# masnottuh/point-cloud-toolbox

Measured on AMD Instinct MI355X. Metric: points/sec curvature (1M-pt torus, k=50); HBM GB/s k-NN vs peak, higher is better.
Workload: dtype f64

## Files before the change

### point-cloud-toolbox_amd/csrc/pct_api.hip

```cpp
#include "pct_internal.h"

#include <execinfo.h>
#include <math.h>
#include <mutex>
#include <signal.h>
#include <stdarg.h>
#include <stdlib.h>
#include <sys/prctl.h>
#include <unistd.h>

int pct_fail(pct_ctx* ctx, int code, const char* fmt, ...) {
    if (ctx) {
        va_list ap;
        va_start(ap, fmt);
        vsnprintf(ctx->err, sizeof(ctx->err), fmt, ap);
        va_end(ap);
    }
    return code;
}

extern char** environ;
const char* pct_getenv(const char* name) {
    struct Entry { const char* name; const char* value; };
    static std::mutex m;
    static Entry cache[48];
    static int used = 0;
    static uintptr_t fp = 0;
    std::lock_guard<std::mutex> g(m);
    uintptr_t now = 1469598103934665603ull;
    for (char** e = environ; e && *e; ++e) now = (now ^ (uintptr_t)*e) * 1099511628211ull;
    if (now != fp) { fp = now; used = 0; }
    for (int i = 0; i < used; ++i)
        if (cache[i].name == name) return cache[i].value;
    const char* v = getenv(name);
    if (used < 48) cache[used++] = Entry{name, v};
    return v;
}

void pct_release(pct_buf* b) {
    if (b->p) (void)hipFree(b->p);
    b->p = nullptr;
    b->cap = 0;
}

int pct_reserve(pct_ctx* ctx, pct_buf* b, size_t bytes) {
    if (bytes == 0) bytes = 16;
    if (b->cap >= bytes) return PCT_OK;
    if (b->p) {
        PCT_HIP(ctx, hipStreamSynchronize(ctx->stream));
        pct_release(b);
    }
    size_t want = bytes + bytes / 8 + 256;
    if (pct_getenv("PCT_NO_HEADROOM")) want = bytes;
    hipError_t e = hipMalloc(&b->p, want);
    if (e != hipSuccess) {
        b->p = nullptr;
        return pct_fail(ctx, PCT_ERR_OOM, "hipMalloc(%zu) failed: %s", want, hipGetErrorString(e));
    }
    b->cap = want;
    return PCT_OK;
}

static void release(pct_buf* b) { pct_release(b); }

static float ev_ms(const hipEvent_t* ev, int a, int b) {
    float ms = 0.f;
    if (hipEventElapsedTime(&ms, ev[a], ev[b]) != hipSuccess) ms = 0.f;
    return ms;
}
static float ev_ms(pct_ctx* ctx, int a, int b) { return ev_ms(ctx->ev, a, b); }

static unsigned long long* stat_slot(pct_ctx* ctx, int par) { return (unsigned long long*)(ctx->pin + (par ? 256 : 192)); }
static long long* svd_slot(pct_ctx* ctx, int par) { return (long long*)(ctx->pin + 2048 + 8 * par); }

static void finish_pending(pct_ctx* ctx, const hipEvent_t* ev) {
    pct_timings t = ctx->tm_snap;
    const unsigned long long* c = stat_slot(ctx, ctx->pend_par);
    t.ring_fallbacks = (int64_t)c[0];
    t.lds_overflows = (int64_t)c[1];
    t.flushes = (int64_t)c[2];
    t.candidate_steps = (int64_t)c[3];
    t.redone_queries = (int64_t)c[4];
    t.grid_ms = ev_ms(ev, 2, 3);
    t.knn_ms = ev_ms(ev, 3, 4);
    t.knn_fast_ms = ctx->pend_sorted ? ev_ms(ev, 3, 7) : 0.f;
    t.fit_ms = ev_ms(ev, 4, 6);
    t.total_ms = ev_ms(ev, 2, 6);
    t.fit_svd_rows = *svd_slot(ctx, ctx->pend_par);
    const int64_t redone = (int64_t)(unsigned)(c[7] & 0xFFFFFFFFull);
    if (ctx->pend_sorted && !ctx->pend_levels) ctx->uneven = redone * 20 > ctx->pend_owned && ctx->pend_owned >= 65536;
    else if (ctx->pend_levels && t.levels <= 1) ctx->uneven = false;
    ctx->tm_done = t;
    ctx->pending = false;
}

static int drain(pct_ctx* ctx) {
    if (!ctx->pending) return PCT_OK;
    const hipError_t e = hipStreamSynchronize(ctx->stream);
    finish_pending(ctx, ctx->ev);
    ctx->tm = ctx->tm_done;
    PCT_HIP(ctx, e);
    return PCT_OK;
}

extern "C" {

const char* pct_version(void) { return "pct_hip 0.1 (gfx950)"; }

int pct_device_count(int* count) {
    int n = 0;
    hipError_t e = hipGetDeviceCount(&n);
    if (e != hipSuccess) n = 0;
    if (count) *count = n;
    return e == hipSuccess ? PCT_OK : PCT_ERR_NO_DEVICE;
}

extern "C++" { const char* pct_last_launch = "(none)"; }
static struct sigaction g_prev_abrt;
static int g_abrt_fd = 2;
static volatile sig_atomic_t g_in_abort_trace = 0;
static void abort_trace(int) {
    if (g_in_abort_trace) {
        sigaction(SIGABRT, &g_prev_abrt, nullptr);
        raise(SIGABRT);
        return;
    }
    g_in_abort_trace = 1;
    static const char head[] = "\n[pct] SIGABRT -- native backtrace of the raising thread";
    const int fd = g_abrt_fd;
    (void)!write(fd, head, sizeof(head) - 1);
    char name[32] = {0};
    if (prctl(PR_GET_NAME, name, 0, 0, 0) == 0) {
        (void)!write(fd, " (", 2);
        (void)!write(fd, name, strnlen(name, sizeof(name)));
        (void)!write(fd, ")", 1);
    }
    (void)!write(fd, ":\n", 2);
    static const char last[] = "[pct] last kernel launched by the library: ";
    (void)!write(fd, last, sizeof(last) - 1);
    const char* ll = __atomic_load_n(&pct_last_launch, __ATOMIC_RELAXED);
    (void)!write(fd, ll, strlen(ll));
    (void)!write(fd, "\n", 1);
    void* frames[64];
    const int n = backtrace(frames, 64);
    backtrace_symbols_fd(frames, n, fd);
    sigaction(SIGABRT, &g_prev_abrt, nullptr);
    raise(SIGABRT);
}
static void install_abort_trace() {
    static std::once_flag once;
    std::call_once(once, [] {
        const char* e = getenv("PCT_ABORT_TRACE");
        if (!e) return;
        const int fd = atoi(e);
        if (fd > 2) g_abrt_fd = fd;
        void* warm[4];
        (void)backtrace(warm, 4);
        struct sigaction sa;
        memset(&sa, 0, sizeof(sa));
        sa.sa_handler = abort_trace;
        sigemptyset(&sa.sa_mask);
        sa.sa_flags = 0;
        sigaction(SIGABRT, &sa, &g_prev_abrt);
    });
}

int pct_create(int device, pct_ctx** out) {
    if (!out) return PCT_ERR_INVALID;
    *out = nullptr;
    install_abort_trace();
    int n = 0;
    if (hipGetDeviceCount(&n) != hipSuccess || n <= 0 || device < 0 || device >= n) return PCT_ERR_NO_DEVICE;
    if (hipSetDevice(device) != hipSuccess) return PCT_ERR_NO_DEVICE;
    pct_ctx* ctx = new pct_ctx();
    ctx->device = device;
    if (hipStreamCreateWithFlags(&ctx->stream, hipStreamNonBlocking) != hipSuccess) {
        delete ctx;
        return PCT_ERR_HIP;
    }
    for (auto& e : ctx->ev)
        if (hipEventCreate(&e) != hipSuccess) {
            delete ctx;
            return PCT_ERR_HIP;
        }
    for (int i = 2; i <= 7; ++i)
        if (hipEventCreate(&ctx->ev_prev[i]) != hipSuccess) {
            delete ctx;
            return PCT_ERR_HIP;
        }
    if (hipHostMalloc((void**)&ctx->pin, 4096, hipHostMallocMapped) != hipSuccess) {
        delete ctx;
        return PCT_ERR_OOM;
    }
    memset(ctx->pin, 0, 4096);
    *out = ctx;
    return PCT_OK;
}

void pct_destroy(pct_ctx* ctx) {
    if (!ctx) return;
    (void)hipSetDevice(ctx->device);
    if (ctx->stream) (void)hipStreamSynchronize(ctx->stream);
    pct_comm_release(ctx);
    pct_buf* all[] = {&ctx->xyz, &ctx->pts4, &ctx->pts4d, &ctx->cell_of, &ctx->cell_cnt, &ctx->cell_fill,
                      &ctx->scan_tmp, &ctx->occ, &ctx->redo, &ctx->row_of, &ctx->owned_pos, &ctx->cell_own, &ctx->cell_oth, &ctx->own_start, &ctx->sorted4, &ctx->sorted4d, &ctx->red, &ctx->nbr_pos,
                      &ctx->nbr_dist, &ctx->nbr_cnt, &ctx->counters, &ctx->coefs, &ctx->K, &ctx->H, &ctx->H2,
                      &ctx->stage_a, &ctx->stage_b, &ctx->stage_c, &ctx->stage_d, &ctx->row_done, &ctx->redo_m, &ctx->flag_buf, &ctx->dens_buf, &ctx->pub_pos, &ctx->pub_dist, &ctx->pub_cnt, &ctx->qpts4, &ctx->fit_flag, &ctx->lvl_src,
                      &ctx->tree_codes, &ctx->tree_vals, &ctx->tree_lvl, &ctx->tree_head, &ctx->tree_marks, &ctx->tree_seg, &ctx->tree_runs, &ctx->tree_range, &ctx->tree_bucket, &ctx->tree_tmp,
                      &ctx->pca, &ctx->pca_aux, &ctx->pca_nbr, &ctx->pca_orig,
                      &ctx->bin_rec, &ctx->bin_mat, &ctx->bin_plan, &ctx->bin_base};
    for (pct_buf* b : all) release(b);
    if (ctx->pin) (void)hipHostFree(ctx->pin);
    for (auto& e : ctx->ev)
        if (e) (void)hipEventDestroy(e);
    for (auto& e : ctx->ev_prev)
        if (e) (void)hipEventDestroy(e);
    if (ctx->stream) (void)hipStreamDestroy(ctx->stream);
    delete ctx;
}

const char* pct_last_error(const pct_ctx* ctx) { return ctx ? ctx->err : "null context"; }

static int begin_call(pct_ctx* ctx, bool wait_for_pending = true) {
    if (!ctx) return PCT_ERR_INVALID;
    ctx->err[0] = 0;
    PCT_HIP(ctx, hipSetDevice(ctx->device));
    if (wait_for_pending) PCT_TRY(drain(ctx));
    return PCT_OK;
}

static int new_cloud(pct_ctx* ctx, int64_t n) {
    if (n <= 0 || n > (int64_t)INT32_MAX - 1024) return pct_fail(ctx, PCT_ERR_INVALID, "cloud size %lld out of range", (long long)n);
    ctx->n = n;
    ctx->q_begin = 0;
    ctx->q_end = n;
    ctx->slab_parts = ctx->slab_part = 0;
    ctx->slab_split_valid = false;
    ctx->grid_valid = ctx->knn_valid = ctx->fit_valid = ctx->pts4_valid = ctx->qpts4_valid = false;
    ctx->pca_valid = false;
    ctx->has_f64 = false;
    ctx->no_cull = ctx->culled = false;
    ctx->retries = 0;
    ctx->tm = pct_timings{};
    return PCT_OK;
}

int pct_set_points_f32(pct_ctx* ctx, const float* xyz, int64_t n) {
    PCT_TRY(begin_call(ctx));
    if (!xyz) return pct_fail(ctx, PCT_ERR_INVALID, "null coordinates");
    PCT_TRY(new_cloud(ctx, n));
    PCT_TRY(pct_reserve(ctx, &ctx->xyz, (size_t)n * 3 * sizeof(float)));
    PCT_HIP(ctx, hipEventRecord(ctx->ev[0], ctx->stream));
    PCT_HIP(ctx, hipMemcpyAsync(ctx->xyz.p, xyz, (size_t)n * 3 * sizeof(float), hipMemcpyHostToDevice, ctx->stream));
    ctx->xyz_view = (const float*)ctx->xyz.p;
    PCT_HIP(ctx, hipEventRecord(ctx->ev[1], ctx->stream));
    PCT_HIP(ctx, hipStreamSynchronize(ctx->stream));
    ctx->tm.upload_ms = ev_ms(ctx, 0, 1);
    return PCT_OK;
}

int pct_set_points_f64(pct_ctx* ctx, const double* xyz, int64_t n) {
    PCT_TRY(begin_call(ctx));
    if (!xyz) return pct_fail(ctx, PCT_ERR_INVALID, "null coordinates");
    PCT_TRY(new_cloud(ctx, n));
    PCT_TRY(pct_reserve(ctx, &ctx->stage_a, (size_t)n * 3 * sizeof(double)));
    PCT_HIP(ctx, hipEventRecord(ctx->ev[0], ctx->stream));
    PCT_HIP(ctx, hipMemcpyAsync(ctx->stage_a.p, xyz, (size_t)n * 3 * sizeof(double), hipMemcpyHostToDevice, ctx->stream));
    PCT_TRY(pct_pack_points_f64(ctx, (const double*)ctx->stage_a.p));
    PCT_HIP(ctx, hipEventRecord(ctx->ev[1], ctx->stream));
    PCT_HIP(ctx, hipStreamSynchronize(ctx->stream));
    ctx->has_f64 = true;
    ctx->tm.upload_ms = ev_ms(ctx, 0, 1);
    return PCT_OK;
}

int pct_set_points_device_f32(pct_ctx* ctx, const void* dev_xyz, int64_t n) {
    PCT_TRY(begin_call(ctx));
    if (!dev_xyz) return pct_fail(ctx, PCT_ERR_INVALID, "null coordinates");
    PCT_TRY(new_cloud(ctx, n));
    PCT_TRY(pct_reserve(ctx, &ctx->xyz, (size_t)n * 3 * sizeof(float)));
    PCT_HIP(ctx, hipMemcpyAsync(ctx->xyz.p, dev_xyz, (size_t)n * 3 * sizeof(float), hipMemcpyDeviceToDevice, ctx->stream));
    PCT_HIP(ctx, hipStreamSynchronize(ctx->stream));
    ctx->xyz_view = (const float*)ctx->xyz.p;
    return PCT_OK;
}

int pct_use_points_device_f32(pct_ctx* ctx, const void* dev_xyz, int64_t n) {
    PCT_TRY(begin_call(ctx));
    if (!dev_xyz) return pct_fail(ctx, PCT_ERR_INVALID, "null coordinates");
    hipPointerAttribute_t attr;
    if (hipPointerGetAttributes(&attr, dev_xyz) != hipSuccess || attr.type != hipMemoryTypeDevice || attr.device != ctx->device) {
        (void)hipGetLastError();
        return pct_fail(ctx, PCT_ERR_INVALID, "pct_use_points_device_f32: not a device pointer of device %d", ctx->device);
    }
    PCT_TRY(new_cloud(ctx, n));
    ctx->xyz_view = (const float*)dev_xyz;
    return PCT_OK;
}

int pct_set_query_range(pct_ctx* ctx, int64_t begin, int64_t end) {
    PCT_TRY(begin_call(ctx));
    if (ctx->n <= 0) return pct_fail(ctx, PCT_ERR_INVALID, "no cloud loaded");
    if (begin < 0 || end > ctx->n || begin > end) return pct_fail(ctx, PCT_ERR_INVALID, "bad query range [%lld,%lld)", (long long)begin, (long long)end);
    ctx->q_begin = begin;
    ctx->q_end = end;
    ctx->slab_parts = ctx->slab_part = 0;
    ctx->slab_split_valid = false;
    ctx->knn_valid = ctx->fit_valid = ctx->grid_valid = false;
    ctx->no_cull = false;
    ctx->retries = 0;
    return PCT_OK;
}

int pct_set_query_slab(pct_ctx* ctx, int32_t part, int32_t parts) {
    PCT_TRY(begin_call(ctx));
    if (ctx->n <= 0) return pct_fail(ctx, PCT_ERR_INVALID, "no cloud loaded");
    if (parts > PCT_SLAB_PARTS_MAX || (parts >= 1 && (part < 0 || part >= parts)))
        return pct_fail(ctx, PCT_ERR_INVALID, "bad slab %d of %d (at most %d parts)", part, parts, PCT_SLAB_PARTS_MAX);
    if (parts >= 1 && (ctx->has_f64 || ctx->n < 4096))
        return pct_fail(ctx, PCT_ERR_INVALID, "slab ownership serves float32 clouds of at least 4096 points (use index ranges)");
    ctx->q_begin = 0;
    ctx->q_end = ctx->n;
    ctx->slab_parts = parts >= 1 ? parts : 0;
    ctx->slab_part = parts >= 1 ? part : 0;
    ctx->slab_split_valid = false;
    ctx->knn_valid = ctx->fit_valid = ctx->grid_valid = false;
    ctx->no_cull = false;
    ctx->retries = 0;
    return PCT_OK;
}

static int refuse_in_slab_mode(pct_ctx* ctx, const char* what) {
    if (ctx->slab_parts >= 1)
        return pct_fail(ctx, PCT_ERR_INVALID, "%s: this handle owns a slab, not an index range (pct_slab_records / pct_scatter_records)", what);
    return PCT_OK;
}

int pct_slab_counts(pct_ctx* ctx, int64_t* counts, int32_t parts) {
    PCT_TRY(begin_call(ctx));
    if (ctx->slab_parts < 1 || !ctx->slab_split_valid || !ctx->fit_valid)
        return pct_fail(ctx, PCT_ERR_INVALID, "pct_slab_counts: no slab pass on this handle (pct_set_query_slab, pct_curvature)");
    if (!counts || parts != ctx->slab_parts) return pct_fail(ctx, PCT_ERR_INVALID, "pct_slab_counts: %d parts asked, the cloud was cut into %d", parts, ctx->slab_parts);
    for (int p = 0; p < parts; ++p) counts[p] = ctx->slab_counts[p];
    return PCT_OK;
}

namespace {
__global__ __launch_bounds__(256) void k_slab_records(const float4* __restrict__ sorted4, const int* __restrict__ owned_pos,
                                                      const float* __restrict__ K, const float* __restrict__ H, int64_t rows,
                                                      float* __restrict__ out) {
    const int64_t r = (int64_t)blockIdx.x * 256 + threadIdx.x;
    if (r >= rows) return;
    out[3 * r + 0] = sorted4[owned_pos[r]].w;
    out[3 * r + 1] = K[r];
    out[3 * r + 2] = H[r];
}

__global__ __launch_bounds__(256) void k_scatter_records(const float* __restrict__ rec, int64_t n_rec, int64_t begin, int64_t end,
                                                         float* __restrict__ K, float* __restrict__ H, unsigned long long* __restrict__ hits) {
    const int64_t i = (int64_t)blockIdx.x * 256 + threadIdx.x;
    bool hit = false;
    if (i < n_rec) {
        const int64_t pub = (int64_t)__float_as_int(rec[3 * i + 0]);
        hit = pub >= begin && pub < end;
        if (hit) {
            K[pub - begin] = rec[3 * i + 1];
            H[pub - begin] = rec[3 * i + 2];
        }
    }
    const unsigned long long m = __ballot(hit);
    if ((threadIdx.x & 63) == 0 && m) atomicAdd(hits, (unsigned long long)__popcll(m));
}
}

int pct_slab_records(pct_ctx* ctx, float* dev_records, int64_t capacity_rows, int64_t* rows_out) {
    PCT_TRY(begin_call(ctx));
    if (ctx->slab_parts < 1 || !ctx->slab_split_valid || !ctx->fit_valid || !ctx->knn_sorted_space || !ctx->fit_row_order)
        return pct_fail(ctx, PCT_ERR_INVALID, "pct_slab_records: no slab pass on this handle (pct_set_query_slab, pct_curvature)");
    const int64_t rows = ctx->q_end - ctx->q_begin;
// ... 793 lines not shown
```

### point-cloud-toolbox_amd/csrc/pct_fit.hip

```cpp
#include "pct_internal.h"

#include <math.h>

namespace {

constexpr int kFitBlock = 64;

struct FitArgs {
    const float4* pts;
    const double4* ptsd;
    const int* table;
    const int* cnt;
    const int64_t* row_query;
    const int* row_query32;
    int64_t row_offset;
    int64_t rows;
    int k;
    int pitch;
    int kp;
    int out_by_row;
    int64_t out_base;
    int q_begin, q_end;
    float* coefs;
    float* K;
    float* H;
    float* H2;
    double* coefs64;
    double* K64;
    double* H64;
    int* flag_list;
    int* flag_count;
    int* flag_next;
    const unsigned long long* stat_src;
    unsigned long long* stat_dst;
    unsigned n_pts;
    const int* row_mask;
    int svd_accumulate;
    int blocks_per_xcd;
};

constexpr double kPivotRatioMin = 1e-6;

#define JACOBI_ROT(app, aqq, apq, arp, arq, vp0, vp1, vp2, vq0, vq1, vq2)          \
    do {                                                                            \
        if (apq != 0.0) {                                                           \
            const double alpha = 0.5 * (aqq - app);                                 \
            const double beta = apq;                                                \
            const double t = (alpha >= 0.0 ? beta : -beta) / (fabs(alpha) + sqrt(alpha * alpha + beta * beta)); \
            const double c = rsqrt(t * t + 1.0);                                    \
            const double s = t * c;                                                 \
            app -= t * apq;                                                         \
            aqq += t * apq;                                                         \
            apq = 0.0;                                                              \
            const double rp = arp, rq = arq;                                        \
            arp = c * rp - s * rq;                                                  \
            arq = s * rp + c * rq;                                                  \
            double a0 = vp0, b0 = vq0; vp0 = c * a0 - s * b0; vq0 = s * a0 + c * b0; \
            double a1 = vp1, b1 = vq1; vp1 = c * a1 - s * b1; vq1 = s * a1 + c * b1; \
            double a2 = vp2, b2 = vq2; vp2 = c * a2 - s * b2; vq2 = s * a2 + c * b2; \
        }                                                                           \
    } while (0)

__device__ __forceinline__ void monge_curvatures(float A, float B, float C, float D, float E, float& Kg, float& Kh) {
    const float Fx = D, Fy = E;
    const float Fxx = 2.0f * A, Fyy = 2.0f * B, Fxy = C;
    const float fx2 = Fx * Fx, fy2 = Fy * Fy;
    const float wgt = (1.0f + fx2) + fy2;
    const float den_k = wgt * wgt;
    const float den_h = (float)((double)wgt * sqrt((double)wgt));
    Kg = (Fxx * Fyy - Fxy * Fxy) / den_k;
    Kh = (((1.0f + fx2) * Fyy - ((2.0f * Fx) * Fy) * Fxy) + (1.0f + fy2) * Fxx) / (2.0f * den_h);
}

template <bool F64>
__device__ __forceinline__ void load_centred(const FitArgs& a, int id, double qx, double qy, double qz,
                                             float qxf, float qyf, float qzf, double& x, double& y, double& z) {
    if (F64) {
        const double4 p = a.ptsd[id];
        x = p.x - qx; y = p.y - qy; z = p.z - qz;
    } else {
        const float4 p = a.pts[id];
        x = (double)(p.x - qxf);
        y = (double)(p.y - qyf);
        z = (double)(p.z - qzf);
    }
}

template <bool F64>
__device__ __forceinline__ void plane_rotation(int m, double sx, double sy, double sz, double sxx, double sxy, double sxz,
                                               double syy, double syz, double szz, double fx, double fy, double fz,
                                               double lx, double ly, double lz, double (&rot)[9]) {
    const double inv_m = 1.0 / (double)m, inv_m1 = 1.0 / (double)(m - 1);
    const double mx = sx * inv_m, my_ = sy * inv_m, mz = sz * inv_m;
    double a00 = (sxx - sx * mx) * inv_m1, a01 = (sxy - sx * my_) * inv_m1, a02 = (sxz - sx * mz) * inv_m1;
    double a11 = (syy - sy * my_) * inv_m1, a12 = (syz - sy * mz) * inv_m1, a22 = (szz - sz * mz) * inv_m1;

    double v00 = 1, v01 = 0, v02 = 0, v10 = 0, v11 = 1, v12 = 0, v20 = 0, v21 = 0, v22 = 1;
#pragma unroll 1
    for (int sweep = 0; sweep < 8; ++sweep) {
        const double off = fabs(a01) + fabs(a02) + fabs(a12);
        if (off <= 1e-22 * (fabs(a00) + fabs(a11) + fabs(a22))) break;
        JACOBI_ROT(a00, a11, a01, a02, a12, v00, v10, v20, v01, v11, v21);
        JACOBI_ROT(a00, a22, a02, a01, a12, v00, v10, v20, v02, v12, v22);
        JACOBI_ROT(a11, a22, a12, a01, a02, v01, v11, v21, v02, v12, v22);
    }
    double n0, n1, n2;
    if (a00 <= a11 && a00 <= a22) { n0 = v00; n1 = v10; n2 = v20; }
    else if (a11 <= a22)          { n0 = v01; n1 = v11; n2 = v21; }
    else                          { n0 = v02; n1 = v12; n2 = v22; }

    double rx, ry, rz;
    if (F64) { rx = lx - fx; ry = ly - fy; rz = lz - fz; }
    else     { rx = (double)((float)lx - (float)fx); ry = (double)((float)ly - (float)fy); rz = (double)((float)lz - (float)fz); }
    {
        const double nn = sqrt((n0 * n0 + n1 * n1) + n2 * n2);
        const double rn = sqrt((rx * rx + ry * ry) + rz * rz);
        const double dot = ((n0 / nn) * (rx / rn) + (n1 / nn) * (ry / rn)) + (n2 / nn) * (rz / rn);
        if (dot < 0) { n0 = -n0; n1 = -n1; n2 = -n2; }
    }
    double r00 = 1, r01 = 0, r02 = 0, r10 = 0, r11 = 1, r12 = 0, r20 = 0, r21 = 0, r22 = 1;
    {
        const double nn = sqrt((n0 * n0 + n1 * n1) + n2 * n2);
        const double ax = n0 / nn, ay = n1 / nn, az = n2 / nn;
        const double v0 = ay, v1 = -ax;
        const double c = az;
        const double s = sqrt(v0 * v0 + v1 * v1);
        if (s != 0.0) {
            const double f = (1.0 - c) / (s * s);
            r00 = 1.0 + (-(v1 * v1)) * f;  r01 = (v1 * v0) * f;            r02 = v1;
            r10 = (v0 * v1) * f;           r11 = 1.0 + (-(v0 * v0)) * f;   r12 = -v0;
            r20 = -v1;                     r21 = v0;                       r22 = 1.0 + (-(v1 * v1) + -(v0 * v0)) * f;
        }
    }

    rot[0] = r00; rot[1] = r01; rot[2] = r02; rot[3] = r10; rot[4] = r11; rot[5] = r12; rot[6] = r20; rot[7] = r21; rot[8] = r22;
}

template <bool F64, bool OUT64 = false, bool STAGED = true, bool MASKED = false>
__global__ __launch_bounds__(kFitBlock) void k_fit(FitArgs a) {
    extern __shared__ int s_idx[];
    const int lane = threadIdx.x;
    if (blockIdx.x == 0) {
        if (lane == 0 && a.flag_next) *a.flag_next = 0;
        if (a.stat_dst && lane < 8) a.stat_dst[lane] = a.stat_src[lane];
    }
    const int64_t row0 = (a.blocks_per_xcd ? (int64_t)(blockIdx.x & 7u) * a.blocks_per_xcd + (blockIdx.x >> 3) : (int64_t)blockIdx.x) * kFitBlock;
    if (row0 >= a.rows) return;
    const int k = a.k, kp = a.kp;

    const int nrow = (int)min((int64_t)kFitBlock, a.rows - row0);
    if constexpr (STAGED) {
        const int sub = lane >> 4, c4 = (lane & 15) << 2;
        for (int cb = 0; cb < k; cb += 64) {
            const int c = cb + c4;
#pragma unroll 4
            for (int r0 = 0; r0 < kFitBlock; r0 += 4) {
                const int r = r0 + sub;
                if (r < nrow && c < a.pitch) {
                    const int4 v = *(const int4*)(a.table + (row0 + r) * a.pitch + c);
                    int* dst = s_idx + r * kp + c;
                    if (c + 0 < k) dst[0] = v.x;
                    if (c + 1 < k) dst[1] = v.y;
                    if (c + 2 < k) dst[2] = v.z;
                    if (c + 3 < k) dst[3] = v.w;
                }
            }
        }
    }
    __syncthreads();

    const int64_t row = row0 + lane;
    if (row >= a.rows) return;
    if constexpr (MASKED) {
        if (!a.row_mask[row]) return;
    }
    const int64_t qid = a.row_query32 ? (int64_t)a.row_query32[row] : a.row_query ? a.row_query[row] : row + a.row_offset;
    const float4 qp = a.pts[qid];
    const int pub = __float_as_int(qp.w);
    if (!a.out_by_row && (pub < a.q_begin || pub >= a.q_end)) return;
    const int64_t out = a.out_by_row ? row : (int64_t)pub - a.out_base;

    double qx = qp.x, qy = qp.y, qz = qp.z;
    if (F64) {
        const double4 qd = a.ptsd[qid];
        qx = qd.x; qy = qd.y; qz = qd.z;
    }
    const int m = a.cnt ? a.cnt[row] : k;
    const int* my = STAGED ? s_idx + lane * kp : a.table + row * a.pitch;
    const float nanf_ = __int_as_float(0x7fc00000);

    const auto hand_over = [&]() {
        const unsigned long long fm = __ballot(1);
        const int leader = (int)__builtin_ctzll(fm);
        int base = 0;
        if (lane == leader) base = atomicAdd(a.flag_count, (int)__popcll(fm));
        base = __shfl(base, leader);
        a.flag_list[base + (int)__popcll(fm & ((1ull << lane) - 1ull))] = (int)row;
    };
    if (m < 6) {
        if constexpr (OUT64) {
            for (int j = 0; j < 6; ++j) a.coefs64[out * 6 + j] = (double)nanf_;
            a.K64[out] = (double)nanf_; a.H64[out] = (double)nanf_;
        } else {
            for (int j = 0; j < 6; ++j) a.coefs[out * 6 + j] = nanf_;
            a.K[out] = nanf_; a.H[out] = nanf_; a.H2[out] = nanf_;
        }
        if (m >= 2) hand_over();
        return;
    }

    double sx = 0, sy = 0, sz = 0, sxx = 0, sxy = 0, sxz = 0, syy = 0, syz = 0, szz = 0;
    double fx = 0, fy = 0, fz = 0, lx = 0, ly = 0, lz = 0;
#define PASS1_ACC(x, y, z)                                                          \
    do {                                                                            \
        sx += x; sy += y; sz += z;                                                  \
        sxx = fma(x, x, sxx); sxy = fma(x, y, sxy); sxz = fma(x, z, sxz);           \
        syy = fma(y, y, syy); syz = fma(y, z, syz); szz = fma(z, z, szz);           \
    } while (0)
    bool bad_id = false;
    const auto checked = [&](int id) {
        bad_id |= (unsigned)id >= a.n_pts;
        return (int)min((unsigned)id, a.n_pts - 1u);
    };
    {
        int j = 0;
        for (; j + 8 <= m; j += 8) {
            double x[8], y[8], z[8];
#pragma unroll
            for (int u = 0; u < 8; ++u) load_centred<F64>(a, checked(my[j + u]), qx, qy, qz, qp.x, qp.y, qp.z, x[u], y[u], z[u]);
            if (j == 0) { fx = x[0]; fy = y[0]; fz = z[0]; }
#pragma unroll
            for (int u = 0; u < 8; ++u) PASS1_ACC(x[u], y[u], z[u]);
            lx = x[7]; ly = y[7]; lz = z[7];
        }
        for (; j < m; ++j) {
            double x, y, z;
            load_centred<F64>(a, checked(my[j]), qx, qy, qz, qp.x, qp.y, qp.z, x, y, z);
            if (j == 0) { fx = x; fy = y; fz = z; }
            PASS1_ACC(x, y, z);
            lx = x; ly = y; lz = z;
        }
    }
#undef PASS1_ACC
    if (bad_id) {
        if constexpr (OUT64) {
            for (int j = 0; j < 6; ++j) a.coefs64[out * 6 + j] = (double)nanf_;
            a.K64[out] = (double)nanf_; a.H64[out] = (double)nanf_;
        } else {
            for (int j = 0; j < 6; ++j) a.coefs[out * 6 + j] = nanf_;
            a.K[out] = nanf_; a.H[out] = nanf_; a.H2[out] = nanf_;
        }
        return;
    }
    double rot[9];
    plane_rotation<F64>(m, sx, sy, sz, sxx, sxy, sxz, syy, syz, szz, fx, fy, fz, lx, ly, lz, rot);
    const double r00 = rot[0], r01 = rot[1], r02 = rot[2], r10 = rot[3], r11 = rot[4], r12 = rot[5], r20 = rot[6], r21 = rot[7], r22 = rot[8];

    double g[21];
    double b[6];
#pragma unroll
    for (int i = 0; i < 21; ++i) g[i] = 0;
#pragma unroll
    for (int i = 0; i < 6; ++i) b[i] = 0;
#define PASS2_ACC(x, y, z)                                                          \
    do {                                                                            \
        const float pa = (float)((r00 * x + r01 * y) + r02 * z);                    \
        const float pb = (float)((r10 * x + r11 * y) + r12 * z);                    \
        const float pz = (float)((r20 * x + r21 * y) + r22 * z);                    \
        double c[6];                                                                \
        c[0] = (double)(pa * pa);                                                   \
        c[1] = (double)(pb * pb);                                                   \
        c[2] = (double)(pa * pb);                                                   \
        c[3] = (double)pa;                                                          \
        c[4] = (double)pb;                                                          \
        c[5] = 1.0;                                                                 \
        const double zz = (double)pz;                                               \
        int t = 0;                                                                  \
        _Pragma("unroll") for (int i = 0; i < 6; ++i) {                             \
            _Pragma("unroll") for (int jj = 0; jj <= i; ++jj) { g[t] = fma(c[i], c[jj], g[t]); ++t; } \
            b[i] = fma(c[i], zz, b[i]);                                             \
        }                                                                           \
    } while (0)
    {
        int j = 0;
        for (; j + 8 <= m; j += 8) {
            double x[8], y[8], z[8];
#pragma unroll
            for (int u = 0; u < 8; ++u) load_centred<F64>(a, my[j + u], qx, qy, qz, qp.x, qp.y, qp.z, x[u], y[u], z[u]);
#pragma unroll
            for (int u = 0; u < 8; ++u) PASS2_ACC(x[u], y[u], z[u]);
        }
        for (; j < m; ++j) {
            double x, y, z;
            load_centred<F64>(a, my[j], qx, qy, qz, qp.x, qp.y, qp.z, x, y, z);
            PASS2_ACC(x, y, z);
        }
    }
#undef PASS2_ACC

#define GI(i, j) ((i) * ((i) + 1) / 2 + (j))
    double dinv[6];
    bool well = true;
#pragma unroll
    for (int j = 0; j < 6; ++j) {
        double d = g[GI(j, j)];
#pragma unroll
        for (int p = 0; p < j; ++p) d -= g[GI(j, p)] * g[GI(j, p)];
        well = well && d > kPivotRatioMin * g[GI(j, j)];
        const double inv = rsqrt(d);
        dinv[j] = inv;
#pragma unroll
        for (int i = j + 1; i < 6; ++i) {
            double s = g[GI(i, j)];
#pragma unroll
            for (int p = 0; p < j; ++p) s -= g[GI(i, p)] * g[GI(j, p)];
            g[GI(i, j)] = s * inv;
        }
    }
#pragma unroll
    for (int i = 0; i < 6; ++i) {
        double s = b[i];
#pragma unroll
        for (int p = 0; p < i; ++p) s -= g[GI(i, p)] * b[p];
        b[i] = s * dinv[i];
    }
#pragma unroll
    for (int i = 5; i >= 0; --i) {
        double s = b[i];
#pragma unroll
        for (int p = i + 1; p < 6; ++p) s -= g[GI(p, i)] * b[p];
        b[i] = s * dinv[i];
    }
#undef GI
    if (!well) hand_over();
    if constexpr (OUT64) {
        double* co64 = a.coefs64 + out * 6;
        for (int j = 0; j < 6; ++j) co64[j] = b[j];
        const double Fx = b[3], Fy = b[4], Fxx = 2.0 * b[0], Fyy = 2.0 * b[1], Fxy = b[2];
        const double wgt = (1.0 + Fx * Fx) + Fy * Fy;
        a.K64[out] = (Fxx * Fyy - Fxy * Fxy) / (wgt * wgt);
        a.H64[out] = (((1.0 + Fx * Fx) * Fyy - ((2.0 * Fx) * Fy) * Fxy) + (1.0 + Fy * Fy) * Fxx) / (2.0 * (wgt * sqrt(wgt)));
        return;
    }
    const float A = (float)b[0], B = (float)b[1], C = (float)b[2];
    const float D = (float)b[3], E = (float)b[4], F = (float)b[5];
    float* co = a.coefs + out * 6;
    co[0] = A; co[1] = B; co[2] = C; co[3] = D; co[4] = E; co[5] = F;

    float Kg, Kh;
    monge_curvatures(A, B, C, D, E, Kg, Kh);
    a.K[out] = Kg;
    a.H[out] = Kh;
    a.H2[out] = Kh * Kh;
}

__global__ __launch_bounds__(256) void k_curv(const float* __restrict__ coefs, int64_t rows, float* __restrict__ K,
                                              float* __restrict__ H, float* __restrict__ H2) {
    const int64_t r = (int64_t)blockIdx.x * 256 + threadIdx.x;
    if (r >= rows) return;
    const float* c = coefs + r * 6;
    float Kg, Kh;
    monge_curvatures(c[0], c[1], c[2], c[3], c[4], Kg, Kh);
    K[r] = Kg;
    H[r] = Kh;
    H2[r] = Kh * Kh;
}

struct Lstsq6 {
    double A[6][6];
    double y[6];

    __device__ __forceinline__ void init() {
#pragma unroll
        for (int c = 0; c < 6; ++c) {
            y[c] = 0;
#pragma unroll
            for (int r = 0; r < 6; ++r) A[c][r] = 0;
        }
    }

    __device__ __forceinline__ void add(float pa, float pb, float pc) {
        double x[6] = {(double)(pa * pa), (double)(pb * pb), (double)(pa * pb), (double)pa, (double)pb, 1.0};
        double zi = (double)pc;
#pragma unroll
        for (int r = 0; r < 6; ++r) {
            const double xr = x[r];
            if (xr != 0.0) {
                const double rr = A[r][r];
                const double h = sqrt(rr * rr + xr * xr);
                const double inv = 1.0 / h;
                const double c = rr * inv, sn = xr * inv;
                A[r][r] = h;
#pragma unroll
                for (int c2 = r + 1; c2 < 6; ++c2) {
                    const double t = A[c2][r];
                    A[c2][r] = c * t + sn * x[c2];
                    x[c2] = c * x[c2] - sn * t;
                }
                const double t = y[r];
                y[r] = c * t + sn * zi;
                zi = c * zi - sn * t;
            }
        }
    }

    __device__ __forceinline__ void solve(int m, double (&sol)[6]) {
        double V[6][6];
#pragma unroll
        for (int c = 0; c < 6; ++c)
#pragma unroll
            for (int r = 0; r < 6; ++r) V[c][r] = c == r ? 1.0 : 0.0;
#pragma unroll 1
        for (int sweep = 0; sweep < 40; ++sweep) {
            bool rotated = false;
#pragma unroll
            for (int p = 0; p < 5; ++p) {
#pragma unroll
                for (int q = p + 1; q < 6; ++q) {
                    double al = 0, be = 0, ga = 0;
#pragma unroll
                    for (int r = 0; r < 6; ++r) {
                        al = fma(A[p][r], A[p][r], al);
                        be = fma(A[q][r], A[q][r], be);
                        ga = fma(A[p][r], A[q][r], ga);
                    }
                    if (ga != 0.0 && fabs(ga) > 1e-15 * sqrt(al * be)) {
                        rotated = true;
                        const double zeta = (be - al) / (2.0 * ga);
                        const double t = (zeta >= 0.0 ? 1.0 : -1.0) / (fabs(zeta) + sqrt(1.0 + zeta * zeta));
                        const double c = rsqrt(1.0 + t * t), sn = c * t;
#pragma unroll
                        for (int r = 0; r < 6; ++r) {
                            const double ap = A[p][r], aq = A[q][r];
                            A[p][r] = c * ap - sn * aq;
                            A[q][r] = sn * ap + c * aq;
                            const double vp = V[p][r], vq = V[q][r];
                            V[p][r] = c * vp - sn * vq;
                            V[q][r] = sn * vp + c * vq;
                        }
                    }
                }
            }
            if (!__any(rotated)) break;
        }
        double sig2[6], smax2 = 0;
#pragma unroll
        for (int c = 0; c < 6; ++c) {
            double t = 0;
#pragma unroll
            for (int r = 0; r < 6; ++r) t = fma(A[c][r], A[c][r], t);
            sig2[c] = t;
            smax2 = fmax(smax2, t);
        }
        const double rcond = 2.220446049250313e-16 * (double)(m > 6 ? m : 6);
        const double cut = rcond * sqrt(smax2);
#pragma unroll
        for (int r = 0; r < 6; ++r) sol[r] = 0;
#pragma unroll
        for (int c = 0; c < 6; ++c) {
            if (sqrt(sig2[c]) > cut) {
                double t = 0;
#pragma unroll
                for (int r = 0; r < 6; ++r) t = fma(A[c][r], y[r], t);
                const double w = t / sig2[c];
#pragma unroll
                for (int r = 0; r < 6; ++r) sol[r] = fma(V[c][r], w, sol[r]);
            }
        }
    }
};

template <bool F64, bool OUT64>
__global__ __launch_bounds__(64) void k_fit_svd(FitArgs a, const int* __restrict__ list, const int* __restrict__ list_count,
                                                long long* __restrict__ host_count) {
    const int total = *list_count;
    if (blockIdx.x == 0 && threadIdx.x == 0) *host_count = (a.svd_accumulate ? *host_count : 0ll) + total;
    const float nanf_ = __int_as_float(0x7fc00000);
    for (int64_t it = (int64_t)blockIdx.x * 64 + threadIdx.x; it < total; it += (int64_t)gridDim.x * 64) {
        const int64_t row = list[it];
        const int64_t qid = a.row_query32 ? (int64_t)a.row_query32[row] : a.row_query ? a.row_query[row] : row + a.row_offset;
        const float4 qp = a.pts[qid];
        const int64_t out = a.out_by_row ? row : (int64_t)__float_as_int(qp.w) - a.out_base;
        double qx = qp.x, qy = qp.y, qz = qp.z;
        if (F64) { const double4 qd = a.ptsd[qid]; qx = qd.x; qy = qd.y; qz = qd.z; }
        const int m = a.cnt ? a.cnt[row] : a.k;
        const int* my = a.table + row * a.pitch;

        double sx = 0, sy = 0, sz = 0, sxx = 0, sxy = 0, sxz = 0, syy = 0, syz = 0, szz = 0;
        double fx = 0, fy = 0, fz = 0, lx = 0, ly = 0, lz = 0;
        for (int j = 0; j < m; ++j) {
            double x, y, z;
            load_centred<F64>(a, (int)min((unsigned)my[j], a.n_pts - 1u), qx, qy, qz, qp.x, qp.y, qp.z, x, y, z);
            if (j == 0) { fx = x; fy = y; fz = z; }
            lx = x; ly = y; lz = z;
            sx += x; sy += y; sz += z;
            sxx = fma(x, x, sxx); sxy = fma(x, y, sxy); sxz = fma(x, z, sxz);
            syy = fma(y, y, syy); syz = fma(y, z, syz); szz = fma(z, z, szz);
        }
        double rot[9];
        plane_rotation<F64>(m, sx, sy, sz, sxx, sxy, sxz, syy, syz, szz, fx, fy, fz, lx, ly, lz, rot);

        Lstsq6 ls;
        ls.init();
#pragma unroll 1
        for (int j = 0; j < m; ++j) {
            double px, py, pz;
            load_centred<F64>(a, (int)min((unsigned)my[j], a.n_pts - 1u), qx, qy, qz, qp.x, qp.y, qp.z, px, py, pz);
            ls.add((float)((rot[0] * px + rot[1] * py) + rot[2] * pz), (float)((rot[3] * px + rot[4] * py) + rot[5] * pz),
                   (float)((rot[6] * px + rot[7] * py) + rot[8] * pz));
        }
        double sol[6];
        ls.solve(m, sol);
        if (m < 2) {
#pragma unroll
            for (int r = 0; r < 6; ++r) sol[r] = (double)nanf_;
        }
        if constexpr (OUT64) {
            double* co64 = a.coefs64 + out * 6;
            for (int j = 0; j < 6; ++j) co64[j] = sol[j];
            const double Fx = sol[3], Fy = sol[4], Fxx = 2.0 * sol[0], Fyy = 2.0 * sol[1], Fxy = sol[2];
            const double wgt = (1.0 + Fx * Fx) + Fy * Fy;
            a.K64[out] = (Fxx * Fyy - Fxy * Fxy) / (wgt * wgt);
            a.H64[out] = (((1.0 + Fx * Fx) * Fyy - ((2.0 * Fx) * Fy) * Fxy) + (1.0 + Fy * Fy) * Fxx) / (2.0 * (wgt * sqrt(wgt)));
        } else {
            const float Af = (float)sol[0], Bf = (float)sol[1], Cf = (float)sol[2], Df = (float)sol[3], Ef = (float)sol[4];
            float* co = a.coefs + out * 6;
            co[0] = Af; co[1] = Bf; co[2] = Cf; co[3] = Df; co[4] = Ef; co[5] = (float)sol[5];
            float Kg, Kh;
            monge_curvatures(Af, Bf, Cf, Df, Ef, Kg, Kh);
            a.K[out] = Kg;
            a.H[out] = Kh;
            a.H2[out] = Kh * Kh;
        }
    }
}

template <bool F64>
__global__ __launch_bounds__(64) void k_plane_rotate(const void* __restrict__ nbrs, int64_t batch, int m, double* __restrict__ out) {
    const int64_t b = (int64_t)blockIdx.x * 64 + threadIdx.x;
    if (b >= batch) return;
    const auto at = [&](int j, double& x, double& y, double& z) {
        if (F64) { const double* p = (const double*)nbrs + (b * m + j) * 3; x = p[0]; y = p[1]; z = p[2]; }
        else { const float* p = (const float*)nbrs + (b * m + j) * 3; x = (double)p[0]; y = (double)p[1]; z = (double)p[2]; }
    };
    double mx = 0, my = 0, mz = 0;
    for (int j = 0; j < m; ++j) { double x, y, z; at(j, x, y, z); mx += x; my += y; mz += z; }
    mx /= (double)m; my /= (double)m; mz /= (double)m;
    double sxx = 0, sxy = 0, sxz = 0, syy = 0, syz = 0, szz = 0;
    for (int j = 0; j < m; ++j) {
        double x, y, z;
        at(j, x, y, z);
        x -= mx; y -= my; z -= mz;
        sxx = fma(x, x, sxx); sxy = fma(x, y, sxy); sxz = fma(x, z, sxz);
        syy = fma(y, y, syy); syz = fma(y, z, syz); szz = fma(z, z, szz);
    }
    double fx, fy, fz, lx, ly, lz;
    at(0, fx, fy, fz);
    at(m - 1, lx, ly, lz);
    double rot[9];
    plane_rotation<F64>(m, 0.0, 0.0, 0.0, sxx, sxy, sxz, syy, syz, szz, fx, fy, fz, lx, ly, lz, rot);
    for (int j = 0; j < m; ++j) {
        double x, y, z;
        at(j, x, y, z);
        double* o = out + (b * m + j) * 3;
        o[0] = (rot[0] * x + rot[1] * y) + rot[2] * z;
        o[1] = (rot[3] * x + rot[4] * y) + rot[5] * z;
        o[2] = (rot[6] * x + rot[7] * y) + rot[8] * z;
    }
}

__global__ __launch_bounds__(64) void k_quadric_rows(const float* __restrict__ pts, int64_t batch, int m, float* __restrict__ coefs) {
    const int64_t b = (int64_t)blockIdx.x * 64 + threadIdx.x;
    if (b >= batch) return;
    Lstsq6 ls;
    ls.init();
#pragma unroll 1
    for (int j = 0; j < m; ++j) {
        const float* p = pts + (b * m + j) * 3;
        ls.add(p[0], p[1], p[2]);
    }
    double sol[6];
    ls.solve(m, sol);
    for (int j = 0; j < 6; ++j) coefs[b * 6 + j] = (float)sol[j];
}

__global__ __launch_bounds__(256) void k_prefix_rows(const int* __restrict__ sample_row, const int* __restrict__ owned_pos,
                                                     int q_begin, int64_t n_samples, int n_lo, int n_hi,
                                                     const int* __restrict__ nbr_pos, int nbr_pitch,
                                                     int* __restrict__ table, int pitch, int* __restrict__ cnt,
                                                     int64_t* __restrict__ row_query) {
    const int nn = n_hi - n_lo + 1;
    const int64_t row = blockIdx.x;
    if (row >= n_samples * nn) return;
    const int64_t s = row / nn;
    const int n = n_lo + (int)(row - s * nn);
    const int trow = sample_row[s];
    const int q = owned_pos ? owned_pos[trow] : trow + q_begin;
    int* dst = table + row * pitch;
    for (int j = threadIdx.x; j <= n; j += 256) dst[j] = j == 0 ? q : nbr_pos[(int64_t)trow * nbr_pitch + (j - 1)];
    if (threadIdx.x == 0) { cnt[row] = n + 1; row_query[row] = q; }
}

__global__ __launch_bounds__(256) void k_gather_fit(const int* __restrict__ row_of, int64_t first, int64_t rows,
                                                    const float* __restrict__ coefs, const float* __restrict__ K,
                                                    const float* __restrict__ H, const float* __restrict__ H2,
                                                    float* __restrict__ o_coefs, float* __restrict__ o_K,
                                                    float* __restrict__ o_H, float* __restrict__ o_H2) {
    const int64_t i = (int64_t)blockIdx.x * 256 + threadIdx.x;
    if (i >= rows) return;
    const int64_t r = row_of[first + i];
    if (o_coefs) {
#pragma unroll
        for (int j = 0; j < 6; ++j) o_coefs[i * 6 + j] = coefs[r * 6 + j];
    }
    if (o_K) o_K[i] = K[r];
    if (o_H) o_H[i] = H[r];
    if (o_H2) o_H2[i] = H2[r];
}

int launch(pct_ctx* ctx, const FitArgs& a0, bool f64) {
    FitArgs a = a0;
    a.kp = a.k | 1;
    if (a.row_mask && ((size_t)kFitBlock * a.kp * sizeof(int) > 64 * 1024 || a.coefs64))
        return pct_fail(ctx, PCT_ERR_INVALID, "masked fit: rows too long");
    size_t lds = (size_t)kFitBlock * a.kp * sizeof(int);
    const bool staged = lds <= 64 * 1024;
    if (!staged) lds = 0;
    int blocks = (int)((a.rows + kFitBlock - 1) / kFitBlock);
    if (blocks <= 0) return PCT_OK;
    a.blocks_per_xcd = pct_getenv("PCT_NO_XCD_MAP") ? 0 : (blocks + 7) / 8;
    if (a.blocks_per_xcd) blocks = a.blocks_per_xcd * 8;
    PCT_TRY(pct_reserve(ctx, &ctx->fit_flag, 64 + (size_t)a.rows * sizeof(int)));
    if (ctx->fit_flag.p != ctx->fit_flag_seen || ctx->fit_flag.cap != ctx->fit_flag_cap_seen) {
        PCT_HIP(ctx, hipMemsetAsync(ctx->fit_flag.p, 0, 64, ctx->stream));
        ctx->fit_flag_seen = ctx->fit_flag.p;
        ctx->fit_flag_cap_seen = ctx->fit_flag.cap;
        ctx->fit_parity = 0;
    }
    a.stat_src = nullptr;
    a.stat_dst = nullptr;
    if (ctx->stats_mirror_req && ctx->counters.p) {
        a.stat_src = (const unsigned long long*)ctx->counters.p;
        a.stat_dst = (unsigned long long*)(ctx->pin + (ctx->fit_par ? 256 : 192));
        ctx->stats_mirrored = true;
    }
    ctx->stats_mirror_req = false;
    a.flag_count = (int*)ctx->fit_flag.p + ctx->fit_parity;
    a.flag_next = (int*)ctx->fit_flag.p + (ctx->fit_parity ^ 1);
    ctx->fit_parity ^= 1;
    a.flag_list = (int*)ctx->fit_flag.p + 16;
#define PCT_FIT_LAUNCH(F_, O_)                                                                                      \
    do {                                                                                                            \
        if (a.row_mask && staged && !O_) PCT_LAUNCH((k_fit<F_, false, true, true>), dim3(blocks), dim3(kFitBlock), lds, ctx->stream, a); \
        else if (staged) PCT_LAUNCH((k_fit<F_, O_, true>), dim3(blocks), dim3(kFitBlock), lds, ctx->stream, a);  \
        else PCT_LAUNCH((k_fit<F_, O_, false>), dim3(blocks), dim3(kFitBlock), 0, ctx->stream, a);          \
    } while (0)
    if (a.coefs64) {
        if (f64) PCT_FIT_LAUNCH(true, true);
        else PCT_FIT_LAUNCH(false, true);
    } else if (f64) PCT_FIT_LAUNCH(true, false);
    else PCT_FIT_LAUNCH(false, false);
#undef PCT_FIT_LAUNCH
    PCT_HIP(ctx, hipGetLastError());
    const int sblocks = blocks < 1024 ? blocks : 1024;
    long long* note = (long long*)(ctx->pin + 2048 + 8 * ctx->fit_par);
    if (a.coefs64) {
        if (f64)
            PCT_LAUNCH((k_fit_svd<true, true>), dim3(sblocks), dim3(64), 0, ctx->stream, a, a.flag_list, a.flag_count, note);
        else
            PCT_LAUNCH((k_fit_svd<false, true>), dim3(sblocks), dim3(64), 0, ctx->stream, a, a.flag_list, a.flag_count, note);
    } else if (f64)
        PCT_LAUNCH((k_fit_svd<true, false>), dim3(sblocks), dim3(64), 0, ctx->stream, a, a.flag_list, a.flag_count, note);
    else
        PCT_LAUNCH((k_fit_svd<false, false>), dim3(sblocks), dim3(64), 0, ctx->stream, a, a.flag_list, a.flag_count, note);
    PCT_HIP(ctx, hipGetLastError());
    return PCT_OK;
}

}

int pct_launch_fit_pass(pct_ctx* ctx, int64_t rows) {
    const int64_t nq = ctx->q_end - ctx->q_begin;
    PCT_TRY(pct_reserve(ctx, &ctx->coefs, (size_t)nq * 6 * sizeof(float)));
    PCT_TRY(pct_reserve(ctx, &ctx->K, (size_t)nq * sizeof(float)));
    PCT_TRY(pct_reserve(ctx, &ctx->H, (size_t)nq * sizeof(float)));
    PCT_TRY(pct_reserve(ctx, &ctx->H2, (size_t)nq * sizeof(float)));
    FitArgs a = {};
    a.pts = (const float4*)ctx->sorted4.p;
    a.ptsd = ctx->has_f64 ? (const double4*)ctx->sorted4d.p : nullptr;
    a.table = (const int*)ctx->nbr_pos.p;
    a.cnt = ctx->eps > 0 ? (const int*)ctx->nbr_cnt.p : nullptr;
    a.row_query32 = (const int*)ctx->owned_pos.p;
    a.rows = rows;
    a.k = ctx->k;
    a.pitch = (ctx->k + 3) & ~3;
    a.out_by_row = 0;
    a.out_base = ctx->q_begin;
    a.q_begin = (int)ctx->q_begin;
    a.q_end = (int)ctx->q_end;
    a.coefs = (float*)ctx->coefs.p;
    a.K = (float*)ctx->K.p;
    a.H = (float*)ctx->H.p;
    a.H2 = (float*)ctx->H2.p;
    a.n_pts = (unsigned)ctx->n_grid;
    a.row_mask = (const int*)ctx->row_done.p;
    a.svd_accumulate = 1;
    return launch(ctx, a, ctx->has_f64);
}

int pct_launch_fit_table(pct_ctx* ctx) {
    if (ctx->levels_fitted) {
        ctx->levels_fitted = false;
        ctx->fit_row_order = false;
        return PCT_OK;
    }
    const int64_t nq = ctx->q_end - ctx->q_begin;
    PCT_TRY(pct_reserve(ctx, &ctx->coefs, (size_t)nq * 6 * sizeof(float)));
    PCT_TRY(pct_reserve(ctx, &ctx->K, (size_t)nq * sizeof(float)));
    PCT_TRY(pct_reserve(ctx, &ctx->H, (size_t)nq * sizeof(float)));
    PCT_TRY(pct_reserve(ctx, &ctx->H2, (size_t)nq * sizeof(float)));
    FitArgs a = {};
    const bool sorted = ctx->knn_sorted_space;
    a.pts = (const float4*)(sorted ? ctx->sorted4.p : ctx->pts4.p);
    a.ptsd = ctx->has_f64 ? (const double4*)(sorted ? ctx->sorted4d.p : ctx->pts4d.p) : nullptr;
    a.table = (const int*)ctx->nbr_pos.p;
    a.cnt = ctx->eps > 0 ? (const int*)ctx->nbr_cnt.p : nullptr;
    a.row_query = nullptr;
    a.row_query32 = sorted ? (const int*)ctx->owned_pos.p : nullptr;
    a.row_offset = sorted ? 0 : ctx->q_begin;
    a.rows = nq;
    a.k = ctx->k;
    a.pitch = ctx->nbr_pitch;
    a.out_by_row = sorted ? 1 : 0;
    ctx->fit_row_order = sorted;
    a.out_base = ctx->q_begin;
    a.q_begin = (int)ctx->q_begin;
    a.q_end = (int)ctx->q_end;
    a.coefs = (float*)ctx->coefs.p;
    a.K = (float*)ctx->K.p;
    a.H = (float*)ctx->H.p;
    a.H2 = (float*)ctx->H2.p;
    a.n_pts = (unsigned)(sorted ? ctx->n_grid : ctx->n);
    return launch(ctx, a, ctx->has_f64);
}

int pct_launch_gather_fit(pct_ctx* ctx, int64_t first, int64_t rows, float* d_coefs, float* d_K, float* d_H, float* d_H2) {
    PCT_TRY(pct_ensure_row_of(ctx));
    PCT_LAUNCH(k_gather_fit, dim3((unsigned)((rows + 255) / 256)), dim3(256), 0, ctx->stream, (const int*)ctx->row_of.p,
                       first, rows, (const float*)ctx->coefs.p, (const float*)ctx->K.p, (const float*)ctx->H.p,
                       (const float*)ctx->H2.p, d_coefs, d_K, d_H, d_H2);
    PCT_HIP(ctx, hipGetLastError());
    return PCT_OK;
}

int pct_launch_fit_rows(pct_ctx* ctx, const int32_t* d_idx, const int32_t* d_cnt, const int64_t* d_query,
                        int64_t rows, int32_t k, int32_t pitch, float* d_coefs, float* d_K, float* d_H, float* d_H2,
                        bool sorted_space) {
    FitArgs a = {};
    a.pts = (const float4*)(sorted_space ? ctx->sorted4.p : ctx->pts4.p);
    a.ptsd = ctx->has_f64 ? (const double4*)(sorted_space ? ctx->sorted4d.p : ctx->pts4d.p) : nullptr;
    a.table = d_idx;
    a.cnt = d_cnt;
    a.row_query = d_query;
    a.rows = rows;
    a.k = k;
    a.pitch = pitch;
    a.out_by_row = 1;
    a.out_base = 0;
    a.q_begin = 0;
    a.q_end = (int)ctx->n;
    a.coefs = d_coefs;
    a.K = d_K;
    a.H = d_H;
    a.H2 = d_H2;
    a.n_pts = (unsigned)(sorted_space ? ctx->n_grid : ctx->n);
    return launch(ctx, a, ctx->has_f64);
}

int pct_launch_fit_rows_f64(pct_ctx* ctx, const int32_t* d_idx, const int32_t* d_cnt, const int64_t* d_query, int64_t rows,
                            int32_t k, int32_t pitch, double* d_coefs, double* d_K, double* d_H) {
    PCT_TRY(pct_ensure_plain_records(ctx));
    FitArgs a = {};
    a.pts = (const float4*)ctx->qpts4.p;
    a.ptsd = ctx->has_f64 ? (const double4*)ctx->pts4d.p : nullptr;
    a.table = d_idx;
    a.cnt = d_cnt;
    a.row_query = d_query;
    a.rows = rows;
    a.k = k;
    a.pitch = pitch;
    a.out_by_row = 1;
    a.q_begin = 0;
    a.q_end = (int)ctx->n;
    a.coefs64 = d_coefs;
    a.K64 = d_K;
    a.H64 = d_H;
    a.n_pts = (unsigned)ctx->n;
    return launch(ctx, a, ctx->has_f64);
}

int pct_launch_prefix_rows(pct_ctx* ctx, const int* d_sample_row, int64_t n_samples, int n_lo, int n_hi, int* d_table,
                           int pitch, int* d_cnt, int64_t* d_row_query) {
    const int64_t rows = n_samples * (n_hi - n_lo + 1);
    PCT_LAUNCH(k_prefix_rows, dim3((unsigned)rows), dim3(256), 0, ctx->stream, d_sample_row,
                       ctx->knn_sorted_space ? (const int*)ctx->owned_pos.p : nullptr, (int)ctx->q_begin, n_samples, n_lo, n_hi,
                       (const int*)ctx->nbr_pos.p, ctx->nbr_pitch, d_table, pitch, d_cnt, d_row_query);
    PCT_HIP(ctx, hipGetLastError());
    return PCT_OK;
}

int pct_launch_curvatures(pct_ctx* ctx, const float* d_coefs, int64_t rows, float* d_K, float* d_H, float* d_H2) {
    const int blocks = (int)((rows + 255) / 256);
    if (blocks <= 0) return PCT_OK;
    PCT_LAUNCH(k_curv, dim3(blocks), dim3(256), 0, ctx->stream, d_coefs, rows, d_K, d_H, d_H2);
    PCT_HIP(ctx, hipGetLastError());
    return PCT_OK;
}

int pct_launch_plane_rotate(pct_ctx* ctx, const void* d_nbrs, bool f64, int64_t batch, int32_t m, double* d_out) {
    const unsigned blocks = (unsigned)((batch + 63) / 64);
    if (f64)
        PCT_LAUNCH(k_plane_rotate<true>, dim3(blocks), dim3(64), 0, ctx->stream, d_nbrs, batch, m, d_out);
    else
        PCT_LAUNCH(k_plane_rotate<false>, dim3(blocks), dim3(64), 0, ctx->stream, d_nbrs, batch, m, d_out);
    PCT_HIP(ctx, hipGetLastError());
    return PCT_OK;
}

int pct_launch_quadric_rows(pct_ctx* ctx, const float* d_pts, int64_t batch, int32_t m, float* d_coefs) {
    PCT_LAUNCH(k_quadric_rows, dim3((unsigned)((batch + 63) / 64)), dim3(64), 0, ctx->stream, d_pts, batch, m, d_coefs);
    PCT_HIP(ctx, hipGetLastError());
    return PCT_OK;
}
```

### point-cloud-toolbox_amd/csrc/pct_internal.h

```cpp
#pragma once

#include <hip/hip_runtime.h>
#include <stdint.h>
#include <stdio.h>
#include <string.h>
#include <stdlib.h>

#include "../../include/pct_hip.h"

#define PCT_WAVE 64
#define PCT_K_MAX 511

extern const char* pct_last_launch;
#define PCT_STR2(x) #x
#define PCT_STR(x) PCT_STR2(x)
#define PCT_LAUNCH(kernelName, ...)                                                          \
    do {                                                                                     \
        __atomic_store_n(&pct_last_launch, __FILE__ ":" PCT_STR(__LINE__) "  " #kernelName, __ATOMIC_RELAXED); \
        hipLaunchKernelGGL((kernelName), __VA_ARGS__);                                       \
    } while (0)

struct pct_grid {
    double ox, oy, oz;
    double cell;
    double inv_cell;
    int32_t nx, ny, nz;
    int64_t ncell;
    double lim_lo[3], lim_hi[3];
};

struct pct_buf {
    void* p = nullptr;
    size_t cap = 0;
};

struct pct_comm;

struct pct_ctx {
    int device = 0;
    pct_comm* comm = nullptr;
    hipStream_t stream = nullptr;
    hipEvent_t ev[9] = {};
    hipEvent_t ev_prev[9] = {};
    bool async_mode = false;
    bool pending = false;
    int pend_par = 0;
    bool pend_sorted = false, pend_levels = false;
    int64_t pend_owned = 0;
    int fit_par = 0;
    pct_timings tm_snap = {};
    pct_timings tm_done = {};
    char err[512] = {0};

    int64_t n = 0;
    int64_t q_begin = 0, q_end = 0;
    int64_t n_grid = 0, g_begin = 0;
    bool culled = false;
    bool no_cull = false;
    float cull_box[6] = {0, 0, 0, 0, 0, 0};
    bool cull_box_valid = false;
    int64_t cull_box_n = 0, cull_box_q0 = 0, cull_box_q1 = 0;
    int32_t retries = 0;
    int32_t slab_part = 0, slab_parts = 0;
    int32_t slab_axis = 0, slab_bin_lo = 0, slab_bin_hi = 0;
    float slab_x0 = 0, slab_inv = 0;
    float slab_bbox[6] = {0, 0, 0, 0, 0, 0};
    int64_t slab_counts[PCT_SLAB_PARTS_MAX] = {};
    bool slab_split_valid = false;
    double hint_edge = 0, hint_guess = 0, hint_target = 0;
    float spec_bbox[6] = {0, 0, 0, 0, 0, 0};
    float spec_raw[6] = {0, 0, 0, 0, 0, 0};
    int64_t spec_n = 0;
    bool spec_valid = false;
    const void* own_flag = nullptr;
    float own_lo = 0, own_hi = 0;
    float level_box[6] = {0, 0, 0, 0, 0, 0};
    bool level_box_valid = false;
    int64_t own_count = 0;
    double level_edge = 0;
    bool level_mode = false;
    bool levels_fuse_fit = false;
    bool levels_fitted = false;
    pct_buf lvl_src;
    bool lvl_src_valid = false;
    float lvl_bbox[6] = {0, 0, 0, 0, 0, 0};
    int tree_bits = 0;
    int64_t tree_segs = 0;
    double tree_two_level_share = 1.0;
    int tree_level_spread = 0;
    pct_buf tree_codes, tree_vals;
    pct_buf tree_lvl;
    pct_buf tree_head, tree_marks;
    pct_buf tree_seg, tree_runs;
    pct_buf tree_range;
    pct_buf tree_bucket;
    pct_buf tree_tmp;
    pct_buf row_done;
    pct_buf redo_m;
    pct_buf flag_buf;
    pct_buf dens_buf;
    pct_buf pub_pos, pub_dist, pub_cnt;
    bool uneven = false;
    bool auto_probe = false;
    bool auto_probe_tree = false;
    bool grid_skewed = false;
    float auto_tree_bbox[6] = {0, 0, 0, 0, 0, 0};
    float tree_bbox[6] = {0, 0, 0, 0, 0, 0};
    bool tree_check_bbox = false, tree_hint_mismatch = false;
    int64_t auto_tree_n = 0;
    int32_t auto_tree_calls = 0;
    bool last_levels = false;
    bool has_f64 = false;
    double occupancy_factor = 0.0;
    bool collect_stats = false;

    pct_buf xyz;
    const float* xyz_view = nullptr;
    pct_buf pts4;
    pct_buf pts4d;
    pct_grid grid = {};
    pct_buf cell_of;
    pct_buf cell_cnt;
    pct_buf cell_own;
    pct_buf cell_oth;
    pct_buf own_start;
    pct_buf cell_fill;
    pct_buf scan_tmp;
    pct_buf bin_rec;
    pct_buf bin_mat;
    pct_buf bin_plan;
    pct_buf bin_base;
    pct_buf occ;
    pct_buf redo;
    int64_t n_items = 0;
    int64_t nonempty_cells = 0;
    int32_t items_q = 12;
    pct_buf sorted4;
    pct_buf sorted4d;
    pct_buf row_of;
    bool row_of_valid = true;
    int64_t row_of_rows = 0;
    int32_t row_of_begin = 0;
    pct_buf owned_pos;
    pct_buf red;
    unsigned char* pin = nullptr;
    int64_t n_occ = 0;
    bool grid_valid = false;
    bool pts4_valid = false;

    pct_buf nbr_pos;
    pct_buf nbr_dist;
    pct_buf nbr_cnt;
    int32_t k = 0;
    int32_t nbr_pitch = 0;
    double eps = 0.0;
    bool counters_clean = false;
    int fit_parity = 0;
    void* fit_flag_seen = nullptr;
    size_t fit_flag_cap_seen = 0;
    bool stats_mirror_req = false;
    bool stats_mirrored = false;
    bool knn_valid = false;
    bool knn_sorted_space = false;
    bool skip_dist_req = false;
    bool dist_valid = true;
    pct_buf counters;

    pct_buf coefs;
    pct_buf K, H, H2;
    int64_t fit_rows = 0;
    bool fit_valid = false;
    bool fit_row_order = false;
    bool fit_cloud_aligned = false;

    pct_buf fit_flag;
    pct_buf stage_a, stage_b, stage_c, stage_d;
    pct_buf qpts4;
    bool qpts4_valid = false;

    pct_buf pca;
    pct_buf pca_aux;
    pct_buf pca_nbr;
    pct_buf pca_orig;
    bool pca_valid = false, pca_has_nbr = false, pca_recentred = false;
    int32_t pca_k = 0;
    int64_t pca_rows = 0;

    pct_timings tm = {};
};

int pct_fail(pct_ctx* ctx, int code, const char* fmt, ...);
const char* pct_getenv(const char* name);
void pct_comm_release(pct_ctx* ctx);

#ifndef PCT_FAST_R1_MAX
#define PCT_FAST_R1_MAX 61
#endif
inline int pct_fast_r1_max() {
    static const int v = [] { const char* e = getenv("PCT_FAST_R1_MAX"); const int x = e ? atoi(e) : PCT_FAST_R1_MAX; return x < 2 ? 2 : x > 64 ? 64 : x; }();
    return v;
}
inline double pct_default_factor(int k) {
    if (k + 1 <= pct_fast_r1_max()) {
        const double per_cell = k <= 47 ? 27.0 : k >= 52 ? 29.5 : 27.0 + 0.5 * (k - 47);
        return per_cell / (k + 1);
    }
    const double n = k + 1;
    if (n > 128) return 0.35;
    return n <= 85 ? 0.52 : n <= 101 ? 0.52 - 0.07 * (n - 85) / 16.0 : 0.45 - 0.05 * (n - 101) / 27.0;
}
int pct_reserve(pct_ctx* ctx, pct_buf* b, size_t bytes);
void pct_release(pct_buf* b);

__host__ __device__ inline unsigned long long pct_spread3(unsigned v) {
    unsigned long long x = v & 0x1fffffu;
    x = (x | x << 32) & 0x1f00000000ffffull;
    x = (x | x << 16) & 0x1f0000ff0000ffull;
    x = (x | x << 8) & 0x100f00f00f00f00full;
    x = (x | x << 4) & 0x10c30c30c30c30c3ull;
    x = (x | x << 2) & 0x1249249249249249ull;
    return x;
}
__host__ __device__ inline unsigned pct_compact3(unsigned long long x) {
    x &= 0x1249249249249249ull;
    x = (x ^ (x >> 2)) & 0x10c30c30c30c30c3ull;
    x = (x ^ (x >> 4)) & 0x100f00f00f00f00full;
    x = (x ^ (x >> 8)) & 0x1f0000ff0000ffull;
    x = (x ^ (x >> 16)) & 0x1f00000000ffffull;
    x = (x ^ (x >> 32)) & 0x1fffffull;
    return (unsigned)x;
}
__host__ __device__ inline void pct_stencil_cell(int t, int* dx, int* dy, int* dz) {
    const int i = t == 0 ? 13 : t == 13 ? 0 : t;
    *dx = i % 3 - 1;
    *dy = (i / 3) % 3 - 1;
    *dz = i / 9 - 1;
}
__device__ inline int64_t pct_code_lower_bound(const unsigned long long* __restrict__ codes, int64_t n, unsigned long long key) {
    int64_t lo = 0, hi = n;
    while (lo < hi) {
        const int64_t mid = (lo + hi) >> 1;
        if (codes[mid] < key) lo = mid + 1; else hi = mid;
    }
    return lo;
}
constexpr int kTreeBucketBits = 18, kTreeBucketShift = 63 - kTreeBucketBits;
__device__ inline int64_t pct_code_lower_bound(const unsigned long long* __restrict__ codes, const int* __restrict__ bucket,
                                               unsigned long long key) {
    const unsigned p = (unsigned)(key >> kTreeBucketShift);
    int64_t lo = bucket[p], hi = bucket[p + 1];
    while (lo < hi) {
        const int64_t mid = (lo + hi) >> 1;
        if (codes[mid] < key) lo = mid + 1; else hi = mid;
    }
    return lo;
}

#define PCT_HIP(ctx, call)                                                        \
    do {                                                                          \
        hipError_t e_ = (call);                                                   \
        if (e_ != hipSuccess)                                                     \
            return pct_fail((ctx), e_ == hipErrorOutOfMemory ? PCT_ERR_OOM : PCT_ERR_HIP, \
                            "%s failed: %s (%s:%d)", #call, hipGetErrorString(e_), __FILE__, __LINE__); \
    } while (0)

#define PCT_TRY(expr)            \
    do {                         \
        int s_ = (expr);         \
        if (s_ != PCT_OK) return s_; \
    } while (0)

int pct_pack_points(pct_ctx* ctx, float* bbox6);
int pct_pack_points_f64(pct_ctx* ctx, const double* d_xyz64);
int pct_build_grid(pct_ctx* ctx, int32_t k, double eps);
int pct_launch_knn_grid(pct_ctx* ctx, int32_t k, double eps, bool exact_only, int phase = 0);
int pct_launch_knn_brute(pct_ctx* ctx, int32_t k, double eps);
int pct_item_census(pct_ctx* ctx, int32_t k, unsigned long long out4[4]);
int pct_knn_levels(pct_ctx* ctx, int32_t k, double eps);
int pct_build_tree(pct_ctx* ctx, int32_t k, double eps, bool* usable);
int pct_launch_knn_tree(pct_ctx* ctx, int32_t k, double eps);
int pct_launch_export_neighbors(pct_ctx* ctx, int64_t begin, int64_t end,
                                int32_t* d_idx, float* d_dist, int32_t* d_cnt);
int pct_launch_fit_table(pct_ctx* ctx);
int pct_launch_fit_pass(pct_ctx* ctx, int64_t rows);
int pct_launch_fit_rows(pct_ctx* ctx, const int32_t* d_idx, const int32_t* d_cnt,
                        const int64_t* d_query, int64_t rows, int32_t k, int32_t pitch,
                        float* d_coefs, float* d_K, float* d_H, float* d_H2, bool sorted_space);
int pct_launch_prefix_rows(pct_ctx* ctx, const int* d_sample_pos, int64_t n_samples, int n_lo, int n_hi, int* d_table,
                           int pitch, int* d_cnt, int64_t* d_row_query);
int pct_launch_gather_fit(pct_ctx* ctx, int64_t first, int64_t rows, float* d_coefs, float* d_K, float* d_H, float* d_H2);
int pct_launch_curvatures(pct_ctx* ctx, const float* d_coefs, int64_t rows, float* d_K, float* d_H, float* d_H2);
int pct_launch_plane_rotate(pct_ctx* ctx, const void* d_nbrs, bool f64, int64_t batch, int32_t m, double* d_out);
int pct_launch_quadric_rows(pct_ctx* ctx, const float* d_pts, int64_t batch, int32_t m, float* d_coefs);
int pct_launch_selftest(pct_ctx* ctx, int* d_fails);
int pct_ensure_plain_records(pct_ctx* ctx);
int pct_launch_fit_rows_f64(pct_ctx* ctx, const int32_t* d_idx, const int32_t* d_cnt, const int64_t* d_query, int64_t rows,
                            int32_t k, int32_t pitch, double* d_coefs, double* d_K, double* d_H);
int pct_launch_query_points(pct_ctx* ctx, const double* d_q, int64_t m, int32_t k, double eps, int32_t* d_idx, double* d_dist);
int pct_launch_gather_int(pct_ctx* ctx, const int* d_map, int* d_inout, int64_t n);
int pct_ensure_row_of(pct_ctx* ctx);
int pct_launch_export_rows(pct_ctx* ctx, const int64_t* d_rows, int64_t n_rows, int32_t* d_idx, float* d_dist, int32_t* d_cnt);
int pct_launch_mesh_energies(pct_ctx* ctx, const double* d_v, const int* d_tri, int64_t n_tri, const void* d_K, const void* d_H,
                             bool f64, double* d_partial, int nblk, double* d_out);
int pct_voxel_downsample_device(pct_ctx* ctx, const void* d_xyz, bool f64, int64_t n, double voxel, int64_t* d_out, int64_t* count);
int pct_launch_surface_variation(pct_ctx* ctx, float* d_out);
#define PCT_PCA_EXTRA 16
int pct_pca_prep(pct_ctx* ctx, double* round_off, bool* nonfinite, double origin[3]);
int pct_pca_restore(pct_ctx* ctx);
int pct_launch_pca(pct_ctx* ctx, int32_t k, double round2, const double origin[3], bool keep_neighbors, int64_t* exact_rows);
```

### point-cloud-toolbox_amd/csrc/pct_knn.hip

```cpp
#include "pct_knn_sweep.h"

namespace {

constexpr unsigned kPadElem = 0xFFFFFFFFu;

template <int R>
struct FastK {
    unsigned e[R];
};

__device__ __forceinline__ unsigned umed3(unsigned a, unsigned b, unsigned c) {
    unsigned r;
    asm("v_med3_u32 %0, %1, %2, %3" : "=v"(r) : "v"(a), "v"(b), "v"(c));
    return r;
}

struct SortLanes {
    unsigned sel[6];
    int a31, a63;
};

__device__ __forceinline__ SortLanes make_sort_lanes() {
    SortLanes c;
    const int lane = lane_id();
// ... 116 lines not shown
            double pd = INFINITY;
#pragma unroll
            for (int r2 = 0; r2 < R; ++r2)
                if (pr == r2) { pe = be[r2]; pd = __hiloint2double(bhi[r2], blo[r2]); }
            const bool same = pr >= 0 && pr < R && e[r] != kPadElem && pe != kPadElem && ((e[r] ^ pe) >> SLOT_BITS) == 0u;
            bool p_lt_m = pd < d[r], m_lt_p = d[r] < pd;
            const bool tie = same && pd == d[r];
            if (__builtin_amdgcn_ballot_w64(tie) != 0ull) {
                const int my_pos = pos_of(e[r] & PAYLOAD), p_pos = pos_of(pe & PAYLOAD);
                if (tie) {
                    const int mp = pub_index(pts, my_pos), pp = pub_index(pts, p_pos);
                    p_lt_m = pp < mp;
                    m_lt_p = mp < pp;
                }
            }
            const bool take = same && (pl > lane ? p_lt_m : m_lt_p);
            if (take) { e[r] = pe; d[r] = pd; }
            any |= take;
        }
        if (__builtin_amdgcn_ballot_w64(any) != 0ull) quiet = 0;
        else if (++quiet == 2) return true;
    }
    return false;
}

#ifndef PCT_FAST_WAVES
#define PCT_FAST_WAVES 4
#endif
template <int R> constexpr int kFastWaves = PCT_FAST_WAVES;

typedef float float2v __attribute__((ext_vector_type(2)));


template <int R, bool EPS, bool PRE, bool PAIR = false, bool Q64 = false, bool TREE = false>
__global__ __launch_bounds__(64 * kFastWaves<R>, (TREE ? (R == 1 ? (PCT_TREE_CAP <= 512 ? 6 : PCT_TREE_CAP <= 768 ? 4 : 3) : (PCT_TREE_CAP2 <= 768 ? 4 : 3)) : R == 1 ? (Q64 ? 5 : 6) : 4)) void k_knn_fast(KnnArgs a, const int2* __restrict__ items, int64_t n_items,
                                                                  int items_q, int* __restrict__ redo,
                                                                  int* __restrict__ redo_count) {
#ifndef PCT_STAGE_CAP2
#define PCT_STAGE_CAP2 768
#endif
    constexpr int CAP = TREE ? (R == 1 ? PCT_TREE_CAP : PCT_TREE_CAP2) : R == 1 ? kStageCap : PCT_STAGE_CAP2;
    constexpr int SLOT_BITS = PRE ? (R == 1 ? 6 : 7) : (R == 1 ? 9 : 10);
    constexpr int KEY_BITS = 32 - SLOT_BITS;
    constexpr int CAP_POW2 = 1024;
    static_assert(CAP <= CAP_POW2, "staging capacity");
    static_assert(PRE || CAP <= (1 << SLOT_BITS), "slot field too narrow");
    __shared__ float s_cx[kFastWaves<R>][CAP];
    __shared__ float s_cy[kFastWaves<R>][CAP];
    __shared__ float s_cz[kFastWaves<R>][CAP];
    __shared__ unsigned s_pend[kFastWaves<R>][64 * R];
    __shared__ unsigned short s_pend2[kFastWaves<R>][PAIR ? 64 * R : 2];
    __shared__ int s_offc[kFastWaves<R>][16];

    const int w = __builtin_amdgcn_readfirstlane(threadIdx.x >> 6);
    const int lane = lane_id();
    const int64_t item = (int64_t)blockIdx.x * kFastWaves<R> + w;
    if (item >= n_items) return;
    const SortLanes sort_dir = make_sort_lanes();

    pct_grid g = a.g;
    const int* __restrict__ cs = a.cell_start;
    const int2 it2 = items[item];
    int cx, cy, cz, qs, nq, row0;
    constexpr int NRUNS = TREE ? 27 : 9;
    int run_s = 0, run_len = 0;
    float* cand_x = s_cx[w];
    float* cand_y = s_cy[w];
    float* cand_z = s_cz[w];
    unsigned* pend = s_pend[w];
    int* offc = s_offc[w];
    if constexpr (TREE) {
        const int seg = __builtin_amdgcn_readfirstlane(it2.y);
        if (seg < 0) return;
        const unsigned packed = (unsigned)__builtin_amdgcn_readfirstlane(it2.x);
        qs = (int)(packed & 0x3ffffffu);
        nq = (int)(packed >> 26) + 1;
        row0 = qs;
        const int4 hd = a.tree_seg[seg];
        const int level = __builtin_amdgcn_readfirstlane(hd.x);
        cx = __builtin_amdgcn_readfirstlane(hd.y);
        cy = __builtin_amdgcn_readfirstlane(hd.z);
        cz = __builtin_amdgcn_readfirstlane(hd.w);
        g.cell = __builtin_ldexp(a.g.cell, level);
        g.inv_cell = __builtin_ldexp(a.g.inv_cell, -level);
        g.nx = g.ny = g.nz = 1 << (a.tree_bits - level);
        if (lane < 27) {
            const int2 r = a.tree_runs[(int64_t)seg * 27 + lane];
            run_s = r.x;
            run_len = r.y;
        }
    } else {
        const int cell = __builtin_amdgcn_readfirstlane(it2.x);
        const int chunk = __builtin_amdgcn_readfirstlane(it2.y);
        cx = cell % g.nx;
        cy = (cell / g.nx) % g.ny;
        cz = cell / (g.nx * g.ny);
        qs = cs[cell] + chunk * items_q;
        const int qe = min(cs[cell] + a.cell_own[cell], qs + items_q);
        nq = qe - qs;
        row0 = a.own_start[cell] + chunk * items_q;

        if (lane < 9) {
            const int z = cz + kRowOrder[lane][0], y = cy + kRowOrder[lane][1];
            if (z >= 0 && z < g.nz && y >= 0 && y < g.ny) {
                const int row = (z * g.ny + y) * g.nx;
                run_s = cs[row + max(cx - 1, 0)];
                run_len = cs[row + min(cx + 1, g.nx - 1) + 1] - run_s;
            }
        }
    }
    float4 my_q = make_float4(0.f, 0.f, 0.f, 0.f);
    double4 my_qd = make_double4(0., 0., 0., 0.);
    if (lane < nq) {
        my_q = a.pts[qs + lane];
        if (a.ptsd) my_qd = a.ptsd[qs + lane];
    }
    float my_eq = 0.f;
    if constexpr (Q64) {
        const double ex = my_qd.x - (double)my_q.x, ey = my_qd.y - (double)my_q.y, ez = my_qd.z - (double)my_q.z;
        my_eq = (float)sqrt((ex * ex + ey * ey) + ez * ez) * (1.0f + 0x1p-22f);
        if (!(my_eq >= 0.f)) my_eq = INFINITY;
    }
    int my_pre = 0, m = 0;
    {
        int acc = 0;
#pragma unroll
        for (int t = 0; t < NRUNS; ++t) {
            my_pre = lane == t ? acc : my_pre;
            acc += __builtin_amdgcn_readlane(run_len, t);
        }
        m = acc;
    }
    unsigned long long n_flush = 0, n_step = 0, n_redo = 0;
    unsigned long long redo_mask = 0ull, redo_why_lo = 0ull, redo_why_hi = 0ull;
    const auto note_redo = [&](int row, int why) {
        const int q = row - row0;
        redo_mask |= 1ull << q;
        redo_why_lo |= (unsigned long long)(why & 1) << q;
        redo_why_hi |= (unsigned long long)((why >> 1) & 1) << q;
    };

    const bool hopeless = !EPS && a.row_done != nullptr && m < a.k + 1;
    const bool crowded = TREE && __popcll(__builtin_amdgcn_ballot_w64(lane < NRUNS && run_len > 0)) > 16;
    if (m > CAP || hopeless || crowded) {
        if (a.row_done) {
            if (lane < nq) a.redo_m[row0 + lane] = ((hopeless ? 1 : 2) << 29) | min(m, (1 << 29) - 1);
            return;
        }
        int base = 0;
        if (lane == 0) base = atomicAdd(redo_count, nq);
        base = __builtin_amdgcn_readfirstlane(base);
        if (lane < nq) {
            redo[base + lane] = row0 + lane;
        }
        if (a.stats && lane == 0) {
            if (!hopeless) atomicAdd(&a.counters[1], 1ull);
            atomicAdd(&a.counters[4], (unsigned long long)nq);
        }
        return;
    }

    unsigned run_code[(CAP / 64 + 7) / 8];
#pragma unroll
    for (int i = 0; i < (CAP / 64 + 7) / 8; ++i) run_code[i] = 0u;
    {
        unsigned* bits = pend;
        static_assert(CAP / 32 <= 64 * R, "bit string does not fit the list area");
        if (lane < CAP / 32) bits[lane] = 0u;
        wave_lds_sync();
        const bool nonempty = lane < NRUNS && run_len > 0;
        const unsigned long long ne = __builtin_amdgcn_ballot_w64(nonempty);
        if (nonempty) {
            atomicOr(&bits[my_pre >> 5], 1u << (my_pre & 31));
            offc[__builtin_amdgcn_mbcnt_lo((unsigned)ne, 0)] = run_s - my_pre;
        }
        wave_lds_sync();
        float4 tmp[CAP / 64];
        int ubase = -1;
#pragma unroll
        for (int b = 0; b < CAP / 64; ++b) {
            tmp[b] = make_float4(0.f, 0.f, 0.f, 0.f);
            if (b * 64 < m) {
                const unsigned lo = (unsigned)__builtin_amdgcn_readfirstlane((int)bits[2 * b]);
                const unsigned hi = (unsigned)__builtin_amdgcn_readfirstlane((int)bits[2 * b + 1]);
                const unsigned long long B = ((unsigned long long)hi << 32) | lo;
                const unsigned long long S = B >> 1;
                const int c0 = ubase + (int)(lo & 1u);
                const int u = (int)__builtin_amdgcn_mbcnt_hi((unsigned)(S >> 32), __builtin_amdgcn_mbcnt_lo((unsigned)S, (unsigned)c0));
                ubase += (int)__popcll(B);
                const int j = b * 64 + lane;
                run_code[b >> 3] |= (unsigned)u << (4 * (b & 7));
                if (j < m) tmp[b] = a.pts[j + offc[u]];
            }
        }
        wave_lds_sync();
#pragma unroll
        for (int b = 0; b < CAP / 64; ++b) {
            const int j = b * 64 + lane;
            if (j < m) {
                cand_x[j] = tmp[b].x; cand_y[j] = tmp[b].y; cand_z[j] = tmp[b].z;
            } else if (PRE && (b & ~1) * 64 < m) {
                cand_x[j] = INFINITY; cand_y[j] = 0.f; cand_z[j] = 0.f;
            }
        }
    }
    wave_lds_sync();
    const int k = a.k;
    const double eps2 = EPS ? a.eps2 : (double)INFINITY;
    constexpr double kKeyRange = 2.3;
    const double scale = (double)(1u << KEY_BITS) / (kKeyRange * g.cell * g.cell);
    const unsigned key_max = (1u << KEY_BITS) - 1u;
    unsigned my_gkey;
    {
        const double lqx = a.ptsd ? my_qd.x : (double)my_q.x, lqy = a.ptsd ? my_qd.y : (double)my_q.y,
                     lqz = a.ptsd ? my_qd.z : (double)my_q.z;
        const double gx = (lqx - g.ox) * g.inv_cell - cx;
        const double gy = (lqy - g.oy) * g.inv_cell - cy;
        const double gz = (lqz - g.oz) * g.inv_cell - cz;
        const double g2 = fmin(guaranteed_r2(g, cx, cy, cz, gx, gy, gz, 1), limit_r2(g, cx, cy, cz, gx, gy, gz));
        my_gkey = g2 == INFINITY ? 0xFFFFFFFFu : (unsigned)fmin(g2 * scale, 4294967294.0);
    }
    const unsigned eps_key = EPS && eps2 < 1e300 ? (unsigned)fmin(ceil(eps2 * scale), 4294967295.0) : 0xFFFFFFFFu;

    constexpr int NB = CAP / 64;
    constexpr int LIST = 64 * R;
    unsigned t_prev = 0;
    float t_prev_f = 0.f;
    const float cell2f = (float)(g.cell * g.cell);
    const float eps2a = EPS ? (float)fmin(eps2 * (1.0 + 0x1p-18), 3.0e38) : INFINITY;
    const double eps1 = EPS ? sqrt(eps2) * (1.0 + 0x1p-50) : 0.0;

    if constexpr (PRE && PAIR) {
        unsigned short* pend_b = s_pend2[w];
        const auto push_redo = [&](int row, int why) { note_redo(row, why); };
        const auto cut_key = [&](float T, double eq) {
            double lo2 = (double)T * (1.0 - 0x1p-20);
            if constexpr (Q64) {
                const double root_up = (double)__builtin_sqrtf(T) * (1.0 + 0x1p-21);
                lo2 = fmax(lo2 - 2.0 * eq * root_up, 0.0);
            }
            return (unsigned)fmin(lo2 * scale, 4294967294.0);
        };
        const auto pair_loop = [&](auto NBP_, auto GUARD_) {
            constexpr int NBP = decltype(NBP_)::value, NBU = 2 * NBP;
            constexpr bool GUARD = decltype(GUARD_)::value;
            for (int qi = 0; qi < nq; qi += 2) {
                const bool live_b = qi + 1 < nq;
                const int qj = live_b ? qi + 1 : qi;
                const int row_a = row0 + qi, row_b = row0 + qj;
                float ax, ay, az, bx, by, bz;
                if constexpr (!Q64) {
                    ax = __int_as_float(__builtin_amdgcn_readlane(__float_as_int(my_q.x), qi));
                    ay = __int_as_float(__builtin_amdgcn_readlane(__float_as_int(my_q.y), qi));
                    az = __int_as_float(__builtin_amdgcn_readlane(__float_as_int(my_q.z), qi));
                    bx = __int_as_float(__builtin_amdgcn_readlane(__float_as_int(my_q.x), qj));
                    by = __int_as_float(__builtin_amdgcn_readlane(__float_as_int(my_q.y), qj));
                    bz = __int_as_float(__builtin_amdgcn_readlane(__float_as_int(my_q.z), qj));
                }
                double qax, qay, qaz, qbx, qby, qbz, eq_a = 0.0, eq_b = 0.0;
                if constexpr (Q64) {
                    const auto rl = [&](double v, int l) {
                        return __hiloint2double(__builtin_amdgcn_readlane(__double2hiint(v), l), __builtin_amdgcn_readlane(__double2loint(v), l));
                    };
                    qax = rl(my_qd.x, qi); qay = rl(my_qd.y, qi); qaz = rl(my_qd.z, qi);
                    qbx = rl(my_qd.x, qj); qby = rl(my_qd.y, qj); qbz = rl(my_qd.z, qj);
                    ax = (float)qax; ay = (float)qay; az = (float)qaz;
                    bx = (float)qbx; by = (float)qby; bz = (float)qbz;
                    eq_a = (double)__int_as_float(__builtin_amdgcn_readlane(__float_as_int(my_eq), qi));
                    eq_b = (double)__int_as_float(__builtin_amdgcn_readlane(__float_as_int(my_eq), qj));
                } else {
                    qax = (double)ax; qay = (double)ay; qaz = (double)az; qbx = (double)bx; qby = (double)by; qbz = (double)bz;
                }
                float ap_a[NBU], ap_b[NBU];
#pragma unroll
                for (int p2 = 0; p2 < NBP; ++p2) {
                    ap_a[2 * p2] = ap_a[2 * p2 + 1] = INFINITY;
                    ap_b[2 * p2] = ap_b[2 * p2 + 1] = INFINITY;
                    if (!GUARD || p2 * 128 < m) {
                        const int sa = p2 * 128 + lane, sb = sa + 64;
                        const float2v vx = {cand_x[sa], cand_x[sb]}, vy = {cand_y[sa], cand_y[sb]}, vz = {cand_z[sa], cand_z[sb]};
                        {
                            const float2v dx = vx - ax, dy = vy - ay, dz = vz - az;
                            float2v d = dx * dx;
                            d = __builtin_elementwise_fma(dy, dy, d);
                            d = __builtin_elementwise_fma(dz, dz, d);
                            ap_a[2 * p2] = d.x;
                            ap_a[2 * p2 + 1] = d.y;
                        }
                        {
                            const float2v dx = vx - bx, dy = vy - by, dz = vz - bz;
                            float2v d = dx * dx;
                            d = __builtin_elementwise_fma(dy, dy, d);
                            d = __builtin_elementwise_fma(dz, dz, d);
                            ap_b[2 * p2] = d.x;
                            ap_b[2 * p2 + 1] = d.y;
                        }
                        n_step += 4;
                    }
                }
                float T_a = EPS ? eps2a : INFINITY, T_b = T_a;
                if constexpr (EPS && Q64) {
                    const double ea = eps1 + eq_a, eb = eps1 + eq_b;
                    T_a = (float)fmin(ea * ea * (1.0 + 0x1p-18), 3.0e38);
                    T_b = (float)fmin(eb * eb * (1.0 + 0x1p-18), 3.0e38);
                }
                int tot_a = m, tot_b = m;
// ... 389 lines not shown
                        if (b * 64 < m) c += (int)__popcll(__builtin_amdgcn_ballot_w64(key[b] < t));
                    if (c >= k + 1 && c <= LIST) { T = t; cnt = c; found = true; break; }
                    if (c < k + 1) lo = t; else hi = t;
                    if (hi - lo <= 1u) break;
                    const float guess = (float)t * target * __builtin_amdgcn_rcpf((float)(c > 0 ? c : 1));
                    unsigned nt = guess >= 4294967040.f ? hi : (unsigned)guess;
                    if (c == 0) nt = t * 4u > t ? t * 4u : hi;
                    if (nt <= lo || nt >= hi) nt = lo + (hi - lo) / 2u;
                    t = nt;
                }
                if (!found) {
                    note_redo(row, 3);
                    continue;
                }
            }
            t_prev = T <= key_max ? T : t_prev;

            {
                int base = 0;
                wave_lds_sync();
#pragma unroll
                for (int b = 0; b < NB; ++b) {
                    if (b * 64 < m) {
                        const bool pass = key[b] < T;
                        const unsigned long long mask = __builtin_amdgcn_ballot_w64(pass);
                        if (pass) {
                            const int at = base + __builtin_amdgcn_mbcnt_hi((unsigned)(mask >> 32), __builtin_amdgcn_mbcnt_lo((unsigned)mask, 0));
                            pend[at] = (key[b] << SLOT_BITS) | (unsigned)(b * 64 + lane);
                        }
                        base += (int)__popcll(mask);
                    }
                }
                wave_lds_sync();
                const int have = cnt < LIST ? cnt : LIST;
#pragma unroll
                for (int r = 0; r < R; ++r) {
                    const int i = lane + 64 * r;
                    best.e[r] = i < have ? pend[i] : kPadElem;
                }
                wave_lds_sync();
                fast_sort_from<R, 2>(best, sort_dir);
                ++n_flush;
            }
        }
        unsigned tau;
        {
            const int sl = k >> 6, src = k & 63;
            unsigned v = best.e[0];
#pragma unroll
            for (int r = 1; r < R; ++r)
                if (sl == r) v = best.e[r];
            tau = (unsigned)__builtin_amdgcn_readlane((int)v, src);
        }

        bool sparse = false;
        {
            const unsigned gkey = (unsigned)__builtin_amdgcn_readlane((int)my_gkey, qi);
            const unsigned tkey = tau >> SLOT_BITS;
            const unsigned need = min(tau == kPadElem ? 0xFFFFFFFFu : tkey + 1u, eps_key);
            sparse = need > gkey;
            amb |= need > min(gkey, bkey);
            amb |= tau != kPadElem && tkey >= key_max - 1u;
        }
        {
#pragma unroll
            for (int r = 0; r < R; ++r) {
                unsigned up = __shfl_down(best.e[r], 1);
                if (r + 1 < R) {
                    const unsigned first_next = (unsigned)__builtin_amdgcn_readlane((int)best.e[r + 1 < R ? r + 1 : r], 0);
                    if (lane == 63) up = first_next;
                } else if (lane == 63) {
                    up = kPadElem;
                }
                const int i = lane + 64 * r;
                col |= i <= k && best.e[r] != kPadElem && up != kPadElem && ((best.e[r] ^ up) >> SLOT_BITS) == 0u;
            }
        }
        if (__ballot(amb) != 0ull) {
            note_redo(row, sparse ? 1 : 3);
            continue;
        }
        const auto slot_pos = [&](int j) {
            unsigned code = (unsigned)__builtin_amdgcn_ds_bpermute((j & 63) << 2, (int)run_code[0]);
            if constexpr ((CAP / 64 + 7) / 8 > 1) {
                const unsigned hi = (unsigned)__builtin_amdgcn_ds_bpermute((j & 63) << 2, (int)run_code[1]);
                code = (j >> 9) ? hi : code;
            }
            return j + offc[(code >> ((((unsigned)j >> 6) & 7u) << 2)) & 15u];
        };
        if (__ballot(col) != 0ull) {
            const auto slot_of = [&](unsigned at) {
                int j = (int)at;
                if constexpr (PRE) j = (int)pend[j] & (CAP_POW2 - 1);
                return j;
            };
            const bool done = order_equal_keys<R, SLOT_BITS>(&best.e[0], a.pts,
                [&](unsigned at) {
                    const int j = slot_of(at);
                    const double dx = (double)cand_x[j] - qx, dy = (double)cand_y[j] - qy, dz = (double)cand_z[j] - qz;
                    return (dx * dx + dy * dy) + dz * dz;
                },
                [&](unsigned at) { return slot_pos(slot_of(at) & (CAP_POW2 - 1)); });
            if (!done) {
                note_redo(row, 3);
                continue;
            }
        }

        int found = 0;
#pragma unroll
        for (int r = 0; r < R; ++r) {
            const int i = lane + 64 * r;
            const unsigned e = best.e[r];
            const bool real = e != kPadElem;
            int j = (int)(e & ((1u << SLOT_BITS) - 1u));
            if constexpr (PRE) j = (int)pend[j] & (CAP_POW2 - 1);
            unsigned code = (unsigned)__builtin_amdgcn_ds_bpermute((j & 63) << 2, (int)run_code[0]);
            if constexpr ((CAP / 64 + 7) / 8 > 1) {
                const unsigned hi = (unsigned)__builtin_amdgcn_ds_bpermute((j & 63) << 2, (int)run_code[1]);
                code = (j >> 9) ? hi : code;
            }
            const unsigned t = (code >> ((((unsigned)j >> 6) & 7u) << 2)) & 15u;
            const int pos_real = j + offc[t];
            if (i >= 1 && i <= k) {
                int pos = -1;
                float dist = INFINITY;
                if (real) {
                    const double dx = (double)cand_x[j] - qx, dy = (double)cand_y[j] - qy, dz = (double)cand_z[j] - qz;
                    dist = (float)sqrt((dx * dx + dy * dy) + dz * dz);
                    pos = pos_real;
                }
                a.nbr_pos[(int64_t)row * a.pitch + (i - 1)] = pos;
                a.nbr_dist[(int64_t)row * a.pitch + (i - 1)] = dist;
                found += real;
            }
        }
        if (a.nbr_cnt) {
            for (int o = 32; o > 0; o >>= 1) found += __shfl_xor(found, o);
            if (lane == 0) a.nbr_cnt[row] = found;
        }
        if (a.row_done && lane == 0) a.row_done[row] = 1;
    }
    if (redo_mask) {
        const int cnt = (int)__popcll(redo_mask);
        if (a.row_done) {
            if ((redo_mask >> lane) & 1ull) {
                const int why = (int)((redo_why_lo >> lane) & 1ull) | ((int)((redo_why_hi >> lane) & 1ull) << 1);
                a.redo_m[row0 + lane] = (why << 29) | min(m, (1 << 29) - 1);
            }
        } else {
            int base = 0;
            if (lane == 0) base = atomicAdd(redo_count, cnt);
            base = __builtin_amdgcn_readfirstlane(base);
            if ((redo_mask >> lane) & 1ull) redo[base + (int)__popcll(redo_mask & ((1ull << lane) - 1ull))] = row0 + lane;
        }
        n_redo += (unsigned long long)cnt;
    }
    if (a.stats && lane == 0) {
        atomicAdd(&a.counters[2], n_flush);
        atomicAdd(&a.counters[3], n_step);
        if (n_redo) atomicAdd(&a.counters[4], n_redo);
    }
}

#ifndef PCT_SORT_INC
#define PCT_SORT_INC "pct_sort_pair.inc"
#endif
#include PCT_SORT_INC

__device__ __forceinline__ void sort_pair_asm(unsigned& ea, unsigned& eb, const SortLanes& c) {
    unsigned ta, tb;
    asm volatile(PCT_SORT_PAIR_ASM
                 : [ea] "+v"(ea), [eb] "+v"(eb), [ta] "=&v"(ta), [tb] "=&v"(tb)
                 : [sel0] "v"(c.sel[0]), [sel1] "v"(c.sel[1]), [sel2] "v"(c.sel[2]), [sel3] "v"(c.sel[3]), [sel4] "v"(c.sel[4]),
                   [sel5] "v"(c.sel[5]), [a31] "v"(c.a31), [a63] "v"(c.a63));
    ea = PCT_SORT_PAIR_RESULT_A;
    eb = PCT_SORT_PAIR_RESULT_B;
}

struct PairArgs {
    const float4* pts;
    const double4* ptsd;
    const int* cell_start;
    const int* cell_own;
    const int* own_start;
    const int2* items;
    int* nbr_pos;
    float* nbr_dist;
    int* nbr_cnt;
    int* redo;
    int* redo_count;
    unsigned long long* counters;
    int n_items, items_q;
    int items_per_xcd;
    int k, pitch;
    int stats;
    unsigned magic_x, magic_xy;
    int shift_x, shift_xy;
    double eps2;
    pct_grid g;
    const int4* tree_seg;
    const int2* tree_runs;
    int tree_bits;
};

constexpr int kPairCap = kStageCap;
static_assert((kPairCap & (kPairCap - 1)) == 0 && kPairCap % 128 == 0 && kPairCap <= 512, "staging capacity of k_knn_pair");
static_assert(PCT_TREE_CAP % 128 == 0 && PCT_TREE_CAP <= 1024, "staging capacity of k_knn_pair on the hierarchical cell list");
template <int CAP>
struct PairLdsT {
    float cx[CAP], cy[CAP], cz[CAP];
    unsigned pend[64 + 4];
    unsigned short pend_b[64 + 8];
    int offc[16];
};
using PairLds = PairLdsT<kPairCap>;

#ifndef PCT_PAIR_WAVES
#define PCT_PAIR_WAVES 1
#endif
constexpr int kPairWaves = PCT_PAIR_WAVES;

template <bool EPS, bool DIST, bool Q64 = false, bool TREE = false>
__global__ __launch_bounds__(64 * kPairWaves, (TREE ? 4 : Q64 ? 5 : 6)) void k_knn_pair(PairArgs a) {
    constexpr int CAP = TREE ? PCT_TREE_CAP : kPairCap, LIST = 64, SLOT_BITS = 6, KEY_BITS = 32 - SLOT_BITS;
    constexpr int SB = TREE ? 10 : 9;
    constexpr unsigned kIdMask = (1u << (SB + 4)) - 1u;
    __shared__ PairLdsT<CAP> s_lds[kPairWaves];
    const int w = kPairWaves == 1 ? 0 : __builtin_amdgcn_readfirstlane(threadIdx.x >> 6);
    const int lane = lane_id();
    const int blk = (int)blockIdx.x * kPairWaves + w;
    const int item = a.items_per_xcd ? (blk & 7) * a.items_per_xcd + (blk >> 3) : blk;
    if (item >= a.n_items || (a.items_per_xcd && (blk >> 3) >= a.items_per_xcd)) return;
    PairLdsT<CAP>& L = s_lds[w];
    const SortLanes sort_dir = make_sort_lanes();
    const int* __restrict__ cs = a.cell_start;

    const int2 it2 = a.items[item];
    constexpr int NRUNS = TREE ? 27 : 9;
    int cx, cy, cz, qs, nq, row0;
    int run_s = 0, run_len = 0;
    pct_grid g_lvl;
    if constexpr (TREE) {
        const int seg = __builtin_amdgcn_readfirstlane(it2.y);
        if (seg < 0) return;
        const unsigned packed = (unsigned)__builtin_amdgcn_readfirstlane(it2.x);
        qs = (int)(packed & 0x3ffffffu);
        nq = (int)(packed >> 26) + 1;
        row0 = qs;
        const int4 hd = a.tree_seg[seg];
        const int level = __builtin_amdgcn_readfirstlane(hd.x);
        cx = __builtin_amdgcn_readfirstlane(hd.y);
        cy = __builtin_amdgcn_readfirstlane(hd.z);
        cz = __builtin_amdgcn_readfirstlane(hd.w);
        g_lvl = a.g;
        g_lvl.cell = __builtin_ldexp(a.g.cell, level);
        g_lvl.inv_cell = __builtin_ldexp(a.g.inv_cell, -level);
        g_lvl.nx = g_lvl.ny = g_lvl.nz = 1 << (a.tree_bits - level);
        if (lane < 27) {
            const int2 r = a.tree_runs[(int64_t)seg * 27 + lane];
            run_s = r.x;
            run_len = r.y;
        }
    } else {
        const int cell = __builtin_amdgcn_readfirstlane(it2.x);
        const int chunk = __builtin_amdgcn_readfirstlane(it2.y);
        const int nx = a.g.nx, ny = a.g.ny, nz = a.g.nz;
        cz = (int)(((unsigned long long)(unsigned)cell * a.magic_xy) >> a.shift_xy);
        const int rem = cell - cz * (nx * ny);
        cy = (int)(((unsigned long long)(unsigned)rem * a.magic_x) >> a.shift_x);
        cx = rem - cy * nx;
        const int c0 = cs[cell];
        qs = c0 + chunk * a.items_q;
        nq = min(c0 + a.cell_own[cell], qs + a.items_q) - qs;
        row0 = a.own_start[cell] + chunk * a.items_q;

        if (lane < 9) {
            const int z = cz + kRowOrder[lane][0], y = cy + kRowOrder[lane][1];
            if (z >= 0 && z < nz && y >= 0 && y < ny) {
                const int row = (z * ny + y) * nx;
                run_s = cs[row + max(cx - 1, 0)];
                run_len = cs[row + min(cx + 1, nx - 1) + 1] - run_s;
            }
        }
    }
    const pct_grid& G = TREE ? g_lvl : a.g;
    float4 my_q = make_float4(0.f, 0.f, 0.f, 0.f);
    double my_qx = 0., my_qy = 0., my_qz = 0.;
    float my_eq = 0.f;
    if (lane < nq) {
        my_q = a.pts[qs + lane];
        if constexpr (Q64) {
            const double4 qd = a.ptsd[qs + lane];
            my_qx = qd.x; my_qy = qd.y; my_qz = qd.z;
        }
    }
    if constexpr (Q64) {
        const double ex = my_qx - (double)my_q.x, ey = my_qy - (double)my_q.y, ez = my_qz - (double)my_q.z;
        my_eq = (float)sqrt((ex * ex + ey * ey) + ez * ez) * (1.0f + 0x1p-22f);
        if (!(my_eq >= 0.f)) my_eq = INFINITY;
    }
    int my_pre = 0, m = 0;
    {
        int acc = 0;
#pragma unroll
        for (int t = 0; t < NRUNS; ++t) {
            my_pre = lane == t ? acc : my_pre;
            acc += __builtin_amdgcn_readlane(run_len, t);
        }
        m = acc;
    }
    const bool crowded = TREE && __popcll(__builtin_amdgcn_ballot_w64(lane < NRUNS && run_len > 0)) > 16;
    if (m > CAP || crowded) {
        int base = 0;
        if (lane == 0) base = atomicAdd(a.redo_count, nq);
        base = __builtin_amdgcn_readfirstlane(base);
        if (lane < nq) a.redo[base + lane] = row0 + lane;
        if (a.stats && lane == 0) {
            atomicAdd(&a.counters[1], 1ull);
            atomicAdd(&a.counters[4], (unsigned long long)nq);
        }
        return;
    }

    unsigned slotx[CAP / 64];
    {
        unsigned* bits = L.pend;
        if (lane < CAP / 32) bits[lane] = 0u;
        wave_lds_sync();
        const bool nonempty = lane < NRUNS && run_len > 0;
        const unsigned long long ne = __builtin_amdgcn_ballot_w64(nonempty);
        if (nonempty) {
            atomicOr(&bits[my_pre >> 5], 1u << (my_pre & 31));
            L.offc[__builtin_amdgcn_mbcnt_lo((unsigned)ne, 0)] = run_s - my_pre;
        }
        wave_lds_sync();
        float4 tmp[CAP / 64];
        int ubase = -1;
#pragma unroll
        for (int b = 0; b < CAP / 64; ++b) {
            tmp[b] = make_float4(0.f, 0.f, 0.f, 0.f);
            slotx[b] = (unsigned)(b * 64 + lane);
            if (b * 64 < m) {
                const unsigned lo = (unsigned)__builtin_amdgcn_readfirstlane((int)bits[2 * b]);
                const unsigned hi = (unsigned)__builtin_amdgcn_readfirstlane((int)bits[2 * b + 1]);
                const unsigned long long B = ((unsigned long long)hi << 32) | lo;
                const unsigned long long S = B >> 1;
                const int s0 = ubase + (int)(lo & 1u);
                const int u = (int)__builtin_amdgcn_mbcnt_hi((unsigned)(S >> 32), __builtin_amdgcn_mbcnt_lo((unsigned)S, (unsigned)s0));
                ubase += (int)__popcll(B);
                const int j = b * 64 + lane;
                slotx[b] |= (unsigned)u << SB;
                if (j < m) tmp[b] = a.pts[j + L.offc[u]];
            }
        }
        wave_lds_sync();
#pragma unroll
        for (int b = 0; b < CAP / 64; ++b) {
            const int j = b * 64 + lane;
            if (j < m) {
                L.cx[j] = tmp[b].x; L.cy[j] = tmp[b].y; L.cz[j] = tmp[b].z;
            } else if ((b & ~1) * 64 < m) {
                L.cx[j] = INFINITY; L.cy[j] = 0.f; L.cz[j] = 0.f;
            }
        }
    }
    wave_lds_sync();

    const int k = a.k;
    const double eps2 = EPS ? a.eps2 : (double)INFINITY;
    constexpr double kKeyRange = 2.3;
    const double edge = G.cell;
    const double scale = (double)(1u << KEY_BITS) / (kKeyRange * edge * edge);
    constexpr unsigned key_max = (1u << KEY_BITS) - 1u;
    unsigned my_gkey;
    {
        const double lqx = Q64 ? my_qx : (double)my_q.x, lqy = Q64 ? my_qy : (double)my_q.y, lqz = Q64 ? my_qz : (double)my_q.z;
        const double gx = (lqx - G.ox) * G.inv_cell - cx;
        const double gy = (lqy - G.oy) * G.inv_cell - cy;
        const double gz = (lqz - G.oz) * G.inv_cell - cz;
        const double g2 = fmin(guaranteed_r2(G, cx, cy, cz, gx, gy, gz, 1), limit_r2(G, cx, cy, cz, gx, gy, gz));
        my_gkey = g2 == INFINITY ? 0xFFFFFFFFu : (unsigned)fmin(g2 * scale, 4294967294.0);
    }
    const unsigned eps_key = EPS && eps2 < 1e300 ? (unsigned)fmin(ceil(eps2 * scale), 4294967295.0) : 0xFFFFFFFFu;
    const float cell2f = (float)(edge * edge);
    const float eps2a = EPS ? (float)fmin(eps2 * (1.0 + 0x1p-18), 3.0e38) : INFINITY;
    const double eps1 = EPS ? sqrt(eps2) * (1.0 + 0x1p-50) : 0.0;
    float t_prev_f = 0.f;
    unsigned long long redo_mask = 0ull;

    char* const pos_item = (char*)(a.nbr_pos + (int64_t)row0 * a.pitch);
    char* const dist_item = DIST ? (char*)(a.nbr_dist + (int64_t)row0 * a.pitch) : nullptr;
    const unsigned lane_off = (unsigned)(lane - 1) * 4u;
    const unsigned pitch4 = (unsigned)a.pitch * 4u;
    const bool col_lane = lane >= 1 && lane <= k;
    const unsigned long long first_k1 = (2ull << k) - 1ull;

    static_assert(CAP <= (1 << SB) && SB + 4 <= 16, "slot ids: SB bits of slot, 4 bits of run index, 16-bit survivor list of query b");
    const auto slot_of = [](unsigned id) { return TREE ? min((int)(id & ((1u << SB) - 1u)), CAP - 1) : (int)(id & (unsigned)(CAP - 1)); };

    const auto pair_loop = [&](auto NBP_) {
        constexpr int NBP = decltype(NBP_)::value, NBU = 2 * NBP;
        for (int qi = 0; qi < nq; qi += 2) {
            const bool live_b = qi + 1 < nq;
            const int qj = live_b ? qi + 1 : qi;
            const float ax = __int_as_float(__builtin_amdgcn_readlane(__float_as_int(my_q.x), qi));
            const float ay = __int_as_float(__builtin_amdgcn_readlane(__float_as_int(my_q.y), qi));
            const float az = __int_as_float(__builtin_amdgcn_readlane(__float_as_int(my_q.z), qi));
            const float bx = __int_as_float(__builtin_amdgcn_readlane(__float_as_int(my_q.x), qj));
            const float by = __int_as_float(__builtin_amdgcn_readlane(__float_as_int(my_q.y), qj));
            const float bz = __int_as_float(__builtin_amdgcn_readlane(__float_as_int(my_q.z), qj));
            const auto rl64 = [&](double v, int l) {
                return __hiloint2double(__builtin_amdgcn_readlane(__double2hiint(v), l), __builtin_amdgcn_readlane(__double2loint(v), l));
            };
            const double qax = Q64 ? rl64(my_qx, qi) : (double)ax, qay = Q64 ? rl64(my_qy, qi) : (double)ay, qaz = Q64 ? rl64(my_qz, qi) : (double)az;
            const double qbx = Q64 ? rl64(my_qx, qj) : (double)bx, qby = Q64 ? rl64(my_qy, qj) : (double)by, qbz = Q64 ? rl64(my_qz, qj) : (double)bz;
            float ap_a[NBU], ap_b[NBU];
#pragma unroll
            for (int p2 = 0; p2 < NBP; ++p2) {
                const int sa = p2 * 128 + lane, sb = sa + 64;
                const float2v vx = {L.cx[sa], L.cx[sb]}, vy = {L.cy[sa], L.cy[sb]}, vz = {L.cz[sa], L.cz[sb]};
                {
                    const float2v dx = vx - ax, dy = vy - ay, dz = vz - az;
                    float2v d = dx * dx;
                    d = __builtin_elementwise_fma(dy, dy, d);
                    d = __builtin_elementwise_fma(dz, dz, d);
                    ap_a[2 * p2] = d.x;
                    ap_a[2 * p2 + 1] = d.y;
                }
                {
                    const float2v dx = vx - bx, dy = vy - by, dz = vz - bz;
                    float2v d = dx * dx;
                    d = __builtin_elementwise_fma(dy, dy, d);
                    d = __builtin_elementwise_fma(dz, dz, d);
                    ap_b[2 * p2] = d.x;
                    ap_b[2 * p2 + 1] = d.y;
                }
            }
            float T_init = eps2a;
            float Ti_a = eps2a, Ti_b = eps2a;
            const float eq_a = Q64 ? __int_as_float(__builtin_amdgcn_readlane(__float_as_int(my_eq), qi)) : 0.f;
            const float eq_b = Q64 ? __int_as_float(__builtin_amdgcn_readlane(__float_as_int(my_eq), qj)) : 0.f;
            const float v_eq = lane == 0 ? eq_a : eq_b;
            if constexpr (EPS && Q64) {
                const double ee = eps1 + (double)v_eq;
                T_init = (float)fmin(ee * ee * (1.0 + 0x1p-18), 3.0e38);
                Ti_a = __int_as_float(__builtin_amdgcn_readlane(__float_as_int(T_init), 0));
                Ti_b = __int_as_float(__builtin_amdgcn_readlane(__float_as_int(T_init), 1));
            }
            int tot_a = m, tot_b = m;
            if constexpr (EPS) {
                tot_a = tot_b = 0;
#pragma unroll
                for (int b = 0; b < NBU; ++b) {
                    tot_a += (int)__popcll(__builtin_amdgcn_ballot_w64(ap_a[b] < Ti_a));
                    tot_b += (int)__popcll(__builtin_amdgcn_ballot_w64(ap_b[b] < Ti_b));
                }
            }
            const bool need_a = tot_a > LIST, need_b = live_b && tot_b > LIST;
            float T_a = Ti_a, T_b = Ti_b;
            int cnt_a = tot_a, cnt_b = tot_b;
            bool ok_a = true, ok_b = live_b;
            unsigned bkey_a = 0xFFFFFFFFu, bkey_b = 0xFFFFFFFFu;
#ifdef PCT_ABL_NO_TRIAL
            T_a = T_b = 0.33f * cell2f; cnt_a = cnt_b = 57;
            if (false)
#endif
            if (need_a || need_b) {
                const float target = 0.5f * (float)(k + 1 + LIST);
                float t0 = t_prev_f > 0.f ? t_prev_f : cell2f;
// ... 66 lines not shown
                        "v_mbcnt_lo_u32_b32 %[rb], s96, 0\n"
                        "v_mbcnt_hi_u32_b32 %[ra], vcc_hi, %[ra]\n"
                        "v_mbcnt_hi_u32_b32 %[rb], s97, %[rb]\n"
                        "v_lshl_add_u32 %[ra], %[ra], 2, %[wra]\n"
                        "v_lshl_add_u32 %[rb], %[rb], 1, %[wrb]\n"
                        "s_mov_b64 exec, vcc\n"
                        "ds_write_b32 %[ra], %[slot]\n"
                        "s_mov_b64 exec, s[96:97]\n"
                        "ds_write_b16 %[rb], %[slot]\n"
                        "s_mov_b64 exec, %[all]\n"
                        "s_lshl2_add_u32 %[wra], %[ca], %[wra]\n"
                        "s_lshl1_add_u32 %[wrb], %[cb], %[wrb]\n"
                        : [ra] "=&v"(ra), [rb] "=&v"(rb), [ca] "=&s"(ca), [cb] "=&s"(cb), [wra] "+s"(wr_a), [wrb] "+s"(wr_b)
                        : [ta] "v"(T_a), [tb] "v"(T_b), [apa] "v"(ap_a[b]), [apb] "v"(ap_b[b]), [slot] "v"(slot), [all] "s"(all)
                        : "vcc", "scc", "s96", "s97", "memory");
                }
#endif
                wave_lds_sync();
            }
            const unsigned sxa = L.pend[lane] & kIdMask, sxb = (unsigned)L.pend_b[lane] & kIdMask;
            const int ja = slot_of(sxa), jb = slot_of(sxb);
            const int out_pa = ja + L.offc[sxa >> SB], out_pb = jb + L.offc[sxb >> SB];
            float out_da = 0.f, out_db = 0.f;
            unsigned e_a, e_b;
#ifdef PCT_ABL_NO_KEYS
            e_a = ((unsigned)ja << 6) | (unsigned)lane; e_b = ((unsigned)jb << 6) | (unsigned)lane;
            if (false)
#endif
            {
                const double dxa = (double)L.cx[ja] - qax, dya = (double)L.cy[ja] - qay, dza = (double)L.cz[ja] - qaz;
                const double dxb = (double)L.cx[jb] - qbx, dyb = (double)L.cy[jb] - qby, dzb = (double)L.cz[jb] - qbz;
                const double d2a = (dxa * dxa + dya * dya) + dza * dza;
                const double d2b = (dxb * dxb + dyb * dyb) + dzb * dzb;
                if constexpr (DIST) {
                    out_da = (float)sqrt(d2a);
                    out_db = (float)sqrt(d2b);
                }
                const unsigned ka = (min((unsigned)(d2a * scale), key_max - 1u) << SLOT_BITS) | (unsigned)lane;
                const unsigned kb = (min((unsigned)(d2b * scale), key_max - 1u) << SLOT_BITS) | (unsigned)lane;
                e_a = lane < cnt_a && (!EPS || d2a < eps2) ? ka : kPadElem;
                e_b = lane < cnt_b && (!EPS || d2b < eps2) ? kb : kPadElem;
            }
            wave_lds_sync();
#ifndef PCT_ABL_NO_SORT
            sort_pair_asm(e_a, e_b, sort_dir);
#endif
            const unsigned tau_a = (unsigned)__builtin_amdgcn_readlane((int)e_a, k);
            const unsigned tau_b = (unsigned)__builtin_amdgcn_readlane((int)e_b, k);
            const unsigned g_a = (unsigned)__builtin_amdgcn_readlane((int)my_gkey, qi);
            const unsigned g_b = (unsigned)__builtin_amdgcn_readlane((int)my_gkey, qj);
            const unsigned tk_a = tau_a >> SLOT_BITS, tk_b = tau_b >> SLOT_BITS;
            const unsigned need_ka = min(tau_a == kPadElem ? 0xFFFFFFFFu : tk_a + 1u, eps_key);
            const unsigned need_kb = min(tau_b == kPadElem ? 0xFFFFFFFFu : tk_b + 1u, eps_key);
            const bool amb_a = need_ka > min(g_a, bkey_a) || (tau_a != kPadElem && tk_a >= key_max - 1u);
            const bool amb_b = need_kb > min(g_b, bkey_b) || (tau_b != kPadElem && tk_b >= key_max - 1u);
#ifndef PCT_ABL_NO_CHECK
            if (ok_a && amb_a) { redo_mask |= 1ull << qi; ok_a = false; }
            if (ok_b && amb_b) { redo_mask |= 1ull << qj; ok_b = false; }
#endif
            {
                unsigned xa, xb;
                asm("v_xor_b32_dpp %0, %2, %2 wave_shl:1 row_mask:0xf bank_mask:0xf bound_ctrl:1\n"
                    "v_xor_b32_dpp %1, %3, %3 wave_shl:1 row_mask:0xf bank_mask:0xf bound_ctrl:1\n"
                    "s_nop 0"
                    : "=&v"(xa), "=&v"(xb) : "v"(e_a), "v"(e_b));
#ifdef PCT_ABL_NO_CHECK
                const unsigned long long cm_any = 0ull;
#else
                const unsigned long long cm_any = __builtin_amdgcn_ballot_w64(min(xa, xb) < 64u) & first_k1;
#endif
                unsigned long long cm_a = 0ull, cm_b = 0ull;
                if (__builtin_expect(cm_any != 0ull, 0)) {
                    cm_a = __builtin_amdgcn_ballot_w64(xa < 64u && e_a != kPadElem) & first_k1;
                    cm_b = __builtin_amdgcn_ballot_w64(xb < 64u && e_b != kPadElem) & first_k1;
                }
                if (__builtin_expect((cm_a | cm_b) != 0ull, 0)) {
                    if (ok_a && cm_a != 0ull) {
                        const double ux = qax, uy = qay, uz = qaz;
                        const bool done = order_equal_keys<1, SLOT_BITS>(&e_a, a.pts,
                            [&](unsigned at) {
                                const int j = slot_of(L.pend[at]);
                                const double dx = (double)L.cx[j] - ux, dy = (double)L.cy[j] - uy, dz = (double)L.cz[j] - uz;
                                return (dx * dx + dy * dy) + dz * dz;
                            },
                            [&](unsigned at) { return __builtin_amdgcn_ds_bpermute((int)(at & 63u) << 2, out_pa); });
                        if (!done) { redo_mask |= 1ull << qi; ok_a = false; }
                    }
                    if (ok_b && cm_b != 0ull) {
                        const double ux = qbx, uy = qby, uz = qbz;
                        const bool done = order_equal_keys<1, SLOT_BITS>(&e_b, a.pts,
                            [&](unsigned at) {
                                const int j = slot_of((unsigned)L.pend_b[at]);
                                const double dx = (double)L.cx[j] - ux, dy = (double)L.cy[j] - uy, dz = (double)L.cz[j] - uz;
                                return (dx * dx + dy * dy) + dz * dz;
                            },
                            [&](unsigned at) { return __builtin_amdgcn_ds_bpermute((int)(at & 63u) << 2, out_pb); });
                        if (!done) { redo_mask |= 1ull << qj; ok_b = false; }
                    }
                }
            }
            {
                const unsigned off_a = lane_off + (unsigned)qi * pitch4, off_b = lane_off + (unsigned)qj * pitch4;
                const bool real_a = e_a != kPadElem, real_b = e_b != kPadElem;
                const int at_a = (int)(e_a << 2), at_b = (int)(e_b << 2);
                const int pos_a = __builtin_amdgcn_ds_bpermute(at_a, out_pa), pos_b = __builtin_amdgcn_ds_bpermute(at_b, out_pb);
                float dist_a = 0.f, dist_b = 0.f;
                if constexpr (DIST) {
                    dist_a = __int_as_float(__builtin_amdgcn_ds_bpermute(at_a, __float_as_int(out_da)));
                    dist_b = __int_as_float(__builtin_amdgcn_ds_bpermute(at_b, __float_as_int(out_db)));
                }
#ifdef PCT_ABL_NO_STORE
                if (pos_a == 0x7fffffff && pos_b == 0x7ffffff1)
#endif
                if (ok_a && col_lane) {
                    *(int*)(pos_item + off_a) = real_a ? pos_a : -1;
                    if constexpr (DIST) *(float*)(dist_item + off_a) = real_a ? dist_a : INFINITY;
                }
#ifdef PCT_ABL_NO_STORE
                if (pos_a == 0x7fffffff && pos_b == 0x7ffffff1)
#endif
                if (ok_b && col_lane) {
                    *(int*)(pos_item + off_b) = real_b ? pos_b : -1;
                    if constexpr (DIST) *(float*)(dist_item + off_b) = real_b ? dist_b : INFINITY;
                }
                if constexpr (EPS) {
                    const int f_a = (int)__popcll(__builtin_amdgcn_ballot_w64(real_a && col_lane));
                    const int f_b = (int)__popcll(__builtin_amdgcn_ballot_w64(real_b && col_lane));
                    if (lane == 0) {
                        if (ok_a) a.nbr_cnt[row0 + qi] = f_a;
                        if (ok_b) a.nbr_cnt[row0 + qj] = f_b;
                    }
                }
            }
        }
    };
    {
        using std::integral_constant;
        const int nbp = (m + 127) >> 7;
        if (nbp <= 1) pair_loop(integral_constant<int, 1>{});
        else if (nbp == 2) pair_loop(integral_constant<int, 2>{});
        else if (nbp == 3) pair_loop(integral_constant<int, (CAP >= 384 ? 3 : 1)>{});
        else if (nbp == 4) pair_loop(integral_constant<int, (CAP >= 512 ? 4 : 1)>{});
        else if (nbp == 5) pair_loop(integral_constant<int, (CAP >= 640 ? 5 : 1)>{});
        else pair_loop(integral_constant<int, (CAP >= 768 ? 6 : 1)>{});
    }
#if defined(PCT_ABL_NO_SORT) || defined(PCT_ABL_NO_COMPACT) || defined(PCT_ABL_NO_KEYS) || defined(PCT_ABL_NO_TRIAL) || defined(PCT_ABL_NO_STORE) || defined(PCT_ABL_NO_CHECK)
    redo_mask = 0ull;
#endif
    if (redo_mask) {
        const int cnt = (int)__popcll(redo_mask);
        int base = 0;
        if (lane == 0) base = atomicAdd(a.redo_count, cnt);
        base = __builtin_amdgcn_readfirstlane(base);
        if ((redo_mask >> lane) & 1ull) a.redo[base + (int)__popcll(redo_mask & ((1ull << lane) - 1ull))] = row0 + lane;
        if (a.stats && lane == 0) atomicAdd(&a.counters[4], (unsigned long long)cnt);
    }
}

#include "pct_sort_duo.inc"

__device__ __forceinline__ void sort_duo_asm(unsigned& ea, unsigned& eb, const SortLanes& c) {
    unsigned ta, tb;
    asm volatile(PCT_SORT_DUO_ASM
                 : [ea] "+v"(ea), [eb] "+v"(eb), [ta] "=&v"(ta), [tb] "=&v"(tb)
                 : [sel0] "v"(c.sel[0]), [sel1] "v"(c.sel[1]), [sel2] "v"(c.sel[2]), [sel3] "v"(c.sel[3]), [sel4] "v"(c.sel[4]),
                   [sel5] "v"(c.sel[5]), [a31] "v"(c.a31), [a63] "v"(c.a63));
    const unsigned lo = PCT_SORT_DUO_RESULT_A, hi = PCT_SORT_DUO_RESULT_B;
    ea = lo;
    eb = hi;
}

#ifndef PCT_DUO_CAP
#define PCT_DUO_CAP 768
#endif
constexpr int kDuoCap = PCT_DUO_CAP;
template <bool DIST, int CAP>
struct DuoLds {
    float cx[CAP], cy[CAP], cz[CAP];
    unsigned short pend[128 + 8];
    int pay_p[128];
    float pay_d[DIST ? 128 : 1];
    int offc[16];
};

template <bool EPS, bool DIST, bool Q64 = false, bool TREE = false>
__global__ __launch_bounds__(64, ((TREE ? PCT_TREE_CAP2 : PCT_DUO_CAP) <= 768 ? 4 : 3)) void k_knn_duo(PairArgs a) {
    constexpr int CAP = TREE ? PCT_TREE_CAP2 : kDuoCap, LIST = 128, SLOT_BITS = 7, KEY_BITS = 32 - SLOT_BITS;
    static_assert(CAP % 128 == 0 && CAP <= 1024, "slot ids: 10 bits of slot, 4 bits of run index");
    __shared__ DuoLds<DIST, CAP> L;
    const int lane = lane_id();
    const int item = a.items_per_xcd ? ((int)blockIdx.x & 7) * a.items_per_xcd + ((int)blockIdx.x >> 3) : (int)blockIdx.x;
    if (item >= a.n_items) return;
    const SortLanes sort_dir = make_sort_lanes();
    const int* __restrict__ cs = a.cell_start;

    const int2 it2 = a.items[item];
    constexpr int NRUNS = TREE ? 27 : 9;
    int cx, cy, cz, qs, nq, row0;
    int run_s = 0, run_len = 0;
    pct_grid g_lvl;
    if constexpr (TREE) {
        const int seg = __builtin_amdgcn_readfirstlane(it2.y);
        if (seg < 0) return;
        const unsigned packed = (unsigned)__builtin_amdgcn_readfirstlane(it2.x);
        qs = (int)(packed & 0x3ffffffu);
        nq = (int)(packed >> 26) + 1;
        row0 = qs;
        const int4 hd = a.tree_seg[seg];
        const int level = __builtin_amdgcn_readfirstlane(hd.x);
        cx = __builtin_amdgcn_readfirstlane(hd.y);
        cy = __builtin_amdgcn_readfirstlane(hd.z);
        cz = __builtin_amdgcn_readfirstlane(hd.w);
        g_lvl = a.g;
        g_lvl.cell = __builtin_ldexp(a.g.cell, level);
        g_lvl.inv_cell = __builtin_ldexp(a.g.inv_cell, -level);
        g_lvl.nx = g_lvl.ny = g_lvl.nz = 1 << (a.tree_bits - level);
        if (lane < 27) {
            const int2 r = a.tree_runs[(int64_t)seg * 27 + lane];
            run_s = r.x;
            run_len = r.y;
        }
    } else {
        const int cell = __builtin_amdgcn_readfirstlane(it2.x);
        const int chunk = __builtin_amdgcn_readfirstlane(it2.y);
        const int nx = a.g.nx, ny = a.g.ny, nz = a.g.nz;
        cz = (int)(((unsigned long long)(unsigned)cell * a.magic_xy) >> a.shift_xy);
        const int rem = cell - cz * (nx * ny);
        cy = (int)(((unsigned long long)(unsigned)rem * a.magic_x) >> a.shift_x);
        cx = rem - cy * nx;
        const int c0 = cs[cell];
        qs = c0 + chunk * a.items_q;
        nq = min(c0 + a.cell_own[cell], qs + a.items_q) - qs;
        row0 = a.own_start[cell] + chunk * a.items_q;
        if (lane < 9) {
            const int z = cz + kRowOrder[lane][0], y = cy + kRowOrder[lane][1];
            if (z >= 0 && z < nz && y >= 0 && y < ny) {
                const int row = (z * ny + y) * nx;
                run_s = cs[row + max(cx - 1, 0)];
                run_len = cs[row + min(cx + 1, nx - 1) + 1] - run_s;
            }
        }
    }
    const pct_grid& G = TREE ? g_lvl : a.g;
    float4 my_q = make_float4(0.f, 0.f, 0.f, 0.f);
    double my_qx = 0., my_qy = 0., my_qz = 0.;
    float my_eq = 0.f;
    if (lane < nq) {
        my_q = a.pts[qs + lane];
        if constexpr (Q64) {
            const double4 qd = a.ptsd[qs + lane];
            my_qx = qd.x; my_qy = qd.y; my_qz = qd.z;
        }
    }
    if constexpr (Q64) {
        const double ex = my_qx - (double)my_q.x, ey = my_qy - (double)my_q.y, ez = my_qz - (double)my_q.z;
        my_eq = (float)sqrt((ex * ex + ey * ey) + ez * ez) * (1.0f + 0x1p-22f);
        if (!(my_eq >= 0.f)) my_eq = INFINITY;
    }
    int my_pre = 0, m = 0;
    {
        int acc = 0;
#pragma unroll
        for (int t = 0; t < NRUNS; ++t) {
            my_pre = lane == t ? acc : my_pre;
            acc += __builtin_amdgcn_readlane(run_len, t);
        }
        m = acc;
    }
    const bool crowded = TREE && __popcll(__builtin_amdgcn_ballot_w64(lane < NRUNS && run_len > 0)) > 16;
    if (m > CAP || crowded) {
        int base = 0;
        if (lane == 0) base = atomicAdd(a.redo_count, nq);
        base = __builtin_amdgcn_readfirstlane(base);
        if (lane < nq) a.redo[base + lane] = row0 + lane;
        if (a.stats && lane == 0) {
            atomicAdd(&a.counters[1], 1ull);
            atomicAdd(&a.counters[4], (unsigned long long)nq);
        }
        return;
    }
    unsigned slotx[CAP / 64];
    {
        unsigned* bits = (unsigned*)L.pend;
        static_assert(sizeof(L.pend) >= CAP / 8, "the run-start bit string lives in the survivor list");
        if (lane < CAP / 32) bits[lane] = 0u;
        wave_lds_sync();
        const bool nonempty = lane < NRUNS && run_len > 0;
        const unsigned long long ne = __builtin_amdgcn_ballot_w64(nonempty);
        if (nonempty) {
            atomicOr(&bits[my_pre >> 5], 1u << (my_pre & 31));
            L.offc[__builtin_amdgcn_mbcnt_lo((unsigned)ne, 0)] = run_s - my_pre;
        }
        wave_lds_sync();
        float4 tmp[CAP / 64];
        int ubase = -1;
#pragma unroll
        for (int b = 0; b < CAP / 64; ++b) {
            tmp[b] = make_float4(0.f, 0.f, 0.f, 0.f);
            slotx[b] = (unsigned)(b * 64 + lane);
            if (b * 64 < m) {
                const unsigned lo = (unsigned)__builtin_amdgcn_readfirstlane((int)bits[2 * b]);
                const unsigned hi = (unsigned)__builtin_amdgcn_readfirstlane((int)bits[2 * b + 1]);
                const unsigned long long B = ((unsigned long long)hi << 32) | lo;
                const unsigned long long S = B >> 1;
                const int s0 = ubase + (int)(lo & 1u);
                const int u = (int)__builtin_amdgcn_mbcnt_hi((unsigned)(S >> 32), __builtin_amdgcn_mbcnt_lo((unsigned)S, (unsigned)s0));
                ubase += (int)__popcll(B);
                const int j = b * 64 + lane;
                slotx[b] |= (unsigned)u << 10;
                if (j < m) tmp[b] = a.pts[j + L.offc[u]];
            }
        }
        wave_lds_sync();
#pragma unroll
        for (int b = 0; b < CAP / 64; ++b) {
            const int j = b * 64 + lane;
            if (j < m) {
                L.cx[j] = tmp[b].x; L.cy[j] = tmp[b].y; L.cz[j] = tmp[b].z;
            } else if ((b & ~1) * 64 < m) {
                L.cx[j] = INFINITY; L.cy[j] = 0.f; L.cz[j] = 0.f;
            }
        }
    }
    wave_lds_sync();

    const int k = a.k;
    const double eps2 = EPS ? a.eps2 : (double)INFINITY;
    constexpr double kKeyRange = 2.3;
    const double edge = G.cell;
    const double scale = (double)(1u << KEY_BITS) / (kKeyRange * edge * edge);
    constexpr unsigned key_max = (1u << KEY_BITS) - 1u;
    unsigned my_gkey;
    {
        const double lqx = Q64 ? my_qx : (double)my_q.x, lqy = Q64 ? my_qy : (double)my_q.y, lqz = Q64 ? my_qz : (double)my_q.z;
        const double gx = (lqx - G.ox) * G.inv_cell - cx;
        const double gy = (lqy - G.oy) * G.inv_cell - cy;
        const double gz = (lqz - G.oz) * G.inv_cell - cz;
        const double g2 = fmin(guaranteed_r2(G, cx, cy, cz, gx, gy, gz, 1), limit_r2(G, cx, cy, cz, gx, gy, gz));
        my_gkey = g2 == INFINITY ? 0xFFFFFFFFu : (unsigned)fmin(g2 * scale, 4294967294.0);
    }
    const unsigned eps_key = EPS && eps2 < 1e300 ? (unsigned)fmin(ceil(eps2 * scale), 4294967295.0) : 0xFFFFFFFFu;
    const float cell2f = (float)(edge * edge);
    const float eps2a = EPS ? (float)fmin(eps2 * (1.0 + 0x1p-18), 3.0e38) : INFINITY;
    const double eps1 = EPS ? sqrt(eps2) * (1.0 + 0x1p-50) : 0.0;
    float t_prev_f = 0.f;
    unsigned long long redo_mask = 0ull;

    char* const pos_item = (char*)(a.nbr_pos + (int64_t)row0 * a.pitch);
    char* const dist_item = DIST ? (char*)(a.nbr_dist + (int64_t)row0 * a.pitch) : nullptr;
    const unsigned pitch4 = (unsigned)a.pitch * 4u;
    const unsigned lane_off0 = (unsigned)(lane - 1) * 4u, lane_off1 = (unsigned)(lane + 63) * 4u;
    const bool col0 = lane >= 1 && lane <= k, col1 = lane + 64 <= k;
    const unsigned long long order_lo = k >= 63 ? ~0ull : (2ull << k) - 1ull;
    const unsigned long long order_hi = k < 64 ? 0ull : k - 64 >= 63 ? ~0ull : (2ull << (k - 64)) - 1ull;
    const unsigned short* pend_hi = &L.pend[64];

    const auto query_loop = [&](auto NBP_) {
        constexpr int NBP = decltype(NBP_)::value, NBU = 2 * NBP;
        for (int qi = 0; qi < nq; ++qi) {
            const float ax = __int_as_float(__builtin_amdgcn_readlane(__float_as_int(my_q.x), qi));
            const float ay = __int_as_float(__builtin_amdgcn_readlane(__float_as_int(my_q.y), qi));
            const float az = __int_as_float(__builtin_amdgcn_readlane(__float_as_int(my_q.z), qi));
            const auto rl64 = [&](double v, int l) {
                return __hiloint2double(__builtin_amdgcn_readlane(__double2hiint(v), l), __builtin_amdgcn_readlane(__double2loint(v), l));
            };
            const double qx = Q64 ? rl64(my_qx, qi) : (double)ax, qy = Q64 ? rl64(my_qy, qi) : (double)ay, qz = Q64 ? rl64(my_qz, qi) : (double)az;
            const float eq = Q64 ? __int_as_float(__builtin_amdgcn_readlane(__float_as_int(my_eq), qi)) : 0.f;
            float ap[NBU];
#pragma unroll
            for (int p2 = 0; p2 < NBP; ++p2) {
                const int sa = p2 * 128 + lane, sb = sa + 64;
                const float2v vx = {L.cx[sa], L.cx[sb]}, vy = {L.cy[sa], L.cy[sb]}, vz = {L.cz[sa], L.cz[sb]};
                const float2v dx = vx - ax, dy = vy - ay, dz = vz - az;
                float2v d = dx * dx;
                d = __builtin_elementwise_fma(dy, dy, d);
                d = __builtin_elementwise_fma(dz, dz, d);
                ap[2 * p2] = d.x;
                ap[2 * p2 + 1] = d.y;
            }
            float T_init = eps2a;
            if constexpr (EPS && Q64) {
                const double ee = eps1 + (double)eq;
                T_init = (float)fmin(ee * ee * (1.0 + 0x1p-18), 3.0e38);
            }
            int tot = m;
            if constexpr (EPS) {
                tot = 0;
#pragma unroll
                for (int b = 0; b < NBU; ++b) tot += (int)__popcll(__builtin_amdgcn_ballot_w64(ap[b] < T_init));
            }
            const bool need = tot > LIST;
            float T = T_init;
            int cnt = tot;
            unsigned bkey = 0xFFFFFFFFu;
            if (need) {
                const float target = 0.5f * (float)(k + 1 + LIST);
                float t = t_prev_f > 0.f ? t_prev_f : cell2f;
                if (!(t < T_init)) t = 0.5f * T_init;
                float lo = 0.f, hi = T_init;
                bool found = false;
#pragma unroll 1
                for (int trial = 0; trial < 16; ++trial) {
                    int c = 0;
#pragma unroll
                    for (int b = 0; b < NBU; ++b) c += (int)__popcll(__builtin_amdgcn_ballot_w64(ap[b] < t));
                    if ((unsigned)(c - (k + 1)) <= (unsigned)(LIST - (k + 1))) { T = t; cnt = c; found = true; break; }
                    const bool below = c < k + 1;
                    lo = below ? t : lo;
                    hi = below ? hi : t;
                    float nt = t * target * __builtin_amdgcn_rcpf((float)c);
                    if (!(nt > lo && nt < hi)) nt = hi < INFINITY ? 0.5f * (lo + hi) : 2.f * lo;
                    if (__builtin_amdgcn_ballot_w64(!(nt > lo && nt < hi)) != 0ull) break;
                    t = nt;
                }
                if (!found || __builtin_amdgcn_ballot_w64(!(T >= 1e-30f)) != 0ull) { redo_mask |= 1ull << qi; continue; }
                t_prev_f = T;
                double lo2 = (double)T * (1.0 - 0x1p-20);
                if constexpr (Q64) {
                    const double root_up = (double)__builtin_sqrtf(T) * (1.0 + 0x1p-21);
                    lo2 = fmax(lo2 - 2.0 * (double)eq * root_up, 0.0);
                }
                bkey = (unsigned)fmin(lo2 * scale, 4294967294.0);
            }
            {
                unsigned wr = (unsigned)(uintptr_t)&L.pend[0], wr1;
                const unsigned long long all = __builtin_amdgcn_read_exec();
                wave_lds_sync();
#pragma unroll
                for (int b = 0; b < NBU; b += 2) {
                    unsigned r0, r1, n0, n1;
                    asm volatile(
                        "v_cmp_gt_f32 vcc, %[t], %[ap0]\n"
                        "v_cmp_gt_f32 s[96:97], %[t], %[ap1]\n"
                        "s_bcnt1_i32_b64 %[n0], vcc\n"
                        "v_mbcnt_lo_u32_b32 %[r0], vcc_lo, 0\n"
                        "s_bcnt1_i32_b64 %[n1], s[96:97]\n"
                        "v_mbcnt_lo_u32_b32 %[r1], s96, 0\n"
                        "v_mbcnt_hi_u32_b32 %[r0], vcc_hi, %[r0]\n"
                        "v_mbcnt_hi_u32_b32 %[r1], s97, %[r1]\n"
                        "s_lshl1_add_u32 %[wr1], %[n0], %[wr]\n"
                        "v_lshl_add_u32 %[r0], %[r0], 1, %[wr]\n"
                        "v_lshl_add_u32 %[r1], %[r1], 1, %[wr1]\n"
                        "s_mov_b64 exec, vcc\n"
                        "ds_write_b16 %[r0], %[slot0]\n"
                        "s_mov_b64 exec, s[96:97]\n"
                        "ds_write_b16 %[r1], %[slot1]\n"
                        "s_mov_b64 exec, %[all]\n"
                        "s_lshl1_add_u32 %[wr], %[n1], %[wr1]\n"
                        : [r0] "=&v"(r0), [r1] "=&v"(r1), [n0] "=&s"(n0), [n1] "=&s"(n1), [wr] "+s"(wr), [wr1] "=&s"(wr1)
                        : [t] "v"(T), [ap0] "v"(ap[b]), [ap1] "v"(ap[b + 1]), [slot0] "v"(slotx[b]), [slot1] "v"(slotx[b + 1]), [all] "s"(all)
                        : "vcc", "scc", "s96", "s97", "memory");
                }
                wave_lds_sync();
            }
            const unsigned sx0 = (unsigned)L.pend[lane] & 0x3FFFu, sx1 = (unsigned)pend_hi[lane] & 0x3FFFu;
            const int j0 = min((int)(sx0 & 1023u), CAP - 1), j1 = min((int)(sx1 & 1023u), CAP - 1);
            unsigned e[2];
            {
                const double dx0 = (double)L.cx[j0] - qx, dy0 = (double)L.cy[j0] - qy, dz0 = (double)L.cz[j0] - qz;
                const double dx1 = (double)L.cx[j1] - qx, dy1 = (double)L.cy[j1] - qy, dz1 = (double)L.cz[j1] - qz;
                const double d20 = (dx0 * dx0 + dy0 * dy0) + dz0 * dz0;
                const double d21 = (dx1 * dx1 + dy1 * dy1) + dz1 * dz1;
                L.pay_p[lane] = j0 + L.offc[sx0 >> 10];
                L.pay_p[lane + 64] = j1 + L.offc[sx1 >> 10];
                if constexpr (DIST) {
                    L.pay_d[lane] = (float)sqrt(d20);
                    L.pay_d[lane + 64] = (float)sqrt(d21);
                }
                const unsigned k0 = (min((unsigned)(d20 * scale), key_max - 1u) << SLOT_BITS) | (unsigned)lane;
                const unsigned k1 = (min((unsigned)(d21 * scale), key_max - 1u) << SLOT_BITS) | (unsigned)(lane + 64);
                e[0] = lane < cnt && (!EPS || d20 < eps2) ? k0 : kPadElem;
                e[1] = lane + 64 < cnt && (!EPS || d21 < eps2) ? k1 : kPadElem;
            }
            wave_lds_sync();
            sort_duo_asm(e[0], e[1], sort_dir);
            const unsigned tau = (unsigned)__builtin_amdgcn_readlane((int)(k < 64 ? e[0] : e[1]), k & 63);
            const unsigned gk = (unsigned)__builtin_amdgcn_readlane((int)my_gkey, qi);
            const unsigned tk = tau >> SLOT_BITS;
            const unsigned need_k = min(tau == kPadElem ? 0xFFFFFFFFu : tk + 1u, eps_key);
            if (need_k > min(gk, bkey) || (tau != kPadElem && tk >= key_max - 1u)) { redo_mask |= 1ull << qi; continue; }
            {
                unsigned n0, n1;
                asm("s_nop 1\n"
                    "v_mov_b32_dpp %0, %2 wave_shl:1 row_mask:0xf bank_mask:0xf bound_ctrl:1\n"
                    "v_mov_b32_dpp %1, %3 wave_shl:1 row_mask:0xf bank_mask:0xf bound_ctrl:1\n"
                    "s_nop 0"
                    : "=&v"(n0), "=&v"(n1) : "v"(e[0]), "v"(e[1]));
                n0 = lane == 63 ? (unsigned)__builtin_amdgcn_readlane((int)e[1], 0) : n0;
                const bool same0 = ((e[0] ^ n0) >> SLOT_BITS) == 0u && e[0] != kPadElem && n0 != kPadElem;
                const bool same1 = ((e[1] ^ n1) >> SLOT_BITS) == 0u && e[1] != kPadElem && n1 != kPadElem && lane < 63;
                const unsigned long long cm = (__builtin_amdgcn_ballot_w64(same0) & order_lo) | (__builtin_amdgcn_ballot_w64(same1) & order_hi);
                if (__builtin_expect(cm != 0ull, 0)) {
                    const bool done = order_equal_keys<2, SLOT_BITS>(e, a.pts,
                        [&](unsigned at) {
                            const int j = min((int)L.pend[at] & 1023, CAP - 1);
                            const double dx = (double)L.cx[j] - qx, dy = (double)L.cy[j] - qy, dz = (double)L.cz[j] - qz;
                            return (dx * dx + dy * dy) + dz * dz;
                        },
                        [&](unsigned at) { return L.pay_p[at]; });
                    if (!done) { redo_mask |= 1ull << qi; continue; }
                }
            }
            {
                const unsigned off0 = lane_off0 + (unsigned)qi * pitch4, off1 = lane_off1 + (unsigned)qi * pitch4;
                const bool real0 = e[0] != kPadElem, real1 = e[1] != kPadElem;
                const int s0 = (int)(e[0] & 127u), s1 = (int)(e[1] & 127u);
                const int pos0 = L.pay_p[s0], pos1 = L.pay_p[s1];
                if (col0) *(int*)(pos_item + off0) = real0 ? pos0 : -1;
                if (col1) *(int*)(pos_item + off1) = real1 ? pos1 : -1;
                if constexpr (DIST) {
                    const float d0 = L.pay_d[s0], d1 = L.pay_d[s1];
                    if (col0) *(float*)(dist_item + off0) = real0 ? d0 : INFINITY;
                    if (col1) *(float*)(dist_item + off1) = real1 ? d1 : INFINITY;
                }
                if constexpr (EPS) {
                    const int f = (int)__popcll(__builtin_amdgcn_ballot_w64(real0 && col0)) + (int)__popcll(__builtin_amdgcn_ballot_w64(real1 && col1));
                    if (lane == 0) a.nbr_cnt[row0 + qi] = f;
                }
            }
            wave_lds_sync();
        }
    };
    {
        using std::integral_constant;
        const int nbp = (m + 127) >> 7;
        if (nbp <= 1) query_loop(integral_constant<int, 1>{});
        else if (nbp == 2) query_loop(integral_constant<int, 2>{});
        else if (nbp == 3) query_loop(integral_constant<int, 3>{});
        else if (nbp == 4) query_loop(integral_constant<int, 4>{});
        else if (nbp == 5) query_loop(integral_constant<int, 5>{});
        else if (nbp == 6) query_loop(integral_constant<int, 6>{});
        else if (nbp == 7) query_loop(integral_constant<int, (CAP >= 896 ? 7 : 1)>{});
        else query_loop(integral_constant<int, (CAP >= 1024 ? 8 : 1)>{});
    }
    if (redo_mask) {
        const int cnt = (int)__popcll(redo_mask);
        int base = 0;
        if (lane == 0) base = atomicAdd(a.redo_count, cnt);
        base = __builtin_amdgcn_readfirstlane(base);
        if ((redo_mask >> lane) & 1ull) a.redo[base + (int)__popcll(redo_mask & ((1ull << lane) - 1ull))] = row0 + lane;
        if (a.stats && lane == 0) atomicAdd(&a.counters[4], (unsigned long long)cnt);
    }
}

__global__ __launch_bounds__(256) void k_plain_records(const float* __restrict__ xyz, int64_t n, float4* __restrict__ out) {
    const int64_t i = (int64_t)blockIdx.x * 256 + threadIdx.x;
    if (i < n) out[i] = make_float4(xyz[3 * i], xyz[3 * i + 1], xyz[3 * i + 2], __int_as_float((int)i));
}

template <int R>
__global__ __launch_bounds__(64 * kWavesPerBlock) void k_query_points(const float4* __restrict__ pts, int n, const double* __restrict__ q_xyz,
                                                                      int64_t m, int k, double eps2, int* __restrict__ idx_out,
                                                                      double* __restrict__ dist_out) {
    __shared__ double s_pend_d[kWavesPerBlock][64 * R + 64];
    __shared__ int s_pend_p[kWavesPerBlock][64 * R + 64];
    const int w = __builtin_amdgcn_readfirstlane(threadIdx.x >> 6);
    const int lane = lane_id();
    const int64_t q = (int64_t)blockIdx.x * kWavesPerBlock + w;
    if (q >= m) return;
    Sweep<R> sw;
    sw.k = k - 1;
    sw.eps2 = eps2;
    sw.pts = pts;
    sw.pend_d = s_pend_d[w];
    sw.pend_p = s_pend_p[w];
    sw.qx = q_xyz[3 * q]; sw.qy = q_xyz[3 * q + 1]; sw.qz = q_xyz[3 * q + 2];
    sw.reset();
    for (int base = 0;; base += 64) {
        const bool have = base < n;
        if (have) {
            const int pos = base + lane;
            const bool valid = pos < n;
            float4 c = make_float4(0.f, 0.f, 0.f, 0.f);
            if (valid) c = pts[pos];
            sw.consider(c, pos, valid);
            if (sw.npend < 64 * R) continue;
        }
        if (sw.npend > 0 || sw.empty) sw.flush();
        if (!have) break;
    }
#pragma unroll
    for (int r = 0; r < R; ++r) {
        const int i = lane + 64 * r;
        if (i < k) {
            const bool real = sw.best.p[r] != INT_MAX;
            idx_out[q * k + i] = real ? sw.best.p[r] : n;
            dist_out[q * k + i] = real ? sqrt(sw.best.d[r]) : (double)INFINITY;
        }
    }
}

__device__ __forceinline__ float table_distance(const float4* pts, const double4* ptsd, int qpos, const float4 c) {
    double qx, qy, qz;
    if (ptsd) { const double4 q = ptsd[qpos]; qx = q.x; qy = q.y; qz = q.z; }
    else { const float4 q = pts[qpos]; qx = (double)q.x; qy = (double)q.y; qz = (double)q.z; }
    const double dx = (double)c.x - qx, dy = (double)c.y - qy, dz = (double)c.z - qz;
    return (float)sqrt((dx * dx + dy * dy) + dz * dz);
}

__global__ __launch_bounds__(256) void k_export(const float4* __restrict__ pts, const double4* __restrict__ ptsd, const int* __restrict__ owned_pos, int q_begin,
                                                const int* __restrict__ nbr_pos, const float* __restrict__ nbr_dist,
                                                const int* __restrict__ nbr_cnt, int64_t n, int64_t n_rows, int k, int pitch,
                                                int64_t begin, int64_t end, int* __restrict__ idx_out,
                                                float* __restrict__ dist_out, int* __restrict__ cnt_out) {
    const int64_t t = (int64_t)blockIdx.x * 256 + threadIdx.x;
    const int64_t row = t / k;
    const int j = (int)(t - row * k);
    if (row >= n_rows) return;
    const int pub = owned_pos ? __float_as_int(pts[owned_pos[row]].w) : (int)row + q_begin;
    if (pub < begin || pub >= end) return;
    const int64_t o = (int64_t)(pub - begin) * k + j;
    const int pos = nbr_pos[row * pitch + j];
    const float4 c = pos < 0 ? make_float4(0.f, 0.f, 0.f, 0.f) : pts[pos];
    if (idx_out) idx_out[o] = pos < 0 ? (int)n : __float_as_int(c.w);
    if (dist_out) dist_out[o] = nbr_dist ? nbr_dist[row * pitch + j] : pos < 0 ? INFINITY : table_distance(pts, ptsd, owned_pos[row], c);
    if (cnt_out && j == 0) cnt_out[pub - begin] = nbr_cnt ? nbr_cnt[row] : k;
}

__global__ __launch_bounds__(128) void k_export_rows(const float4* __restrict__ pts, const double4* __restrict__ ptsd, const int* __restrict__ row_of, const int* __restrict__ owned_pos, int q_begin,
                                                     const int* __restrict__ nbr_pos, const float* __restrict__ nbr_dist,
                                                     const int* __restrict__ nbr_cnt, int64_t n, int k, int pitch,
                                                     const int64_t* __restrict__ rows, int* __restrict__ idx_out,
                                                     float* __restrict__ dist_out, int* __restrict__ cnt_out) {
    const int64_t r = blockIdx.x;
    const int64_t pub = rows[r];
    const int64_t row = row_of ? row_of[pub - q_begin] : pub - q_begin;
    for (int j = threadIdx.x; j < k; j += 128) {
        const int pos = nbr_pos[row * pitch + j];
        const float4 c = pos < 0 ? make_float4(0.f, 0.f, 0.f, 0.f) : pts[pos];
        if (idx_out) idx_out[r * k + j] = pos < 0 ? (int)n : __float_as_int(c.w);
        if (dist_out) dist_out[r * k + j] = nbr_dist ? nbr_dist[row * pitch + j] : pos < 0 ? INFINITY : table_distance(pts, ptsd, owned_pos[row], c);
    }
    if (cnt_out && threadIdx.x == 0) cnt_out[r] = nbr_cnt ? nbr_cnt[row] : k;
}

__global__ __launch_bounds__(64) void k_selftest(int* fails) {
    const int lane = lane_id();
    const int v = lane * 7919 + 13;
    int bad = 0;
    bad += lane_xor<1>(v) != __shfl_xor(v, 1);
    bad += lane_xor<2>(v) != __shfl_xor(v, 2);
    bad += lane_xor<4>(v) != __shfl_xor(v, 4);
    bad += lane_xor<8>(v) != __shfl_xor(v, 8);
    bad += lane_xor<16>(v) != __shfl_xor(v, 16);
    bad += lane_xor<32>(v) != __shfl_xor(v, 32);
    if (bad) atomicAdd(fails, bad);
}

__global__ __launch_bounds__(256) void k_item_census(const int2* __restrict__ items, int64_t n_items, int items_q,
                                                     const int* __restrict__ cs, const int* __restrict__ cell_own, pct_grid g, int k,
                                                     int cap, unsigned long long* __restrict__ out) {
    __shared__ unsigned long long sh[4][4];
    unsigned long long v[4] = {0, 0, 0, 0};
    for (int64_t it = (int64_t)blockIdx.x * 256 + threadIdx.x; it < n_items; it += (int64_t)gridDim.x * 256) {
        const int2 e = items[it];
        const int cell = e.x;
        const int cx = cell % g.nx, cy = (cell / g.nx) % g.ny, cz = cell / (g.nx * g.ny);
        const int nq = min(items_q, cell_own[cell] - e.y * items_q);
        int m = 0, occupied = 0;
        for (int dz = -1; dz <= 1; ++dz)
            for (int dy = -1; dy <= 1; ++dy) {
                const int z = cz + dz, y = cy + dy;
                if (z < 0 || z >= g.nz || y < 0 || y >= g.ny) continue;
                const int row = (z * g.ny + y) * g.nx;
                int prev = cs[row + max(cx - 1, 0)];
                for (int x = max(cx - 1, 0); x <= min(cx + 1, g.nx - 1); ++x) {
                    const int next = cs[row + x + 1];
                    occupied += next > prev;
                    m += next - prev;
                    prev = next;
                }
            }
        v[0] += (unsigned)nq;
        if (m > cap) v[1] += (unsigned)nq;
        else if (2 * m < 5 * (k + 1)) v[2] += (unsigned)nq;
        else v[3] += (unsigned long long)nq * (unsigned)occupied;
    }
    for (int j = 0; j < 4; ++j) {
        for (int o = 32; o > 0; o >>= 1) v[j] += __shfl_xor(v[j], o);
        if ((threadIdx.x & 63) == 0) sh[threadIdx.x >> 6][j] = v[j];
    }
    __syncthreads();
    if (threadIdx.x < 4) atomicAdd(&out[threadIdx.x], sh[0][threadIdx.x] + sh[1][threadIdx.x] + sh[2][threadIdx.x] + sh[3][threadIdx.x]);
}

KnnArgs make_args(pct_ctx* ctx, int32_t k, double eps, bool grid) {
    KnnArgs a = {};
    a.pts = (const float4*)(grid ? ctx->sorted4.p : ctx->pts4.p);
    a.ptsd = ctx->has_f64 ? (const double4*)(grid ? ctx->sorted4d.p : ctx->pts4d.p) : nullptr;
    a.cell_start = (const int*)ctx->cell_cnt.p;
    a.cell_own = (const int*)ctx->cell_own.p;
    a.own_start = (const int*)ctx->own_start.p;
    a.owned_pos = (const int*)ctx->owned_pos.p;
    a.n_owned = ctx->own_flag ? ctx->own_count : ctx->q_end - ctx->q_begin;
    a.occ = (const int*)ctx->occ.p;
    a.n_occ = ctx->n_occ;
    a.n = ctx->n;
    a.g = ctx->grid;
    a.k = k;
    a.pitch = (k + 3) & ~3;
    a.eps2 = eps > 0 ? eps * eps : INFINITY;
    a.q_begin = (int)ctx->q_begin;
    a.q_end = (int)ctx->q_end;
    a.nbr_pos = (int*)ctx->nbr_pos.p;
    a.nbr_dist = (float*)ctx->nbr_dist.p;
    a.nbr_cnt = eps > 0 ? (int*)ctx->nbr_cnt.p : nullptr;
    a.row_done = ctx->own_flag || ctx->level_mode ? (int*)ctx->row_done.p : nullptr;
    a.redo_m = a.row_done ? (int*)ctx->redo_m.p : nullptr;
    a.counters = (unsigned long long*)ctx->counters.p;
    a.stats = ctx->collect_stats ? 1 : 0;
    return a;
}

int reserve_table(pct_ctx* ctx, int32_t k, double eps, bool with_dist = true) {
    ctx->nbr_pitch = (k + 3) & ~3;
    const size_t rows = (size_t)(ctx->own_flag ? ctx->own_count : ctx->q_end - ctx->q_begin);
    PCT_TRY(pct_reserve(ctx, &ctx->nbr_pos, rows * ctx->nbr_pitch * sizeof(int)));
    if (with_dist) PCT_TRY(pct_reserve(ctx, &ctx->nbr_dist, rows * ctx->nbr_pitch * sizeof(float)));
    ctx->dist_valid = with_dist;
    if (eps > 0) PCT_TRY(pct_reserve(ctx, &ctx->nbr_cnt, rows * sizeof(int)));
    PCT_TRY(pct_reserve(ctx, &ctx->counters, 64 * sizeof(unsigned long long)));
    if (!ctx->counters_clean) PCT_HIP(ctx, hipMemsetAsync(ctx->counters.p, 0, 64, ctx->stream));
    ctx->counters_clean = false;
    return PCT_OK;
}

}

int pct_launch_knn_grid(pct_ctx* ctx, int32_t k, double eps, bool exact_only, int phase) {
    const int64_t n_rows = ctx->own_flag ? ctx->own_count : ctx->q_end - ctx->q_begin;
    const double c2_ = ctx->grid.cell * ctx->grid.cell;
    const bool f32_ok_ = c2_ > 1e-30 && c2_ < 1e30 && (!(eps > 0) || eps * eps > 1e-36);
    const pct_grid& gg_ = ctx->grid;
    const double far_ = fmax(fmax(fabs(gg_.ox), fabs(gg_.ox + gg_.nx * gg_.cell)),
                             fmax(fmax(fabs(gg_.oy), fabs(gg_.oy + gg_.ny * gg_.cell)), fmax(fabs(gg_.oz), fabs(gg_.oz + gg_.nz * gg_.cell))));
    const bool q64_ok_ = !ctx->has_f64 || far_ * 0x1p-23 < gg_.cell * 0x1p-7;
    const bool pair_kernel = !exact_only && phase == 0 && q64_ok_ && f32_ok_ && !ctx->own_flag && !ctx->level_mode && ctx->n_items > 0 &&
                             k + 1 <= pct_fast_r1_max() && ctx->n_items < ((int64_t)1 << 31) - 8 && !pct_getenv("PCT_NO_PAIR") &&
                             !pct_getenv("PCT_NO_PAIR_KERNEL");
    const bool duo_kernel = !exact_only && phase == 0 && q64_ok_ && f32_ok_ && !ctx->own_flag && !ctx->level_mode && ctx->n_items > 0 &&
                            k + 1 > pct_fast_r1_max() && k + 1 <= 128 && ctx->n_items < ((int64_t)1 << 31) - 8 &&
                            !pct_getenv("PCT_NO_PAIR") && !pct_getenv("PCT_NO_DUO_KERNEL");
    const bool skip_dist = (pair_kernel || duo_kernel) && ctx->skip_dist_req && !pct_getenv("PCT_KEEP_DIST");
    if (phase != 2) {
        PCT_TRY(reserve_table(ctx, k, eps, !skip_dist));
        PCT_TRY(pct_reserve(ctx, &ctx->redo, ((size_t)n_rows + 16) * sizeof(int)));
        if (ctx->level_mode) PCT_TRY(pct_reserve(ctx, &ctx->redo_m, ((size_t)n_rows + 16) * sizeof(int)));
    }
    KnnArgs a = make_args(ctx, k, eps, true);
    if (!ctx->dist_valid) a.nbr_dist = nullptr;
    int* redo_count = (int*)ctx->counters.p + 14;
    int* redo = (int*)ctx->redo.p;
    const dim3 block(64 * kWavesPerBlock);
    if (!exact_only && phase != 2 && ctx->n_items > 0) {
        const dim3 grid1((unsigned)((ctx->n_items + kFastWaves<1> - 1) / kFastWaves<1>)), block1(64 * kFastWaves<1>);
        const dim3 grid2((unsigned)((ctx->n_items + kFastWaves<2> - 1) / kFastWaves<2>)), block2(64 * kFastWaves<2>);
        const int2* items = (const int2*)ctx->occ.p;
        const double c2 = ctx->grid.cell * ctx->grid.cell;
        const bool f32_ok = c2 > 1e-30 && c2 < 1e30 && (!(eps > 0) || eps * eps > 1e-36);
        const pct_grid& gg = ctx->grid;
        const double far = fmax(fmax(fabs(gg.ox), fabs(gg.ox + gg.nx * gg.cell)),
                                fmax(fmax(fabs(gg.oy), fabs(gg.oy + gg.ny * gg.cell)), fmax(fabs(gg.oz), fabs(gg.oz + gg.nz * gg.cell))));
        const bool q64_ok = ctx->has_f64 && f32_ok && far * 0x1p-23 < gg.cell * 0x1p-7 && !ctx->level_mode;
        const bool e = eps > 0, pre = !ctx->has_f64 && f32_ok, r1 = k + 1 <= pct_fast_r1_max();
#define PCT_FAST(R_, E_, P_, GRID_, BLOCK_) \
    PCT_LAUNCH((k_knn_fast<R_, E_, P_>), GRID_, BLOCK_, 0, ctx->stream, a, items, ctx->n_items, ctx->items_q, redo, redo_count)
        const bool no_pair = pct_getenv("PCT_NO_PAIR") != nullptr;
#define PCT_FAST_PAIR(R_, E_, GRID_, BLOCK_) \
    PCT_LAUNCH((k_knn_fast<R_, E_, true, true>), GRID_, BLOCK_, 0, ctx->stream, a, items, ctx->n_items, ctx->items_q, redo, redo_count)
#define PCT_FAST_PAIR64(R_, E_, GRID_, BLOCK_) \
    PCT_LAUNCH((k_knn_fast<R_, E_, true, true, true>), GRID_, BLOCK_, 0, ctx->stream, a, items, ctx->n_items, ctx->items_q, redo, redo_count)
        if (pair_kernel || duo_kernel) {
            PairArgs pa = {};
            pa.pts = a.pts; pa.ptsd = a.ptsd; pa.cell_start = a.cell_start; pa.cell_own = a.cell_own; pa.own_start = a.own_start;
            pa.items = items;
            pa.nbr_pos = a.nbr_pos; pa.nbr_dist = a.nbr_dist; pa.nbr_cnt = a.nbr_cnt;
            pa.redo = redo; pa.redo_count = redo_count; pa.counters = a.counters;
            pa.n_items = (int)ctx->n_items; pa.items_q = ctx->items_q;
            pa.k = a.k; pa.pitch = a.pitch; pa.stats = a.stats; pa.eps2 = a.eps2; pa.g = a.g;
            const auto magic = [](unsigned d, unsigned* mg, int* sh) {
                int l = 0;
                while ((1ull << l) < d) ++l;
                *sh = 30 + l;
                *mg = (unsigned)(((1ull << *sh) + d - 1) / d);
            };
            magic((unsigned)a.g.nx, &pa.magic_x, &pa.shift_x);
            magic((unsigned)a.g.nx * (unsigned)a.g.ny, &pa.magic_xy, &pa.shift_xy);
            pa.items_per_xcd = (int)((ctx->n_items + 7) / 8);
            if (pct_getenv("PCT_NO_XCD_MAP")) pa.items_per_xcd = 0;
            const int64_t n_blk = pa.items_per_xcd ? (int64_t)pa.items_per_xcd * 8 : ctx->n_items;
            const dim3 gridp((unsigned)((n_blk + kPairWaves - 1) / kPairWaves)), blockp(64 * kPairWaves);
            if (duo_kernel) {
                const dim3 gridd((unsigned)n_blk), blockd(64);
                if (ctx->has_f64) {
                    if (e && skip_dist) PCT_LAUNCH((k_knn_duo<true, false, true>), gridd, blockd, 0, ctx->stream, pa);
                    else if (e) PCT_LAUNCH((k_knn_duo<true, true, true>), gridd, blockd, 0, ctx->stream, pa);
                    else if (skip_dist) PCT_LAUNCH((k_knn_duo<false, false, true>), gridd, blockd, 0, ctx->stream, pa);
                    else PCT_LAUNCH((k_knn_duo<false, true, true>), gridd, blockd, 0, ctx->stream, pa);
                } else
                if (e && skip_dist) PCT_LAUNCH((k_knn_duo<true, false>), gridd, blockd, 0, ctx->stream, pa);
                else if (e) PCT_LAUNCH((k_knn_duo<true, true>), gridd, blockd, 0, ctx->stream, pa);
                else if (skip_dist) PCT_LAUNCH((k_knn_duo<false, false>), gridd, blockd, 0, ctx->stream, pa);
                else PCT_LAUNCH((k_knn_duo<false, true>), gridd, blockd, 0, ctx->stream, pa);
            } else
            if (ctx->has_f64) {
                if (e && skip_dist) PCT_LAUNCH((k_knn_pair<true, false, true>), gridp, blockp, 0, ctx->stream, pa);
                else if (e) PCT_LAUNCH((k_knn_pair<true, true, true>), gridp, blockp, 0, ctx->stream, pa);
                else if (skip_dist) PCT_LAUNCH((k_knn_pair<false, false, true>), gridp, blockp, 0, ctx->stream, pa);
                else PCT_LAUNCH((k_knn_pair<false, true, true>), gridp, blockp, 0, ctx->stream, pa);
            } else
            if (e && skip_dist) PCT_LAUNCH((k_knn_pair<true, false>), gridp, blockp, 0, ctx->stream, pa);
            else if (e) PCT_LAUNCH((k_knn_pair<true, true>), gridp, blockp, 0, ctx->stream, pa);
            else if (skip_dist) PCT_LAUNCH((k_knn_pair<false, false>), gridp, blockp, 0, ctx->stream, pa);
            else PCT_LAUNCH((k_knn_pair<false, true>), gridp, blockp, 0, ctx->stream, pa);
        } else
        if (q64_ok && !no_pair) {
            if (r1 && !e) PCT_FAST_PAIR64(1, false, grid1, block1);
            else if (r1) PCT_FAST_PAIR64(1, true, grid1, block1);
            else if (!e) PCT_FAST_PAIR64(2, false, grid2, block2);
            else PCT_FAST_PAIR64(2, true, grid2, block2);
        } else
        if (r1 && !e && pre && !no_pair) PCT_FAST_PAIR(1, false, grid1, block1);
        else if (r1 && e && pre && !no_pair) PCT_FAST_PAIR(1, true, grid1, block1);
        else if (!r1 && !e && pre && !no_pair) PCT_FAST_PAIR(2, false, grid2, block2);
        else if (!r1 && e && pre && !no_pair) PCT_FAST_PAIR(2, true, grid2, block2);
        else if (r1 && !e && pre) PCT_FAST(1, false, true, grid1, block1);
        else if (r1 && e && pre) PCT_FAST(1, true, true, grid1, block1);
        else if (r1 && !e) PCT_FAST(1, false, false, grid1, block1);
        else if (r1) PCT_FAST(1, true, false, grid1, block1);
        else if (!e && pre) PCT_FAST(2, false, true, grid2, block2);
        else if (e && pre) PCT_FAST(2, true, true, grid2, block2);
        else if (!e) PCT_FAST(2, false, false, grid2, block2);
        else PCT_FAST(2, true, false, grid2, block2);
#undef PCT_FAST
#undef PCT_FAST_PAIR
#undef PCT_FAST_PAIR64
        PCT_HIP(ctx, hipGetLastError());
    }
    PCT_HIP(ctx, hipEventRecord(ctx->ev[7], ctx->stream));
    if (phase != 1) {
        const int64_t waves = exact_only ? n_rows : 32768;
        const int blocks = (int)((waves + kWavesPerBlock - 1) / kWavesPerBlock);
        const int* list = exact_only ? nullptr : redo;
        if (k + 1 <= 64)
            PCT_LAUNCH(k_knn_exact<1>, dim3(blocks), block, 0, ctx->stream, a, list, (const int*)redo_count);
        else if (k + 1 <= 128)
            PCT_LAUNCH(k_knn_exact<2>, dim3(blocks), block, 0, ctx->stream, a, list, (const int*)redo_count);
        else
            PCT_TRY(pct_launch_knn_exact_wide(ctx, a, blocks, list, (const int*)redo_count));
        PCT_HIP(ctx, hipGetLastError());
    }
    ctx->knn_sorted_space = true;
    return PCT_OK;
}

int pct_launch_knn_tree(pct_ctx* ctx, int32_t k, double eps) {
    if (ctx->level_mode || ctx->own_flag || ctx->q_begin != 0 || ctx->q_end != ctx->n)
        return pct_fail(ctx, PCT_ERR_INVALID, "the tree sweep takes whole clouds");
    const int64_t n_rows = ctx->n;
    const bool lean_ok = ctx->n_items > 0 && ctx->n_items < ((int64_t)1 << 31) - 8 && !pct_getenv("PCT_NO_PAIR") &&
                         !pct_getenv("PCT_TREE_EXACT_ONLY");
    const bool pair_tree = lean_ok && k + 1 <= pct_fast_r1_max() && !pct_getenv("PCT_NO_PAIR_KERNEL");
    const bool duo_tree = lean_ok && k + 1 > pct_fast_r1_max() && k + 1 <= 128 && !pct_getenv("PCT_NO_DUO_KERNEL");
    const bool skip_dist = (pair_tree || duo_tree) && ctx->skip_dist_req && !pct_getenv("PCT_KEEP_DIST");
    PCT_TRY(reserve_table(ctx, k, eps, !skip_dist));
    PCT_TRY(pct_reserve(ctx, &ctx->redo, ((size_t)n_rows + 16) * sizeof(int)));
    KnnArgs a = make_args(ctx, k, eps, true);
    if (!ctx->dist_valid) a.nbr_dist = nullptr;
    a.tree_seg = (const int4*)ctx->tree_seg.p;
    a.tree_runs = (const int2*)ctx->tree_runs.p;
    a.tree_bits = ctx->tree_bits;
    a.tree_codes = (const unsigned long long*)ctx->tree_codes.p + ctx->n;
    a.tree_lvl = (const unsigned char*)ctx->tree_lvl.p;
    a.tree_bucket = (const int*)ctx->tree_bucket.p;
    int* redo_count = (int*)ctx->counters.p + 14;
    int* redo = (int*)ctx->redo.p;
    const int2* items = (const int2*)ctx->occ.p;
    const bool r1 = k + 1 <= pct_fast_r1_max();
    const bool exact_only = pct_getenv("PCT_TREE_EXACT_ONLY") != nullptr;
    if (ctx->n_items > 0 && !exact_only) {
        const dim3 grid1((unsigned)((ctx->n_items + kFastWaves<1> - 1) / kFastWaves<1>)), block1(64 * kFastWaves<1>);
        const dim3 grid2((unsigned)((ctx->n_items + kFastWaves<2> - 1) / kFastWaves<2>)), block2(64 * kFastWaves<2>);
        const bool e = eps > 0;
#define PCT_TREE(R_, E_, Q_, GRID_, BLOCK_) \
    PCT_LAUNCH((k_knn_fast<R_, E_, true, true, Q_, true>), GRID_, BLOCK_, 0, ctx->stream, a, items, ctx->n_items, ctx->items_q, redo, redo_count)
        if (pair_tree || duo_tree) {
            PairArgs pa = {};
            pa.pts = a.pts; pa.ptsd = a.ptsd; pa.cell_start = a.cell_start;
            pa.items = items;
            pa.nbr_pos = a.nbr_pos; pa.nbr_dist = a.nbr_dist; pa.nbr_cnt = a.nbr_cnt;
            pa.redo = redo; pa.redo_count = redo_count; pa.counters = a.counters;
            pa.n_items = (int)ctx->n_items; pa.items_q = ctx->items_q;
            pa.k = a.k; pa.pitch = a.pitch; pa.stats = a.stats; pa.eps2 = a.eps2; pa.g = a.g;
            pa.tree_seg = a.tree_seg; pa.tree_runs = a.tree_runs; pa.tree_bits = a.tree_bits;
            pa.items_per_xcd = pct_getenv("PCT_NO_XCD_MAP") ? 0 : (int)((ctx->n_items + 7) / 8);
            const int64_t n_blk = pa.items_per_xcd ? (int64_t)pa.items_per_xcd * 8 : ctx->n_items;
            const dim3 gridp((unsigned)((n_blk + kPairWaves - 1) / kPairWaves)), blockp(64 * kPairWaves);
#define PCT_PAIR_TREE(E_, D_, Q_)                                                                       \
    do {                                                                                                \
        if (duo_tree) PCT_LAUNCH((k_knn_duo<E_, D_, Q_, true>), dim3((unsigned)n_blk), dim3(64), 0, ctx->stream, pa); \
        else PCT_LAUNCH((k_knn_pair<E_, D_, Q_, true>), gridp, blockp, 0, ctx->stream, pa);           \
    } while (0)
            if (ctx->has_f64) {
                if (e && skip_dist) PCT_PAIR_TREE(true, false, true);
                else if (e) PCT_PAIR_TREE(true, true, true);
                else if (skip_dist) PCT_PAIR_TREE(false, false, true);
                else PCT_PAIR_TREE(false, true, true);
            } else if (e && skip_dist) PCT_PAIR_TREE(true, false, false);
            else if (e) PCT_PAIR_TREE(true, true, false);
            else if (skip_dist) PCT_PAIR_TREE(false, false, false);
            else PCT_PAIR_TREE(false, true, false);
#undef PCT_PAIR_TREE
        } else
        if (ctx->has_f64) {
            if (r1 && !e) PCT_TREE(1, false, true, grid1, block1);
            else if (r1) PCT_TREE(1, true, true, grid1, block1);
            else if (!e) PCT_TREE(2, false, true, grid2, block2);
            else PCT_TREE(2, true, true, grid2, block2);
        } else if (r1 && !e) PCT_TREE(1, false, false, grid1, block1);
        else if (r1) PCT_TREE(1, true, false, grid1, block1);
        else if (!e) PCT_TREE(2, false, false, grid2, block2);
        else PCT_TREE(2, true, false, grid2, block2);
#undef PCT_TREE
        PCT_HIP(ctx, hipGetLastError());
    }
    PCT_HIP(ctx, hipEventRecord(ctx->ev[7], ctx->stream));
    const int blocks = (32768 + kWavesPerBlock - 1) / kWavesPerBlock;
    const int* list = exact_only ? nullptr : redo;
    if (k + 1 <= 64)
        PCT_LAUNCH(k_knn_exact_tree<1>, dim3(blocks), dim3(64 * kWavesPerBlock), 0, ctx->stream, a, list, (const int*)redo_count);
    else
        PCT_LAUNCH(k_knn_exact_tree<2>, dim3(blocks), dim3(64 * kWavesPerBlock), 0, ctx->stream, a, list, (const int*)redo_count);
    PCT_HIP(ctx, hipGetLastError());
    ctx->knn_sorted_space = true;
    return PCT_OK;
}

int pct_item_census(pct_ctx* ctx, int32_t k, unsigned long long out4[4]) {
    PCT_TRY(pct_reserve(ctx, &ctx->counters, 64 * sizeof(unsigned long long)));
    PCT_HIP(ctx, hipMemsetAsync(ctx->counters.p, 0, 64, ctx->stream));
    ctx->counters_clean = false;
    const int cap = k + 1 <= pct_fast_r1_max() ? kStageCap : PCT_STAGE_CAP2_HOST;
    const int blocks = (int)((ctx->n_items + 255) / 256 < 1024 ? (ctx->n_items + 255) / 256 : 1024);
    if (blocks > 0) {
        PCT_LAUNCH(k_item_census, dim3(blocks), dim3(256), 0, ctx->stream, (const int2*)ctx->occ.p, ctx->n_items, ctx->items_q,
                           (const int*)ctx->cell_cnt.p, (const int*)ctx->cell_own.p, ctx->grid, k, cap, (unsigned long long*)ctx->counters.p);
        PCT_HIP(ctx, hipGetLastError());
    }
    PCT_HIP(ctx, hipMemcpyAsync(ctx->pin + 2112, ctx->counters.p, 32, hipMemcpyDeviceToHost, ctx->stream));
    PCT_HIP(ctx, hipStreamSynchronize(ctx->stream));
    memcpy(out4, ctx->pin + 2112, 32);
    return PCT_OK;
}

int pct_launch_knn_brute(pct_ctx* ctx, int32_t k, double eps) {
    PCT_TRY(reserve_table(ctx, k, eps));
    KnnArgs a = make_args(ctx, k, eps, false);
    const int64_t nq = ctx->q_end - ctx->q_begin;
    const int blocks = (int)((nq + kWavesPerBlock - 1) / kWavesPerBlock);
    if (blocks > 0) {
        if (k + 1 <= 64)
            PCT_LAUNCH(k_knn_brute<1>, dim3(blocks), dim3(64 * kWavesPerBlock), 0, ctx->stream, a);
        else if (k + 1 <= 128)
            PCT_LAUNCH(k_knn_brute<2>, dim3(blocks), dim3(64 * kWavesPerBlock), 0, ctx->stream, a);
        else
            PCT_TRY(pct_launch_knn_brute_wide(ctx, a, blocks));
        PCT_HIP(ctx, hipGetLastError());
    }
    ctx->knn_sorted_space = false;
    return PCT_OK;
}

int pct_launch_export_neighbors(pct_ctx* ctx, int64_t begin, int64_t end, int32_t* d_idx, float* d_dist,
                                int32_t* d_cnt) {
    const bool sorted = ctx->knn_sorted_space;
    const int64_t n_rows = ctx->q_end - ctx->q_begin;
    const int64_t total = n_rows * ctx->k;
    const int blocks = (int)((total + 255) / 256);
    PCT_LAUNCH(k_export, dim3(blocks), dim3(256), 0, ctx->stream,
                       (const float4*)(sorted ? ctx->sorted4.p : ctx->pts4.p), sorted && ctx->has_f64 ? (const double4*)ctx->sorted4d.p : nullptr,
                       sorted ? (const int*)ctx->owned_pos.p : nullptr,
                       (int)ctx->q_begin, (const int*)ctx->nbr_pos.p, ctx->dist_valid ? (const float*)ctx->nbr_dist.p : nullptr,
                       ctx->eps > 0 ? (const int*)ctx->nbr_cnt.p : nullptr, ctx->n, n_rows, ctx->k, ctx->nbr_pitch, begin, end,
                       d_idx, d_dist, d_cnt);
    PCT_HIP(ctx, hipGetLastError());
    return PCT_OK;
}

int pct_launch_export_rows(pct_ctx* ctx, const int64_t* d_rows, int64_t n_rows, int32_t* d_idx, float* d_dist, int32_t* d_cnt) {
    const bool sorted = ctx->knn_sorted_space;
    if (sorted) PCT_TRY(pct_ensure_row_of(ctx));
    PCT_LAUNCH(k_export_rows, dim3((unsigned)n_rows), dim3(128), 0, ctx->stream,
                       (const float4*)(sorted ? ctx->sorted4.p : ctx->pts4.p), sorted && ctx->has_f64 ? (const double4*)ctx->sorted4d.p : nullptr,
                       sorted ? (const int*)ctx->row_of.p : nullptr,
                       sorted ? (const int*)ctx->owned_pos.p : nullptr,
                       (int)ctx->q_begin, (const int*)ctx->nbr_pos.p, ctx->dist_valid ? (const float*)ctx->nbr_dist.p : nullptr,
                       ctx->eps > 0 ? (const int*)ctx->nbr_cnt.p : nullptr, ctx->n, ctx->k, ctx->nbr_pitch, d_rows, d_idx,
                       d_dist, d_cnt);
    PCT_HIP(ctx, hipGetLastError());
    return PCT_OK;
// ... 33 lines not shown
```

### point-cloud-toolbox_amd/csrc/pct_knn_sweep.h

```cpp
#pragma once
#include "pct_internal.h"

#include <math.h>
#include <type_traits>

struct KnnArgs {
    const float4* pts;
    const double4* ptsd;
    const int* cell_start;
    const int* cell_own;
    const int* own_start;
    const int* owned_pos;
    int64_t n_owned;
    const int* occ;
    int64_t n_occ;
    int64_t n;
    pct_grid g;
    int k;
    int pitch;
    double eps2;
    int q_begin, q_end;
    int* nbr_pos;
    float* nbr_dist;
    int* nbr_cnt;
    int* row_done;
    int* redo_m;
    const int4* tree_seg;
    const int2* tree_runs;
    int tree_bits;
    const unsigned long long* tree_codes;
    const unsigned char* tree_lvl;
    const int* tree_bucket;
    int stats;
    unsigned long long* counters;
};

int pct_launch_knn_exact_wide(pct_ctx* ctx, const KnnArgs& a, int blocks, const int* list, const int* list_count);
int pct_launch_knn_brute_wide(pct_ctx* ctx, const KnnArgs& a, int blocks);

namespace {

constexpr int kWavesPerBlock = 4;
#ifndef PCT_STAGE_CAP
#define PCT_STAGE_CAP 512
#endif
constexpr int kStageCap = PCT_STAGE_CAP;
#ifndef PCT_STAGE_CAP2
#define PCT_STAGE_CAP2 768
#endif
constexpr int PCT_STAGE_CAP2_HOST = PCT_STAGE_CAP2;
#ifndef PCT_TREE_CAP
#define PCT_TREE_CAP 768
#endif
#ifndef PCT_TREE_CAP2
#define PCT_TREE_CAP2 1024
#endif


__device__ __forceinline__ int lane_id() { return threadIdx.x & 63; }

__device__ __forceinline__ void wave_lds_sync() {
    __builtin_amdgcn_fence(__ATOMIC_RELEASE, "wavefront");
    __builtin_amdgcn_wave_barrier();
    __builtin_amdgcn_fence(__ATOMIC_ACQUIRE, "wavefront");
}

template <int S>
__device__ __forceinline__ int lane_xor(int v) {
    if constexpr (S == 1) {
        return __builtin_amdgcn_mov_dpp(v, 0xB1, 0xF, 0xF, true);
    } else if constexpr (S == 2) {
        return __builtin_amdgcn_mov_dpp(v, 0x4E, 0xF, 0xF, true);
    } else if constexpr (S == 4) {
        int t = __builtin_amdgcn_update_dpp(v, v, 0x124, 0xF, 0xA, false);
        return __builtin_amdgcn_update_dpp(t, v, 0x12C, 0xF, 0x5, false);
    } else if constexpr (S == 8) {
        return __builtin_amdgcn_mov_dpp(v, 0x128, 0xF, 0xF, true);
    } else if constexpr (S == 16) {
        const auto r = __builtin_amdgcn_permlane16_swap((unsigned)v, (unsigned)v, false, false);
        return (int)((threadIdx.x & 16) ? r[0] : r[1]);
    } else {
        const auto r = __builtin_amdgcn_permlane32_swap((unsigned)v, (unsigned)v, false, false);
        return (int)((threadIdx.x & 32) ? r[0] : r[1]);
    }
}

__device__ __forceinline__ int pub_index(const float4* pts, int pos) { return __float_as_int(pts[pos].w); }

__device__ __forceinline__ bool key_less(double da, int pa, double db, int pb, const float4* pts) {
    const bool lt = da < db;
    bool tie = (da == db) && (pa != pb) && (pa != INT_MAX) && (pb != INT_MAX);
    bool tb = false;
    if (__builtin_expect(__ballot(tie) != 0ull, 0)) {
        if (tie) tb = pub_index(pts, pa) < pub_index(pts, pb);
    }
    return lt || (tie && tb);
}

template <int R>
struct TopK {
    double d[R];
    int p[R];
};

template <int R, int STRIDE>
__device__ __forceinline__ void bitonic_level(TopK<R>& t, int size, bool descending, const float4* pts) {
    const int lane = lane_id();
    if constexpr (STRIDE >= 64) {
        constexpr int ds = STRIDE >> 6;
#pragma unroll
        for (int r = 0; r < R; ++r) {
            if ((r & ds) == 0 && (r | ds) < R) {
                const int r2 = r | ds;
                const int i = lane + 64 * r;
                const bool asc = ((i & size) == 0) != descending;
                const bool hi_less = key_less(t.d[r2], t.p[r2], t.d[r], t.p[r], pts);
                if (hi_less == asc) {
                    double td = t.d[r]; t.d[r] = t.d[r2]; t.d[r2] = td;
                    int tp = t.p[r]; t.p[r] = t.p[r2]; t.p[r2] = tp;
                }
            }
        }
    } else {
#pragma unroll
        for (int r = 0; r < R; ++r) {
            const int lo = lane_xor<STRIDE>(__double2loint(t.d[r]));
            const int hi = lane_xor<STRIDE>(__double2hiint(t.d[r]));
            const int pp = lane_xor<STRIDE>(t.p[r]);
            const double pd = __hiloint2double(hi, lo);
            const int i = lane + 64 * r;
            const bool asc = ((i & size) == 0) != descending;
            const bool keep_min = ((lane & STRIDE) == 0) == asc;
            const bool partner_less = key_less(pd, pp, t.d[r], t.p[r], pts);
            if (keep_min == partner_less) {
                t.d[r] = pd;
                t.p[r] = pp;
            }
        }
    }
}

template <int R, int STRIDE>
__device__ __forceinline__ void bitonic_strides(TopK<R>& t, int size, bool descending, const float4* pts) {
    bitonic_level<R, STRIDE>(t, size, descending, pts);
    if constexpr (STRIDE > 1) bitonic_strides<R, STRIDE / 2>(t, size, descending, pts);
}

template <int R, int SIZE>
__device__ __forceinline__ void bitonic_sort_from(TopK<R>& t, bool descending, const float4* pts) {
    bitonic_strides<R, SIZE / 2>(t, SIZE, descending, pts);
    if constexpr (SIZE < 64 * R) bitonic_sort_from<R, SIZE * 2>(t, descending, pts);
}

template <int R>
__device__ __forceinline__ void bitonic_merge_min(TopK<R>& best, const TopK<R>& batch, const float4* pts) {
#pragma unroll
    for (int r = 0; r < R; ++r) {
        if (key_less(batch.d[r], batch.p[r], best.d[r], best.p[r], pts)) {
            best.d[r] = batch.d[r];
            best.p[r] = batch.p[r];
        }
    }
    bitonic_strides<R, 32 * R>(best, 64 * R, false, pts);
}

template <int R>
struct Sweep {
    TopK<R> best;
    double tau_d;
    int tau_p;
    int npend;
    bool empty;
    double qx, qy, qz;
    double eps2;
    int k;
    const float4* pts;
    double* pend_d;
    int* pend_p;

    __device__ __forceinline__ void reset() {
#pragma unroll
        for (int r = 0; r < R; ++r) {
            best.d[r] = INFINITY;
            best.p[r] = INT_MAX;
        }
        tau_d = INFINITY;
        tau_p = INT_MAX;
// ... 382 lines not shown
```

Before: 1.404 billion.

## Overlap exact k-NN redo tail and its fit on a side stream with main fit

The fast k-NN sweep now marks rows that need an exact redo in a per-row flag array. The exact redo kernel runs on a second stream. Meanwhile the main fit kernel processes all unflagged rows on the primary stream, and a persistent listed-fit kernel on the side stream fits only the redo rows once they finish. This hides the serial tail of exact k-NN behind the bulk fit. In exchange it adds flag writes, an extra stream and event synchronisation, and a flag-clearing pass inside the SVD fallback kernel.

```diff
diff --git a/point-cloud-toolbox_amd/csrc/pct_api.hip b/point-cloud-toolbox_amd/csrc/pct_api.hip
--- a/point-cloud-toolbox_amd/csrc/pct_api.hip
+++ b/point-cloud-toolbox_amd/csrc/pct_api.hip
@@ -48,6 +48,7 @@
     if (b->cap >= bytes) return PCT_OK;
     if (b->p) {
         PCT_HIP(ctx, hipStreamSynchronize(ctx->stream));
+        if (ctx->tail_fork) PCT_HIP(ctx, hipStreamSynchronize(ctx->side));
         pct_release(b);
     }
     size_t want = bytes + bytes / 8 + 256;
@@ -62,6 +63,15 @@
 }
 
 static void release(pct_buf* b) { pct_release(b); }
+
+void pct_tail_abandon(pct_ctx* ctx) {
+    if (!ctx->tail_fork) return;
+    ctx->tail_fork = false;
+    (void)hipStreamSynchronize(ctx->side);
+    (void)hipStreamSynchronize(ctx->stream);
+    if (ctx->row_flag.p) (void)hipMemsetAsync(ctx->row_flag.p, 0, ctx->row_flag.cap, ctx->stream);
+    (void)hipGetLastError();
+}
 
 static float ev_ms(const hipEvent_t* ev, int a, int b) {
     float ms = 0.f;
@@ -178,18 +188,23 @@
         delete ctx;
         return PCT_ERR_HIP;
     }
+    if (hipStreamCreateWithFlags(&ctx->side, hipStreamNonBlocking) != hipSuccess ||
+        hipEventCreateWithFlags(&ctx->ev_tail, hipEventDisableTiming) != hipSuccess) {
+        pct_destroy(ctx);
+        return PCT_ERR_HIP;
+    }
     for (auto& e : ctx->ev)
         if (hipEventCreate(&e) != hipSuccess) {
-            delete ctx;
+            pct_destroy(ctx);
             return PCT_ERR_HIP;
         }
     for (int i = 2; i <= 7; ++i)
         if (hipEventCreate(&ctx->ev_prev[i]) != hipSuccess) {
-            delete ctx;
+            pct_destroy(ctx);
             return PCT_ERR_HIP;
         }
     if (hipHostMalloc((void**)&ctx->pin, 4096, hipHostMallocMapped) != hipSuccess) {
-        delete ctx;
+        pct_destroy(ctx);
         return PCT_ERR_OOM;
     }
     memset(ctx->pin, 0, 4096);
@@ -200,10 +215,11 @@
 void pct_destroy(pct_ctx* ctx) {
     if (!ctx) return;
     (void)hipSetDevice(ctx->device);
+    if (ctx->side) (void)hipStreamSynchronize(ctx->side);
     if (ctx->stream) (void)hipStreamSynchronize(ctx->stream);
     pct_comm_release(ctx);
     pct_buf* all[] = {&ctx->xyz, &ctx->pts4, &ctx->pts4d, &ctx->cell_of, &ctx->cell_cnt, &ctx->cell_fill,
-                      &ctx->scan_tmp, &ctx->occ, &ctx->redo, &ctx->row_of, &ctx->owned_pos, &ctx->cell_own, &ctx->cell_oth, &ctx->own_start, &ctx->sorted4, &ctx->sorted4d, &ctx->red, &ctx->nbr_pos,
+                      &ctx->scan_tmp, &ctx->occ, &ctx->redo, &ctx->row_flag, &ctx->row_of, &ctx->owned_pos, &ctx->cell_own, &ctx->cell_oth, &ctx->own_start, &ctx->sorted4, &ctx->sorted4d, &ctx->red, &ctx->nbr_pos,
                       &ctx->nbr_dist, &ctx->nbr_cnt, &ctx->counters, &ctx->coefs, &ctx->K, &ctx->H, &ctx->H2,
                       &ctx->stage_a, &ctx->stage_b, &ctx->stage_c, &ctx->stage_d, &ctx->row_done, &ctx->redo_m, &ctx->flag_buf, &ctx->dens_buf, &ctx->pub_pos, &ctx->pub_dist, &ctx->pub_cnt, &ctx->qpts4, &ctx->fit_flag, &ctx->lvl_src,
                       &ctx->tree_codes, &ctx->tree_vals, &ctx->tree_lvl, &ctx->tree_head, &ctx->tree_marks, &ctx->tree_seg, &ctx->tree_runs, &ctx->tree_range, &ctx->tree_bucket, &ctx->tree_tmp,
@@ -215,6 +231,8 @@
         if (e) (void)hipEventDestroy(e);
     for (auto& e : ctx->ev_prev)
         if (e) (void)hipEventDestroy(e);
+    if (ctx->ev_tail) (void)hipEventDestroy(ctx->ev_tail);
+    if (ctx->side) (void)hipStreamDestroy(ctx->side);
     if (ctx->stream) (void)hipStreamDestroy(ctx->stream);
     delete ctx;
 }
@@ -225,6 +243,7 @@
     if (!ctx) return PCT_ERR_INVALID;
     ctx->err[0] = 0;
     PCT_HIP(ctx, hipSetDevice(ctx->device));
+    pct_tail_abandon(ctx);
     if (wait_for_pending) PCT_TRY(drain(ctx));
     return PCT_OK;
 }
diff --git a/point-cloud-toolbox_amd/csrc/pct_fit.hip b/point-cloud-toolbox_amd/csrc/pct_fit.hip
--- a/point-cloud-toolbox_amd/csrc/pct_fit.hip
+++ b/point-cloud-toolbox_amd/csrc/pct_fit.hip
@@ -36,6 +36,10 @@
     unsigned n_pts;
     const int* row_mask;
     int svd_accumulate;
+    const unsigned char* row_flag;
+    const int* redo;
+    const int* redo_count;
+    unsigned char* flag_clear;
     int blocks_per_xcd;
 };
 
@@ -136,19 +140,25 @@
     rot[0] = r00; rot[1] = r01; rot[2] = r02; rot[3] = r10; rot[4] = r11; rot[5] = r12; rot[6] = r20; rot[7] = r21; rot[8] = r22;
 }
 
-template <bool F64, bool OUT64 = false, bool STAGED = true, bool MASKED = false>
+template <bool F64, bool OUT64 = false, bool STAGED = true, bool MASKED = false, int TAIL = 0>
 __global__ __launch_bounds__(kFitBlock) void k_fit(FitArgs a) {
     extern __shared__ int s_idx[];
     const int lane = threadIdx.x;
-    if (blockIdx.x == 0) {
-        if (lane == 0 && a.flag_next) *a.flag_next = 0;
-        if (a.stat_dst && lane < 8) a.stat_dst[lane] = a.stat_src[lane];
-    }
-    const int64_t row0 = (a.blocks_per_xcd ? (int64_t)(blockIdx.x & 7u) * a.blocks_per_xcd + (blockIdx.x >> 3) : (int64_t)blockIdx.x) * kFitBlock;
-    if (row0 >= a.rows) return;
+    if constexpr (TAIL != 2) {
+        if (blockIdx.x == 0) {
+            if (lane == 0 && a.flag_next) *a.flag_next = 0;
+            if (a.stat_dst && lane < 8) a.stat_dst[lane] = a.stat_src[lane];
+        }
+    }
+    const int64_t rows = TAIL == 2 ? (int64_t)*a.redo_count : a.rows;
+    int64_t blk = TAIL != 2 && a.blocks_per_xcd ? (int64_t)(blockIdx.x & 7u) * a.blocks_per_xcd + (blockIdx.x >> 3) : (int64_t)blockIdx.x;
+    do {
+    const int64_t row0 = blk * kFitBlock;
+    if (row0 >= rows) break;
+    if constexpr (TAIL == 2) __syncthreads();
     const int k = a.k, kp = a.kp;
 
-    const int nrow = (int)min((int64_t)kFitBlock, a.rows - row0);
+    const int nrow = (int)min((int64_t)kFitBlock, rows - row0);
     if constexpr (STAGED) {
         const int sub = lane >> 4, c4 = (lane & 15) << 2;
         for (int cb = 0; cb < k; cb += 64) {
@@ -157,7 +167,8 @@
             for (int r0 = 0; r0 < kFitBlock; r0 += 4) {
                 const int r = r0 + sub;
                 if (r < nrow && c < a.pitch) {
-                    const int4 v = *(const int4*)(a.table + (row0 + r) * a.pitch + c);
+                    const int64_t trow = TAIL == 2 ? (int64_t)a.redo[row0 + r] : row0 + r;
+                    const int4 v = *(const int4*)(a.table + trow * a.pitch + c);
                     int* dst = s_idx + r * kp + c;
                     if (c + 0 < k) dst[0] = v.x;
                     if (c + 1 < k) dst[1] = v.y;
@@ -169,15 +180,18 @@
     }
     __syncthreads();
 
-    const int64_t row = row0 + lane;
-    if (row >= a.rows) return;
+    if (row0 + lane >= rows) continue;
+    const int64_t row = TAIL == 2 ? (int64_t)a.redo[row0 + lane] : row0 + lane;
     if constexpr (MASKED) {
-        if (!a.row_mask[row]) return;
+        if (!a.row_mask[row]) continue;
+    }
+    if constexpr (TAIL == 1) {
+        if (a.row_flag[row]) continue;
     }
     const int64_t qid = a.row_query32 ? (int64_t)a.row_query32[row] : a.row_query ? a.row_query[row] : row + a.row_offset;
     const float4 qp = a.pts[qid];
     const int pub = __float_as_int(qp.w);
-    if (!a.out_by_row && (pub < a.q_begin || pub >= a.q_end)) return;
+    if (!a.out_by_row && (pub < a.q_begin || pub >= a.q_end)) continue;
     const int64_t out = a.out_by_row ? row : (int64_t)pub - a.out_base;
 
     double qx = qp.x, qy = qp.y, qz = qp.z;
@@ -206,7 +220,7 @@
             a.K[out] = nanf_; a.H[out] = nanf_; a.H2[out] = nanf_;
         }
         if (m >= 2) hand_over();
-        return;
+        continue;
     }
 
     double sx = 0, sy = 0, sz = 0, sxx = 0, sxy = 0, sxz = 0, syy = 0, syz = 0, szz = 0;
@@ -250,7 +264,7 @@
             for (int j = 0; j < 6; ++j) a.coefs[out * 6 + j] = nanf_;
             a.K[out] = nanf_; a.H[out] = nanf_; a.H2[out] = nanf_;
         }
-        return;
+        continue;
     }
     double rot[9];
     plane_rotation<F64>(m, sx, sy, sz, sxx, sxy, sxz, syy, syz, szz, fx, fy, fz, lx, ly, lz, rot);
@@ -340,7 +354,7 @@
         const double wgt = (1.0 + Fx * Fx) + Fy * Fy;
         a.K64[out] = (Fxx * Fyy - Fxy * Fxy) / (wgt * wgt);
         a.H64[out] = (((1.0 + Fx * Fx) * Fyy - ((2.0 * Fx) * Fy) * Fxy) + (1.0 + Fy * Fy) * Fxx) / (2.0 * (wgt * sqrt(wgt)));
-        return;
+        continue;
     }
     const float A = (float)b[0], B = (float)b[1], C = (float)b[2];
     const float D = (float)b[3], E = (float)b[4], F = (float)b[5];
@@ -352,6 +366,7 @@
     a.K[out] = Kg;
     a.H[out] = Kh;
     a.H2[out] = Kh * Kh;
+    } while (TAIL == 2 && ((blk += gridDim.x), true));
 }
 
 __global__ __launch_bounds__(256) void k_curv(const float* __restrict__ coefs, int64_t rows, float* __restrict__ K,
@@ -475,6 +490,11 @@
                                                 long long* __restrict__ host_count) {
     const int total = *list_count;
     if (blockIdx.x == 0 && threadIdx.x == 0) *host_count = (a.svd_accumulate ? *host_count : 0ll) + total;
+    if (blockIdx.x == 0 && a.stat_dst && threadIdx.x < 8) a.stat_dst[threadIdx.x] = a.stat_src[threadIdx.x];
+    if (a.flag_clear) {
+        const int listed = *a.redo_count;
+        for (int64_t it = (int64_t)blockIdx.x * 64 + threadIdx.x; it < listed; it += (int64_t)gridDim.x * 64) a.flag_clear[a.redo[it]] = 0;
+    }
     const float nanf_ = __int_as_float(0x7fc00000);
     for (int64_t it = (int64_t)blockIdx.x * 64 + threadIdx.x; it < total; it += (int64_t)gridDim.x * 64) {
         const int64_t row = list[it];
@@ -636,12 +656,20 @@
         ctx->fit_flag_seen = ctx->fit_flag.p;
         ctx->fit_flag_cap_seen = ctx->fit_flag.cap;
         ctx->fit_parity = 0;
-    }
+        if (ctx->tail_fork) {
+            PCT_HIP(ctx, hipEventRecord(ctx->ev_tail, ctx->stream));
+            PCT_HIP(ctx, hipStreamWaitEvent(ctx->side, ctx->ev_tail, 0));
+        }
+    }
+    const bool tail = ctx->tail_fork && a.row_flag && staged && !a.row_mask && !a.coefs64;
+    if (ctx->tail_fork && !tail) return pct_fail(ctx, PCT_ERR_INVALID, "fit: a forked sweep without its listed fit");
+    FitArgs sv = a;
     a.stat_src = nullptr;
     a.stat_dst = nullptr;
     if (ctx->stats_mirror_req && ctx->counters.p) {
-        a.stat_src = (const unsigned long long*)ctx->counters.p;
-        a.stat_dst = (unsigned long long*)(ctx->pin + (ctx->fit_par ? 256 : 192));
+        FitArgs& m = tail ? sv : a;
+        m.stat_src = (const unsigned long long*)ctx->counters.p;
+        m.stat_dst = (unsigned long long*)(ctx->pin + (ctx->fit_par ? 256 : 192));
         ctx->stats_mirrored = true;
     }
     ctx->stats_mirror_req = false;
@@ -649,6 +677,23 @@
     a.flag_next = (int*)ctx->fit_flag.p + (ctx->fit_parity ^ 1);
     ctx->fit_parity ^= 1;
     a.flag_list = (int*)ctx->fit_flag.p + 16;
+    sv.flag_count = a.flag_count; sv.flag_next = a.flag_next; sv.flag_list = a.flag_list;
+    sv.kp = a.kp; sv.blocks_per_xcd = a.blocks_per_xcd;
+    if (tail) {
+        sv.flag_clear = (unsigned char*)ctx->row_flag.p;
+        const int lblocks = blocks < 256 ? blocks : 256;
+        if (f64) {
+            PCT_LAUNCH((k_fit<true, false, true, false, 1>), dim3(blocks), dim3(kFitBlock), lds, ctx->stream, a);
+            PCT_LAUNCH((k_fit<true, false, true, false, 2>), dim3(lblocks), dim3(kFitBlock), lds, ctx->side, a);
+        } else {
+            PCT_LAUNCH((k_fit<false, false, true, false, 1>), dim3(blocks), dim3(kFitBlock), lds, ctx->stream, a);
+            PCT_LAUNCH((k_fit<false, false, true, false, 2>), dim3(lblocks), dim3(kFitBlock), lds, ctx->side, a);
+        }
+        PCT_HIP(ctx, hipGetLastError());
+        PCT_HIP(ctx, hipEventRecord(ctx->ev_tail, ctx->side));
+        PCT_HIP(ctx, hipStreamWaitEvent(ctx->stream, ctx->ev_tail, 0));
+        ctx->tail_fork = false;
+    } else {
 #define PCT_FIT_LAUNCH(F_, O_)                                                                                      \
     do {                                                                                                            \
         if (a.row_mask && staged && !O_) PCT_LAUNCH((k_fit<F_, false, true, true>), dim3(blocks), dim3(kFitBlock), lds, ctx->stream, a); \
@@ -662,17 +707,18 @@
     else PCT_FIT_LAUNCH(false, false);
 #undef PCT_FIT_LAUNCH
     PCT_HIP(ctx, hipGetLastError());
+    }
     const int sblocks = blocks < 1024 ? blocks : 1024;
     long long* note = (long long*)(ctx->pin + 2048 + 8 * ctx->fit_par);
     if (a.coefs64) {
         if (f64)
-            PCT_LAUNCH((k_fit_svd<true, true>), dim3(sblocks), dim3(64), 0, ctx->stream, a, a.flag_list, a.flag_count, note);
+            PCT_LAUNCH((k_fit_svd<true, true>), dim3(sblocks), dim3(64), 0, ctx->stream, sv, sv.flag_list, sv.flag_count, note);
         else
-            PCT_LAUNCH((k_fit_svd<false, true>), dim3(sblocks), dim3(64), 0, ctx->stream, a, a.flag_list, a.flag_count, note);
+            PCT_LAUNCH((k_fit_svd<false, true>), dim3(sblocks), dim3(64), 0, ctx->stream, sv, sv.flag_list, sv.flag_count, note);
     } else if (f64)
-        PCT_LAUNCH((k_fit_svd<true, false>), dim3(sblocks), dim3(64), 0, ctx->stream, a, a.flag_list, a.flag_count, note);
+        PCT_LAUNCH((k_fit_svd<true, false>), dim3(sblocks), dim3(64), 0, ctx->stream, sv, sv.flag_list, sv.flag_count, note);
     else
-        PCT_LAUNCH((k_fit_svd<false, false>), dim3(sblocks), dim3(64), 0, ctx->stream, a, a.flag_list, a.flag_count, note);
+        PCT_LAUNCH((k_fit_svd<false, false>), dim3(sblocks), dim3(64), 0, ctx->stream, sv, sv.flag_list, sv.flag_count, note);
     PCT_HIP(ctx, hipGetLastError());
     return PCT_OK;
 }
@@ -741,6 +787,11 @@
     a.H = (float*)ctx->H.p;
     a.H2 = (float*)ctx->H2.p;
     a.n_pts = (unsigned)(sorted ? ctx->n_grid : ctx->n);
+    if (ctx->tail_fork) {
+        a.row_flag = (const unsigned char*)ctx->row_flag.p;
+        a.redo = (const int*)ctx->redo.p;
+        a.redo_count = (const int*)ctx->counters.p + 14;
+    }
     return launch(ctx, a, ctx->has_f64);
 }
 
diff --git a/point-cloud-toolbox_amd/csrc/pct_internal.h b/point-cloud-toolbox_amd/csrc/pct_internal.h
--- a/point-cloud-toolbox_amd/csrc/pct_internal.h
+++ b/point-cloud-toolbox_amd/csrc/pct_internal.h
@@ -40,6 +40,9 @@
     int device = 0;
     pct_comm* comm = nullptr;
     hipStream_t stream = nullptr;
+    hipStream_t side = nullptr;
+    hipEvent_t ev_tail = nullptr;
+    bool tail_fork = false;
     hipEvent_t ev[9] = {};
     hipEvent_t ev_prev[9] = {};
     bool async_mode = false;
@@ -132,6 +135,9 @@
     pct_buf bin_base;
     pct_buf occ;
     pct_buf redo;
+    pct_buf row_flag;
+    void* row_flag_seen = nullptr;
+    size_t row_flag_cap_seen = 0;
     int64_t n_items = 0;
     int64_t nonempty_cells = 0;
     int32_t items_q = 12;
@@ -192,6 +198,7 @@
 int pct_fail(pct_ctx* ctx, int code, const char* fmt, ...);
 const char* pct_getenv(const char* name);
 void pct_comm_release(pct_ctx* ctx);
+void pct_tail_abandon(pct_ctx* ctx);
 
 #ifndef PCT_FAST_R1_MAX
 #define PCT_FAST_R1_MAX 61
diff --git a/point-cloud-toolbox_amd/csrc/pct_knn.hip b/point-cloud-toolbox_amd/csrc/pct_knn.hip
--- a/point-cloud-toolbox_amd/csrc/pct_knn.hip
+++ b/point-cloud-toolbox_amd/csrc/pct_knn.hip
@@ -292,6 +292,7 @@
         base = __builtin_amdgcn_readfirstlane(base);
         if (lane < nq) {
             redo[base + lane] = row0 + lane;
+            if (a.redo_flag) a.redo_flag[row0 + lane] = 1;
         }
         if (a.stats && lane == 0) {
             if (!hopeless) atomicAdd(&a.counters[1], 1ull);
@@ -987,7 +988,10 @@
             int base = 0;
             if (lane == 0) base = atomicAdd(redo_count, cnt);
             base = __builtin_amdgcn_readfirstlane(base);
-            if ((redo_mask >> lane) & 1ull) redo[base + (int)__popcll(redo_mask & ((1ull << lane) - 1ull))] = row0 + lane;
+            if ((redo_mask >> lane) & 1ull) {
+                redo[base + (int)__popcll(redo_mask & ((1ull << lane) - 1ull))] = row0 + lane;
+                if (a.redo_flag) a.redo_flag[row0 + lane] = 1;
+            }
         }
         n_redo += (unsigned long long)cnt;
     }
@@ -1025,6 +1029,7 @@
     int* nbr_cnt;
     int* redo;
     int* redo_count;
+    unsigned char* redo_flag;
     unsigned long long* counters;
     int n_items, items_q;
     int items_per_xcd;
@@ -1150,7 +1155,10 @@
         int base = 0;
         if (lane == 0) base = atomicAdd(a.redo_count, nq);
         base = __builtin_amdgcn_readfirstlane(base);
-        if (lane < nq) a.redo[base + lane] = row0 + lane;
+        if (lane < nq) {
+            a.redo[base + lane] = row0 + lane;
+            if (a.redo_flag) a.redo_flag[row0 + lane] = 1;
+        }
         if (a.stats && lane == 0) {
             atomicAdd(&a.counters[1], 1ull);
             atomicAdd(&a.counters[4], (unsigned long long)nq);
@@ -1523,7 +1531,10 @@
         int base = 0;
         if (lane == 0) base = atomicAdd(a.redo_count, cnt);
         base = __builtin_amdgcn_readfirstlane(base);
-        if ((redo_mask >> lane) & 1ull) a.redo[base + (int)__popcll(redo_mask & ((1ull << lane) - 1ull))] = row0 + lane;
+        if ((redo_mask >> lane) & 1ull) {
+            a.redo[base + (int)__popcll(redo_mask & ((1ull << lane) - 1ull))] = row0 + lane;
+            if (a.redo_flag) a.redo_flag[row0 + lane] = 1;
+        }
         if (a.stats && lane == 0) atomicAdd(&a.counters[4], (unsigned long long)cnt);
     }
 }
@@ -1643,7 +1654,10 @@
         int base = 0;
         if (lane == 0) base = atomicAdd(a.redo_count, nq);
         base = __builtin_amdgcn_readfirstlane(base);
-        if (lane < nq) a.redo[base + lane] = row0 + lane;
+        if (lane < nq) {
+            a.redo[base + lane] = row0 + lane;
+            if (a.redo_flag) a.redo_flag[row0 + lane] = 1;
+        }
         if (a.stats && lane == 0) {
             atomicAdd(&a.counters[1], 1ull);
             atomicAdd(&a.counters[4], (unsigned long long)nq);
@@ -1909,7 +1923,10 @@
         int base = 0;
         if (lane == 0) base = atomicAdd(a.redo_count, cnt);
         base = __builtin_amdgcn_readfirstlane(base);
-        if ((redo_mask >> lane) & 1ull) a.redo[base + (int)__popcll(redo_mask & ((1ull << lane) - 1ull))] = row0 + lane;
+        if ((redo_mask >> lane) & 1ull) {
+            a.redo[base + (int)__popcll(redo_mask & ((1ull << lane) - 1ull))] = row0 + lane;
+            if (a.redo_flag) a.redo_flag[row0 + lane] = 1;
+        }
         if (a.stats && lane == 0) atomicAdd(&a.counters[4], (unsigned long long)cnt);
     }
 }
@@ -2120,6 +2137,17 @@
     }
     KnnArgs a = make_args(ctx, k, eps, true);
     if (!ctx->dist_valid) a.nbr_dist = nullptr;
+    const bool tail = phase == 0 && !exact_only && ctx->skip_dist_req && !ctx->own_flag && !ctx->level_mode && ctx->n_items > 0 &&
+                      k + 1 <= 128 && ctx->side && !pct_getenv("PCT_NO_TAIL_OVERLAP");
+    if (tail) {
+        PCT_TRY(pct_reserve(ctx, &ctx->row_flag, (size_t)n_rows));
+        if (ctx->row_flag.p != ctx->row_flag_seen || ctx->row_flag.cap != ctx->row_flag_cap_seen) {
+            PCT_HIP(ctx, hipMemsetAsync(ctx->row_flag.p, 0, ctx->row_flag.cap, ctx->stream));
+            ctx->row_flag_seen = ctx->row_flag.p;
+            ctx->row_flag_cap_seen = ctx->row_flag.cap;
+        }
+        a.redo_flag = (unsigned char*)ctx->row_flag.p;
+    }
     int* redo_count = (int*)ctx->counters.p + 14;
     int* redo = (int*)ctx->redo.p;
     const dim3 block(64 * kWavesPerBlock);
@@ -2147,6 +2175,7 @@
             pa.items = items;
             pa.nbr_pos = a.nbr_pos; pa.nbr_dist = a.nbr_dist; pa.nbr_cnt = a.nbr_cnt;
             pa.redo = redo; pa.redo_count = redo_count; pa.counters = a.counters;
+            pa.redo_flag = a.redo_flag;
             pa.n_items = (int)ctx->n_items; pa.items_q = ctx->items_q;
             pa.k = a.k; pa.pitch = a.pitch; pa.stats = a.stats; pa.eps2 = a.eps2; pa.g = a.g;
             const auto magic = [](unsigned d, unsigned* mg, int* sh) {
@@ -2213,10 +2242,16 @@
         const int64_t waves = exact_only ? n_rows : 32768;
         const int blocks = (int)((waves + kWavesPerBlock - 1) / kWavesPerBlock);
         const int* list = exact_only ? nullptr : redo;
+        hipStream_t st = ctx->stream;
+        if (tail) {
+            PCT_HIP(ctx, hipStreamWaitEvent(ctx->side, ctx->ev[7], 0));
+            ctx->tail_fork = true;
+            st = ctx->side;
+        }
         if (k + 1 <= 64)
-            PCT_LAUNCH(k_knn_exact<1>, dim3(blocks), block, 0, ctx->stream, a, list, (const int*)redo_count);
+            PCT_LAUNCH(k_knn_exact<1>, dim3(blocks), block, 0, st, a, list, (const int*)redo_count);
         else if (k + 1 <= 128)
-            PCT_LAUNCH(k_knn_exact<2>, dim3(blocks), block, 0, ctx->stream, a, list, (const int*)redo_count);
+            PCT_LAUNCH(k_knn_exact<2>, dim3(blocks), block, 0, st, a, list, (const int*)redo_count);
         else
             PCT_TRY(pct_launch_knn_exact_wide(ctx, a, blocks, list, (const int*)redo_count));
         PCT_HIP(ctx, hipGetLastError());
diff --git a/point-cloud-toolbox_amd/csrc/pct_knn_sweep.h b/point-cloud-toolbox_amd/csrc/pct_knn_sweep.h
--- a/point-cloud-toolbox_amd/csrc/pct_knn_sweep.h
+++ b/point-cloud-toolbox_amd/csrc/pct_knn_sweep.h
@@ -33,6 +33,7 @@
     const int* tree_bucket;
     int stats;
     unsigned long long* counters;
+    unsigned char* redo_flag;
 };
 
 int pct_launch_knn_exact_wide(pct_ctx* ctx, const KnnArgs& a, int blocks, const int* list, const int* list_count);
```

After: 1.353 billion. 3.6% lower.
